# laurabragagnolo/SkelSplat

Hardware: AMD Instinct MI355X
Metric: rendered+backpropagated views/s (differentiable skeletal-Gaussian rasterizer fwd+bwd) (higher is better)
Workload: dtype f32

## Files before the change

include/skelsplat_hip.h:

```cpp
#ifndef SKELSPLAT_HIP_H
#define SKELSPLAT_HIP_H

#include <stddef.h>
#include <stdint.h>

#ifdef __cplusplus
extern "C" {
#endif

#define SKS_MAX_VIEWS 64
#define SKS_MAX_CHANNELS 32
#define SKS_SMALL_P 256

#define SKS_ANTIALIASING 1u
#define SKS_CLAMP01      2u
#define SKS_FORCE_BINNED 4u
#define SKS_DEBUG_SYNC   8u

#define SKS_NO_NT_STORES 16u

#define SKS_RAW_PARAMS   32u
#define SKS_RAW_GRADS    128u
#define SKS_BIN_CLEAN    64u
#define SKS_BIN_GROUPS_SHIFT 16
#define SKS_BIN_GROUPS(n) ((unsigned)(((n) - 1) & 7) << SKS_BIN_GROUPS_SHIFT)
#define SKS_FILL_LINEAR (1u << 21)
#define SKS_FILL_ROWS (1u << 22)
#define SKS_BWD_LDS_LIST (1u << 20)
#define SKS_BWD_WG_SHIFT 23
#define SKS_NO_EARLY_FILL (1u << 30)
#define SKS_EARLY_FILL(n) (((unsigned)(n) & 7u) << SKS_BIN_GROUPS_SHIFT)

const char* sks_last_error(void);
int sks_version(void);

int sks_scratch_bytes(int V, int P, int C, int W, int H, size_t bin_capacity,
                      size_t* geom_bytes, size_t* binning_bytes, size_t* accum_bytes);

int sks_forward(int V, int P, int C, int W, int H,
                const float* viewmatrix, const float* projmatrix,
                const float* tanfovx , const float* tanfovy ,
                const float* means3D, const float* features, const float* opacities,
                const float* scales, const float* rotations, const float* cov3D_precomp,
                float scale_modifier, unsigned flags,
                float* out_color, float* out_invdepth, int* radii,
                void* geom, void* binning, size_t bin_capacity, int* num_rendered_dev,
                float* final_T, uint32_t* n_contrib, void* stream);

int sks_backward(int V, int P, int C, int W, int H,
                 const float* viewmatrix, const float* projmatrix,
                 const float* tanfovx , const float* tanfovy ,
                 const float* bg,
                 const float* means3D, const float* features, const float* opacities,
                 const float* scales, const float* rotations, const float* cov3D_precomp,
                 float scale_modifier, unsigned flags,
                 const int* radii, const void* geom, const void* binning, size_t bin_capacity,
                 const float* dL_dout_color, const float* dL_dout_invdepth,
                 void* accum,
                 float* dL_dmeans3D, float* dL_dmeans2D, float* dL_dopacity,
                 float* dL_dscales, float* dL_drotations, float* dL_dcov3D, float* dL_dfeatures,
                 float* dL_dmeans3D_mean ,
                 void* stream);

#define SKS_FB_NO_JOIN 1u
int sks_forward_backward(int V, int P, int C, int W, int H,
                         const float* viewmatrix, const float* projmatrix,
                         const float* tanfovx , const float* tanfovy ,
                         const float* means3D, const float* features, const float* opacities,
                         const float* scales, const float* rotations, const float* cov3D_precomp,
                         float scale_modifier, unsigned flags,
                         float* out_color, float* out_invdepth, int* radii,
                         void* geom, void* binning, size_t bin_capacity, int* num_rendered_dev,
                         const float* bg, const float* dL_dout_color, const float* dL_dout_invdepth, void* accum,
                         float* dL_dmeans3D, float* dL_dmeans2D, float* dL_dopacity,
                         float* dL_dscales, float* dL_drotations, float* dL_dcov3D, float* dL_dfeatures,
                         float* dL_dmeans3D_mean, void* stream, void* aux_stream, unsigned fb_flags);

int sks_mean_views(int V, int P, const float* dL_dmeans3D, int shard_world, float* mean_out , void* stream);

int sks_mark_visible(int P, const float* means3D, const float* viewmatrix, const float* projmatrix,
                     uint8_t* present, void* stream);

int sks_export_lists(int V, int W, int H, const void* binning, size_t bin_capacity,
                     uint32_t* point_list, uint32_t* ranges, void* stream);

int sks_masked_l2(int V, size_t n_per_view, const float* render, const float* gt, float* dL_unscaled, double* sums,
                  void* stream);
int sks_masked_l2_loss(int V, size_t n_per_view, const float* render, const float* gt, float* dL_unscaled, double* sums,
                       float* loss , float* scale , int mean, void* stream);

#define SKS_SOFTARGMAX_STATS 6
size_t sks_softargmax_scratch_bytes(int planes, int W, int H);
int sks_softargmax_fwd(int planes, int W, int H, float beta, const float* img, float* xy ,
                       float* stats , void* scratch, size_t scratch_bytes, void* stream);
int sks_softargmax_bwd(int planes, int W, int H, float beta, const float* img, const float* stats ,
                       const float* dL_dxy , float* dL_dimg, void* stream);

int sks_heatmaps(int V, int J, int W, int H, const float* row, const float* col, const float* cmin, const float* den,
                 float* out, double* gt_totals, void* stream);
int sks_heatmap_factors(int V, int J, int W, int H, const float* means3D, const float* scales, const float* rotations,
                        float scale_modifier, const float* poses_2d, const float* viewmatrix, const float* tanfovx,
                        const float* tanfovy, float* row, float* col, float* cmin, float* den,
                        int frames ,
                        const int* view_wh ,
                        void* stream);
int sks_heatmap_totals(int V, int J, int W, int H, const float* row, const float* col, const float* cmin, const float* den,
                       const int* view_wh, double* gt_totals, void* stream);

int sks_triangulate(int N, int V, int J, const double* proj, size_t rig_stride, const float* poses_2d,
                    const double* poses_2d_f64, const unsigned char* valid, float* xyz, double* xyzw, int* n_used,
                    void* stream);

int sks_fuse_predictions(int N, int V, int J, const double* proj, size_t rig_stride, const float* poses_3d,
                         const double* poses_3d_f64, const float* poses_2d, const double* poses_2d_f64,
                         const unsigned char* valid, int norm_f32, float* xyz, double* xyz_f64, double* reproj_err,
                         int* n_used, void* stream);

int sks_fused_ssim_fwd(int B, int CH, int H, int W, float C1, float C2, const float* img1, const float* img2,
                       float* ssim_map, float* dm_dmu1, float* dm_dsigma1_sq, float* dm_dsigma12, void* stream);

int sks_fused_ssim_bwd(int B, int CH, int H, int W, float C1, float C2, const float* img1, const float* img2,
                       const float* dL_dmap, const float* dm_dmu1, const float* dm_dsigma1_sq, const float* dm_dsigma12,
                       float* dL_dimg1, void* stream);
int sks_fused_ssim_bwd_uniform(int B, int CH, int H, int W, const float* img1, const float* img2, const float* dL_value,
                               float dL_scale, int crop, const float* dm_dmu1, const float* dm_dsigma1_sq,
                               const float* dm_dsigma12, float* dL_dimg1, void* stream);
#define SKS_SSIM_SUM_SLOTS 64
#define SKS_SSIM_SCRATCH_BYTES (SKS_SSIM_SUM_SLOTS * 8)
int sks_fused_ssim_mean(int B, int CH, int H, int W, float C1, float C2, const float* img1, const float* img2, int crop,
                        float* dm_dmu1, float* dm_dsigma1_sq, float* dm_dsigma12, double* scratch, float* mean_out,
                        void* stream);

int sks_knn3_meandist2(int P, const float* points, float* mean_dist2, void* stream);
size_t sks_knn3_scratch_bytes(int P);
int sks_knn3_meandist2_grid(int P, const float* points, float* mean_dist2, void* scratch, size_t scratch_bytes, void* stream);

int sks_gt_tile_stats(int V, int C, int W, int H, const float* gt, float* tile_S, float* tile_N, double* totals, void* stream);
int sks_geometry(int V, int P, int C, int W, int H, const float* viewmatrix, const float* projmatrix,
                 const float* tanfovx , const float* tanfovy , const float* means3D,
                 const float* opacities, const float* scales, const float* rotations, const float* cov3D_precomp,
                 float scale_modifier, unsigned flags, int* radii, void* geom,
                 const int* view_wh , int frames ,
                 void* stream);
int sks_backward_fused_loss(int V, int P, int C, int W, int H, const float* viewmatrix, const float* projmatrix,
                            const float* tanfovx , const float* tanfovy , const float* bg,
                            const float* means3D, const float* features, const float* opacities, const float* scales,
                            const float* rotations, const float* cov3D_precomp, float scale_modifier, unsigned flags,
                            const int* radii, const void* geom, const float* gt, const float* tile_S, const float* tile_N,
                            const double* gt_totals, void* accum, float* dL_dmeans3D, float* dL_dmeans2D,
                            float* dL_dopacity, float* dL_dscales, float* dL_drotations, float* dL_dcov3D,
                            double* loss_sums, float* packed_raw_grads ,
                            const int* view_wh , const size_t* gt_offsets ,
                            const float* const* hm_factors , void* stream);

int sks_loop_pack_grads(int V, int P, const float* dL_dmeans3D, const float* dL_dscales, const float* dL_drotations,
                        const float* dL_dopacity, const float* raw_scaling, const float* raw_rotation,
                        const float* raw_opacity, const double* loss_sums, float* packed, void* stream);
int sks_loop_adam_step(int V, int P, const float* grads, float* slots, unsigned long long group_mask, int last_view,
                       float* xyz, float* scaling, float* rotation, float* opacity, float* exp_avg, float* exp_avg_sq,
                       int* counters, int acc_steps, const double* lr_sched ,
                       const double* lrs , const double* adam ,
                       float lambda_consistency, const int* limb ,
                       int shard_world ,
                       void* stream);

int sks_loop_adam_step_es(int V, int P, const float* grads, float* slots, unsigned long long group_mask, int last_view,
                          float* xyz, float* scaling, float* rotation, float* opacity, float* exp_avg, float* exp_avg_sq,
                          int* counters, int acc_steps, const double* lr_sched , const double* lrs ,
                          const double* adam , float lambda_consistency, const int* limb ,
                          int shard_world, const double* loss_sums, int* es_state, int es_window, float es_tolerance,
                          int* es_host_flag , void* stream);
size_t sks_loop_shard_floats(int V, int P, int shard_world);

int sks_adam_multi(int n_tensors, float* const* params, const float* const* grads, float* const* exp_avg, float* const* exp_avg_sq,
                   const long long* numel, const double* lr, const long long* step, double beta1, double beta2, double eps, void* stream);

int sks_loop_fused_step(int V, int P, int C, int W, int H, const float* viewmatrix, const float* projmatrix,
                        const float* tanfovx , const float* tanfovy , const float* features,
                        float scale_modifier, unsigned flags, int* radii, void* geom, const float* gt,
                        const double* gt_totals, void* accum, double* loss_sums, float* packed, float* slots,
                        unsigned long long group_mask, int last_view, float* xyz, float* scaling, float* rotation,
                        float* opacity, float* exp_avg, float* exp_avg_sq, int* counters, int acc_steps,
                        const double* lr_sched , const double* lrs , const double* adam ,
                        float lambda_consistency, const int* limb ,
                        const int* view_wh , const size_t* gt_offsets ,
                        int frames, const float* const* hm_factors ,
                        void* stream);
int sks_loop_fused_step_es(int V, int P, int C, int W, int H, const float* viewmatrix, const float* projmatrix,
                           const float* tanfovx , const float* tanfovy , const float* features,
                           float scale_modifier, unsigned flags, int* radii, void* geom, const float* gt,
                           const double* gt_totals, void* accum, double* loss_sums, float* packed, float* slots,
                           unsigned long long group_mask, int last_view, float* xyz, float* scaling, float* rotation,
                           float* opacity, float* exp_avg, float* exp_avg_sq, int* counters, int acc_steps,
                           const double* lr_sched , const double* lrs , const double* adam ,
                           float lambda_consistency, const int* limb ,
                           const int* view_wh , const size_t* gt_offsets ,
                           int frames, const float* const* hm_factors ,
                           int* es_state, int es_window, float es_tolerance, int* es_host_flags ,
                           void* stream);

int sks_rig_select(int R, int V, int frames, const int* rig_ids, const float* bank_viewmatrix, const float* bank_projmatrix,
                   const float* bank_tan, const int* slot_wh, const double* bank_proj, const double* bank_sched,
                   float* viewmatrix, float* projmatrix, void* views_dev, double* proj, double* lr_sched_dev, int* error_word,
                   void* stream);
int sks_geometry_dv(int V, int P, int C, int W, int H, const float* viewmatrix, const float* projmatrix, const void* views_dev,
                    const float* means3D, const float* opacities, const float* scales, const float* rotations,
                    const float* cov3D_precomp, float scale_modifier, unsigned flags, int* radii, void* geom, int frames,
                    void* stream);
int sks_heatmap_factors_dv(int V, int J, int W, int H, const float* means3D, const float* scales, const float* rotations,
                           float scale_modifier, const float* poses_2d, const float* viewmatrix, const void* views_dev,
                           float* row, float* col, float* cmin, float* den, int frames, void* stream);
int sks_heatmap_totals_dv(int V, int J, int W, int H, const float* row, const float* col, const float* cmin, const float* den,
                          const void* views_dev, double* gt_totals, void* stream);
int sks_loop_fused_step_dv(int V, int P, int C, int W, int H, const float* viewmatrix, const float* projmatrix,
                           const void* views_dev, const float* features, float scale_modifier, unsigned flags, int* radii,
// ... 38 lines not shown
```

skelsplat_amd/_lib.py:

```python
import ctypes as C
import os

_HERE = os.path.dirname(os.path.abspath(__file__))
LIB_PATH = os.path.join(_HERE, "libskelsplat_hip.so")
_lib = None

SKS_MAX_VIEWS = 64
SKS_MAX_CHANNELS = 32
SKS_SMALL_P = 256
SKS_ANTIALIASING = 1
SKS_CLAMP01 = 2
SKS_FORCE_BINNED = 4
SKS_DEBUG_SYNC = 8
SKS_NO_NT_STORES = 16
SKS_RAW_PARAMS = 32
SKS_BIN_CLEAN = 64
SKS_RAW_GRADS = 128
SKS_FB_NO_JOIN = 1
SKS_BIN_GROUPS_SHIFT = 16
SKS_BWD_WG_SHIFT = 23
SKS_SSIM_SCRATCH_BYTES = 64 * 8
SKS_SOFTARGMAX_STATS = 6
SKS_REPORT_MAX_SAVES = 8
SKS_EVAL_MAX_GROUPS = 64


SKS_NO_EARLY_FILL = 1 << 30


def SKS_EARLY_FILL(n):
    return (int(n) & 7) << SKS_BIN_GROUPS_SHIFT


def SKS_BIN_GROUPS(n):
    return ((int(n) - 1) & 7) << SKS_BIN_GROUPS_SHIFT


_vp, _i, _u, _f, _sz = C.c_void_p, C.c_int, C.c_uint, C.c_float, C.c_size_t

_CAMERAS = (("V", _i), ("P", _i), ("C", _i), ("W", _i), ("H", _i), ("viewmatrix", _vp), ("projmatrix", _vp),
            ("tanfovx", _vp), ("tanfovy", _vp))
_GAUSSIANS = (("means3D", _vp), ("features", _vp), ("opacities", _vp), ("scales", _vp), ("rotations", _vp),
              ("cov3D_precomp", _vp), ("scale_modifier", _f), ("flags", _u))
_UPSTREAM = (("dL_dout_color", _vp), ("dL_dout_invdepth", _vp), ("accum", _vp))
_GRADS = (("dL_dmeans3D", _vp), ("dL_dmeans2D", _vp), ("dL_dopacity", _vp), ("dL_dscales", _vp), ("dL_drotations", _vp),
          ("dL_dcov3D", _vp), ("dL_dfeatures", _vp), ("dL_dmeans3D_mean", _vp))
_FORWARD_IO = (("out_color", _vp), ("out_invdepth", _vp), ("radii", _vp), ("geom", _vp), ("binning", _vp),
               ("bin_capacity", _sz), ("num_rendered_dev", _vp))
FORWARD_PARAMS = _CAMERAS + _GAUSSIANS + _FORWARD_IO + (("final_T", _vp), ("n_contrib", _vp), ("stream", _vp))
BACKWARD_PARAMS = _CAMERAS + (("bg", _vp),) + _GAUSSIANS + (("radii", _vp), ("geom", _vp), ("binning", _vp), ("bin_capacity", _sz)) \
    + _UPSTREAM + _GRADS + (("stream", _vp),)
FORWARD_BACKWARD_PARAMS = _CAMERAS + _GAUSSIANS + _FORWARD_IO + (("bg", _vp),) + _UPSTREAM + _GRADS \
    + (("stream", _vp), ("aux_stream", _vp), ("fb_flags", _u))

FWD, BWD, FWD_BWD = ({name: i for i, (name, _) in enumerate(params)}
                     for params in (FORWARD_PARAMS, BACKWARD_PARAMS, FORWARD_BACKWARD_PARAMS))
FWD_BWD_SOURCES = tuple(("fwd", FWD[n]) if n in FWD else ("bwd", BWD[n]) if n in BWD else None for n in FWD_BWD)

_ull = C.c_ulonglong
_VIEWS_DV = (("viewmatrix", _vp), ("projmatrix", _vp), ("views_dev", _vp))
RIG_SELECT_PARAMS = (("R", _i), ("V", _i), ("frames", _i), ("rig_ids", _vp), ("bank_viewmatrix", _vp), ("bank_projmatrix", _vp),
                     ("bank_tan", _vp), ("slot_wh", _vp), ("bank_proj", _vp), ("bank_sched", _vp), ("viewmatrix", _vp),
                     ("projmatrix", _vp), ("views_dev", _vp), ("proj", _vp), ("lr_sched_dev", _vp), ("error_word", _vp),
                     ("stream", _vp))
GEOMETRY_DV_PARAMS = (("V", _i), ("P", _i), ("C", _i), ("W", _i), ("H", _i)) + _VIEWS_DV + (
    ("means3D", _vp), ("opacities", _vp), ("scales", _vp), ("rotations", _vp), ("cov3D_precomp", _vp), ("scale_modifier", _f),
    ("flags", _u), ("radii", _vp), ("geom", _vp), ("frames", _i), ("stream", _vp))
HEATMAP_FACTORS_DV_PARAMS = (("V", _i), ("J", _i), ("W", _i), ("H", _i), ("means3D", _vp), ("scales", _vp), ("rotations", _vp),
                             ("scale_modifier", _f), ("poses_2d", _vp), ("viewmatrix", _vp), ("views_dev", _vp), ("row", _vp),
                             ("col", _vp), ("cmin", _vp), ("den", _vp), ("frames", _i), ("stream", _vp))
HEATMAP_TOTALS_DV_PARAMS = (("V", _i), ("J", _i), ("W", _i), ("H", _i), ("row", _vp), ("col", _vp), ("cmin", _vp), ("den", _vp),
                            ("views_dev", _vp), ("gt_totals", _vp), ("stream", _vp))
OPTIMISER_PARAMS = (("slots", _vp), ("group_mask", _ull), ("last_view", _i), ("xyz", _vp), ("scaling", _vp), ("rotation", _vp),
                    ("opacity", _vp), ("exp_avg", _vp), ("exp_avg_sq", _vp), ("counters", _vp), ("acc_steps", _i),
                    ("lr_sched", _vp), ("lrs", _vp), ("adam", _vp), ("lambda_consistency", _f), ("limb", _vp))
OPTIMISER_DV_PARAMS = tuple(("lr_sched_dev", ct) if name == "lr_sched" else (name, ct) for name, ct in OPTIMISER_PARAMS)
_ES = (("es_state", _vp), ("es_window", _i), ("es_tolerance", _f))
ES_PARAMS, ES_FRAMES_PARAMS = _ES + (("es_host_flag", _vp),), _ES + (("es_host_flags", _vp),)
_ADAM_STEP = (("V", _i), ("P", _i), ("grads", _vp)) + OPTIMISER_PARAMS + (("shard_world", _i),)
_STEP_RENDER = (("features", _vp), ("scale_modifier", _f), ("flags", _u), ("radii", _vp), ("geom", _vp), ("gt", _vp),
                ("gt_totals", _vp), ("accum", _vp), ("loss_sums", _vp), ("packed", _vp))
_STEP_HEATMAPS = (("view_wh", _vp), ("gt_offsets", _vp), ("frames", _i), ("hm_factors", _vp))
_STEP = _CAMERAS + _STEP_RENDER + OPTIMISER_PARAMS + _STEP_HEATMAPS
_STEP_DV = (("V", _i), ("P", _i), ("C", _i), ("W", _i), ("H", _i)) + _VIEWS_DV + _STEP_RENDER + OPTIMISER_DV_PARAMS + _STEP_HEATMAPS
LOOP_ADAM_STEP_PARAMS = _ADAM_STEP + (("stream", _vp),)
LOOP_ADAM_STEP_ES_PARAMS = _ADAM_STEP + (("loss_sums", _vp),) + ES_PARAMS + (("stream", _vp),)
LOOP_FUSED_STEP_PARAMS = _STEP + (("stream", _vp),)
LOOP_FUSED_STEP_ES_PARAMS = _STEP + ES_FRAMES_PARAMS + (("stream", _vp),)
LOOP_FUSED_STEP_DV_PARAMS = _STEP_DV + (("stream", _vp),)
LOOP_FUSED_STEP_ES_DV_PARAMS = _STEP_DV + ES_FRAMES_PARAMS + (("stream", _vp),)
STEP_PARAMS = {"sks_loop_adam_step": LOOP_ADAM_STEP_PARAMS, "sks_loop_adam_step_es": LOOP_ADAM_STEP_ES_PARAMS,
               "sks_loop_fused_step": LOOP_FUSED_STEP_PARAMS, "sks_loop_fused_step_es": LOOP_FUSED_STEP_ES_PARAMS}
DV_PARAMS = {"sks_rig_select": RIG_SELECT_PARAMS, "sks_geometry_dv": GEOMETRY_DV_PARAMS,
             "sks_heatmap_factors_dv": HEATMAP_FACTORS_DV_PARAMS, "sks_heatmap_totals_dv": HEATMAP_TOTALS_DV_PARAMS,
             "sks_loop_fused_step_dv": LOOP_FUSED_STEP_DV_PARAMS, "sks_loop_fused_step_es_dv": LOOP_FUSED_STEP_ES_DV_PARAMS}

SIGNATURES = {
    "sks_last_error": (C.c_char_p, []),
    "sks_version": (_i, []),
    "sks_scratch_bytes": (_i, [_i, _i, _i, _i, _i, _sz, C.POINTER(_sz), C.POINTER(_sz), C.POINTER(_sz)]),
    "sks_forward": (_i, [ct for _, ct in FORWARD_PARAMS]),
    "sks_backward": (_i, [ct for _, ct in BACKWARD_PARAMS]),
    "sks_forward_backward": (_i, [ct for _, ct in FORWARD_BACKWARD_PARAMS]),
    "sks_mark_visible": (_i, [_i, _vp, _vp, _vp, _vp, _vp]),
    "sks_mean_views": (_i, [_i, _i, _vp, _i, _vp, _vp]),
    "sks_export_lists": (_i, [_i, _i, _i, _vp, _sz, _vp, _vp, _vp]),
    "sks_masked_l2": (_i, [_i, _sz, _vp, _vp, _vp, _vp, _vp]),
    "sks_masked_l2_loss": (_i, [_i, _sz, _vp, _vp, _vp, _vp, _vp, _vp, _i, _vp]),
    "sks_fused_ssim_fwd": (_i, [_i, _i, _i, _i, _f, _f, _vp, _vp, _vp, _vp, _vp, _vp, _vp]),
    "sks_fused_ssim_bwd": (_i, [_i, _i, _i, _i, _f, _f, _vp, _vp, _vp, _vp, _vp, _vp, _vp, _vp]),
    "sks_fused_ssim_bwd_uniform": (_i, [_i, _i, _i, _i, _vp, _vp, _vp, _f, _i, _vp, _vp, _vp, _vp, _vp]),
    "sks_fused_ssim_mean": (_i, [_i, _i, _i, _i, _f, _f, _vp, _vp, _i, _vp, _vp, _vp, _vp, _vp, _vp]),
    "sks_knn3_meandist2": (_i, [_i, _vp, _vp, _vp]),
    "sks_knn3_scratch_bytes": (_sz, [_i]),
    "sks_knn3_meandist2_grid": (_i, [_i, _vp, _vp, _vp, _sz, _vp]),
    "sks_softargmax_scratch_bytes": (_sz, [_i, _i, _i]),
    "sks_softargmax_fwd": (_i, [_i, _i, _i, _f, _vp, _vp, _vp, _vp, _sz, _vp]),
    "sks_softargmax_bwd": (_i, [_i, _i, _i, _f, _vp, _vp, _vp, _vp, _vp]),
    "sks_heatmaps": (_i, [_i, _i, _i, _i, _vp, _vp, _vp, _vp, _vp, _vp, _vp]),
    "sks_heatmap_factors": (_i, [_i, _i, _i, _i, _vp, _vp, _vp, _f, _vp, _vp, _vp, _vp, _vp, _vp, _vp, _vp, _i, _vp, _vp]),
    "sks_heatmap_totals": (_i, [_i, _i, _i, _i, _vp, _vp, _vp, _vp, _vp, _vp, _vp]),
    "sks_gt_tile_stats": (_i, [_i, _i, _i, _i, _vp, _vp, _vp, _vp, _vp]),
    "sks_geometry": (_i, [_i, _i, _i, _i, _i, _vp, _vp, _vp, _vp, _vp, _vp, _vp, _vp, _vp, _f, _u, _vp, _vp, _vp, _i, _vp]),
    "sks_backward_fused_loss": (_i, [_i, _i, _i, _i, _i, _vp, _vp, _vp, _vp, _vp, _vp, _vp, _vp, _vp, _vp, _vp, _f, _u,
                                     _vp, _vp, _vp, _vp, _vp, _vp, _vp, _vp, _vp, _vp, _vp, _vp, _vp, _vp, _vp, _vp, _vp, _vp, _vp]),
    "sks_loop_pack_grads": (_i, [_i, _i, _vp, _vp, _vp, _vp, _vp, _vp, _vp, _vp, _vp, _vp]),
    "sks_loop_shard_floats": (_sz, [_i, _i, _i]),
    "sks_adam_multi": (_i, [_i, _vp, _vp, _vp, _vp, _vp, _vp, _vp, C.c_double, C.c_double, C.c_double, _vp]),
    "sks_triangulate": (_i, [_i, _i, _i, _vp, _sz, _vp, _vp, _vp, _vp, _vp, _vp, _vp]),
    "sks_fuse_predictions": (_i, [_i, _i, _i, _vp, _sz, _vp, _vp, _vp, _vp, _vp, _i, _vp, _vp, _vp, _vp, _vp]),
    **{name: (_i, [ct for _, ct in params]) for name, params in {**STEP_PARAMS, **DV_PARAMS}.items()},
    "sks_pose_errors": (_i, [_i, _i, _vp, _vp, _vp, _vp, _vp]),
    "sks_loop_report": (_i, [_i, _i, _i, _vp, _vp, _i, _vp, _vp, _vp, _i, _i, _vp, _vp, _vp, _i, _vp, _vp, _vp]),
    "sks_eval_sequence": (_i, [_i, _i, _vp, _vp, _vp, _i, _vp, _vp, _vp]),
    "sks_prof_enable": (_i, [_i]),
    "sks_prof_spin": (_i, [C.c_double, _vp]),
    "sks_prof_read": (_i, [_i, C.POINTER(C.c_double), C.POINTER(C.c_longlong)]),
    "sks_prof_count": (_i, [_i, C.POINTER(C.c_longlong)]),
    "sks_prof_read_quantiles": (_i, [_i, C.POINTER(C.c_double), C.POINTER(C.c_double), C.POINTER(C.c_longlong)]),
}


def load(build_if_missing=True):
    global _lib
    if _lib is not None:
        return _lib
    if build_if_missing:
        try:
            from . import build as _b
            if _b._stale():
                _b.build()
        except Exception as e:
            if not os.path.exists(LIB_PATH):
                raise ImportError(f"libskelsplat_hip.so is missing and could not be built: {e}") from e
    if not os.path.exists(LIB_PATH):
        raise ImportError(f"{LIB_PATH} not found; run `python -m skelsplat_amd.build`")
    lib = C.CDLL(os.environ.get("SKS_LIB_OVERRIDE") or LIB_PATH)
    for name, (res, args) in SIGNATURES.items():
        fn = getattr(lib, name)
        fn.restype = res
        fn.argtypes = args
    _lib = lib
    return lib


def check(rc, what):
    if rc != 0:
        msg = load().sks_last_error().decode(errors="replace")
        raise RuntimeError(f"{what} failed (code {rc}): {msg}")


def scratch_bytes(V, P, C_, W, H, bin_capacity=0):
    g, b, a = _sz(0), _sz(0), _sz(0)
    check(load().sks_scratch_bytes(V, P, C_, W, H, bin_capacity, C.byref(g), C.byref(b), C.byref(a)), "sks_scratch_bytes")
    return g.value, b.value, a.value


def ptr(t):
    if t is None or t.numel() == 0:
        return None
    return t.data_ptr()


def farray(vals):
    return (C.c_float * len(vals))(*[float(v) for v in vals])


def prof_count(kind):
    n = C.c_longlong(0)
    check(load().sks_prof_count(kind, C.byref(n)), "sks_prof_count")
    return n.value


def prof_enable(on, every=1, kinds=(0, 1), recorded=False):
    skip = sum(1 << (16 + k) for k in (0, 1) if k not in kinds)
    check(load().sks_prof_enable((min(0xffff, max(1, int(every))) | skip | ((1 << 18) if recorded else 0)) if on else 0),
          "sks_prof_enable")


def prof_read_quantiles(kind):
    q = (C.c_double * 3)()
    ms, n = C.c_double(0), C.c_longlong(0)
    check(load().sks_prof_read_quantiles(kind, q, C.byref(ms), C.byref(n)), "sks_prof_read_quantiles")
    return ms.value, n.value, (q[0], q[1], q[2])


def prof_read(kind):
    ms, n = C.c_double(0), C.c_longlong(0)
    check(load().sks_prof_read(kind, C.byref(ms), C.byref(n)), "sks_prof_read")
    return ms.value, n.value
```

skelsplat_amd/csrc/sks_bwd_small.inc:

```
template <int CG>
struct BwdPix {
    float T, T_final, last_alpha, accum_inv, last_inv, dLi, bgdot;
    float dL[CG], accum_rec[CG], last_color[CG];
};

struct BwdArgs {
    int P, C, W, H;
    unsigned flags;
    Geom g;
    const float* features;
    const float* bg;
    const float* dL_color;
    const float* dL_invdepth;
    float* accum;
    const float* tile_S;
    const float* tile_N;
    const float* hm_row = nullptr;
    const float* hm_col = nullptr;
    const float* hm_cmin = nullptr;
    const float* hm_den = nullptr;
    const int* es_stop = nullptr;
    int es_stride = 0;
    int es_views = 1;
};
// ... 86 lines not shown
        L.invd[rank] = xyd.w;
        L.xr[rank] = (int)(r.x | (r.z << 16));
        L.yr[rank] = (int)(r.y | (r.w << 16));
        L.id[rank] = tid;
    }
    __syncthreads();
    if (tid < CG) {
        bool act = false;
        if (tid < C) {
            act = DFEAT || a.bg != nullptr;
            for (int k = 0; k < n && !act; k++) act = L.r_feat[L.id[k] * C + tid] != 0.0f;
        }
        s_act[tid] = act ? 1 : 0;
    }
    __syncthreads();
    if (tid < CG && s_act[tid]) {
        int pos = 0;
        for (int c = 0; c < tid; c++) pos += s_act[c];
        s_chan[pos] = tid;
    }
    int nc = 0;
    for (int c = 0; c < CG; c++) nc += s_act[c];
    __syncthreads();
    if (tid < n) {
        const int id = L.id[tid];
#pragma unroll
        for (int j = 0; j < CG; j++) L.feat[tid * CG + j] = j < nc ? L.r_feat[id * C + s_chan[j]] : 0.0f;
    }
    __syncthreads();
    int kg = 0;
    for (int k = 0; k < n; k++) kg = L.id[k] == g ? k : kg;
    const bool do_clamp = a.flags & SKS_CLAMP01;
    const float ddelx_dx = (float)(0.5 * W), ddely_dy = (float)(0.5 * H);
    float sum[NV];
#pragma unroll
    for (int j = 0; j < NV; j++) sum[j] = 0.0f;

    for (int c = sp; c < nchunks; c += BWD_SPLITS) {
        const int i = c * 256 + tid;
        if (i >= npx) continue;
        const int yy = i / wpx;
        const int x = x0 + (i - yy * wpx), y = y0 + yy;
        const int tx = x >> 4, ty = y >> 4;
        const float pxf = (float)x, pyf = (float)y;
        float T = 1.0f, col[CG];
#pragma unroll
        for (int ch = 0; ch < CG; ch++) col[ch] = 0.0f;
        int klast = -1;
        for (int k = 0; k < n; k++) {
            const int xr = L.xr[k], yr = L.yr[k];
            if (tx < (xr & 0xffff) || tx >= (xr >> 16) || ty < (yr & 0xffff) || ty >= (yr >> 16)) continue;
            const float2 xy = L.xy[k];
            const float4 co = L.co[k];
            const float dx = xy.x - pxf, dy = xy.y - pyf;
            const float power = -0.5f * (co.x * dx * dx + co.z * dy * dy) - co.y * dx * dy;
            if (power > 0.0f) continue;
            const float alpha = fminf(0.99f, co.w * expf_fixed(power));
            if (alpha < 1.0f / 255.0f) continue;
            const float test_T = T * (1 - alpha);
            if (test_T < 0.0001f) break;
            if (do_clamp) {
#pragma unroll
                for (int ch = 0; ch < CG; ch++) col[ch] += L.feat[k * CG + ch] * alpha * T;
            }
            T = test_T;
            klast = k;
        }
        if (klast < kg) continue;
        const size_t pix = (size_t)y * W + x;
        float dLraw[CG];
        {
            const float* dLc = a.dL_color + (size_t)v * C * HW + pix;
#pragma unroll
            for (int j = 0; j < CG; j++) dLraw[j] = j < nc ? dLc[(size_t)s_chan[j] * HW] : 0.0f;
        }
        const float dLi_raw = a.dL_invdepth ? a.dL_invdepth[(size_t)v * HW + pix] : 0.0f;
        BwdPix<CG> s;
        s.T = T;
        s.T_final = T;
        s.last_alpha = 0;
        s.accum_inv = 0;
        s.last_inv = 0;
        s.bgdot = 0;
        s.dLi = dLi_raw;
#pragma unroll
        for (int j = 0; j < CG; j++) {
            float d = dLraw[j];
            if (do_clamp && !(col[j] >= 0.0f && col[j] <= 1.0f)) d = 0.0f;
            if (a.bg && j < nc) s.bgdot += a.bg[s_chan[j]] * d;
            s.dL[j] = d;
            s.accum_rec[j] = 0;
            s.last_color[j] = 0;
        }
        for (int k = klast; k >= kg; k--) {
            const int xr = L.xr[k], yr = L.yr[k];
            if (tx < (xr & 0xffff) || tx >= (xr >> 16) || ty < (yr & 0xffff) || ty >= (yr >> 16)) continue;
            const float2 xy = L.xy[k];
            const float4 co = L.co[k];
            const float dx = xy.x - pxf, dy = xy.y - pyf;
            const float power = -0.5f * (co.x * dx * dx + co.z * dy * dy) - co.y * dx * dy;
            if (power > 0.0f) continue;
            const float G = expf_fixed(power);
            const float alpha = fminf(0.99f, co.w * G);
            if (alpha < 1.0f / 255.0f) continue;
            s.T = s.T / (1.f - alpha);
            const float dchannel_dcolor = alpha * s.T;
            float dL_dalpha = 0.0f;
            const bool mine = k == kg;
#pragma unroll
            for (int ch = 0; ch < CG; ch++) {
                const float cc = L.feat[k * CG + ch];
                s.accum_rec[ch] = s.last_alpha * s.last_color[ch] + (1.f - s.last_alpha) * s.accum_rec[ch];
                s.last_color[ch] = cc;
                const float dL_dchannel = s.dL[ch];
                dL_dalpha += (cc - s.accum_rec[ch]) * dL_dchannel;
                if (DFEAT && mine) sum[NACC + ch] += dchannel_dcolor * dL_dchannel;
            }
            const float invd = L.invd[k];
            s.accum_inv = s.last_alpha * s.last_inv + (1.f - s.last_alpha) * s.accum_inv;
            s.last_inv = invd;
            dL_dalpha += (invd - s.accum_inv) * s.dLi;
            dL_dalpha *= s.T;
            s.last_alpha = alpha;
            dL_dalpha += (-s.T_final / (1.f - alpha)) * s.bgdot;
            if (mine) {
                const float dL_dG = co.w * dL_dalpha;
                const float gdx = G * dx, gdy = G * dy;
                const float dG_ddelx = -gdx * co.x - gdy * co.y;
                const float dG_ddely = -gdy * co.z - gdx * co.y;
                sum[0] += dL_dG * dG_ddelx * ddelx_dx;
                sum[1] += dL_dG * dG_ddely * ddely_dy;
                sum[2] += -0.5f * gdx * dx * dL_dG;
                sum[3] += -0.5f * gdx * dy * dL_dG;
                sum[4] += -0.5f * gdy * dy * dL_dG;
                sum[5] += G * dL_dalpha;
                sum[6] += dchannel_dcolor * s.dLi;
            }
        }
    }
    const int lane = tid & 63, wv = tid >> 6;
#pragma unroll
    for (int j = 0; j < NV; j++) {
        const float r = wave_sum(sum[j]);
        if (lane == 0) s_red[wv][j] = r;
    }
    __syncthreads();
    if (tid < NVS)
        out[tid * BWD_SPLITS] = tid < NV ? ((s_red[0][tid] + s_red[1][tid]) + (s_red[2][tid] + s_red[3][tid])) : 0.0f;
}

__device__ __forceinline__ float rl(float x, int lane) { return __int_as_float(__builtin_amdgcn_readlane(__float_as_int(x), lane)); }
__device__ __forceinline__ unsigned rlu(unsigned x, int lane) { return (unsigned)__builtin_amdgcn_readlane((int)x, lane); }

template <int CG, bool DFEAT, bool LOSS, bool HMF = false, bool ES = false>
__global__ __launch_bounds__(256, (DFEAT || CG > 20) ? 1 : 4) void k_render_bwd_wave(BwdArgs a, ViewTan vt, ViewOff vo)
{
    static_assert(!(DFEAT && LOSS), "the fused-loss variant has no feature gradient");
    static_assert(LOSS || !HMF, "heat-map factors belong to the fused-loss variant");
    static_assert(LOSS || !ES, "early stopping belongs to the fused-loss variant");
    if constexpr (ES) {
        if (a.es_stop[(size_t)((int)blockIdx.y / a.es_views) * a.es_stride] != 0) return;
    }
    constexpr int NV = LOSS ? NACC + 1 : NACC + (DFEAT ? CG : 0);
    __shared__ float s_red[2][4][NV];
    const int g = blockIdx.x, v = blockIdx.y, sp = blockIdx.z, zs = gridDim.z, tid = threadIdx.x, lane = tid & 63, wv = tid >> 6;
    const int P = a.P, C = a.C, W = vt.w[v], H = vt.h[v];
    const int NVS = NACC + C;
    const size_t HW = (size_t)H * W;
    const size_t go = (size_t)v * P;
    const float* dL_view = a.dL_color + vo.off[v];
    float* out_g = a.accum + ((size_t)v * P + g) * NVS * BWD_SPLITS;
    const bool has = lane < P;
    const int li = has ? lane : 0;
    const float4 m_co = a.g.co[go + li];
    const float4 m_xyd = a.g.xyd[go + li];
    uint4 m_rect = a.g.rect[go + li];
    if (!has) m_rect = make_uint4(0, 0, 0, 0);
    float m_feat[CG];
    unsigned m_fmask = 0;
#pragma unroll
    for (int ch = 0; ch < CG; ch++) {
        m_feat[ch] = (ch < C && has) ? a.features[li * C + ch] : 0.0f;
        m_fmask |= m_feat[ch] != 0.0f ? (1u << ch) : 0u;
    }

    const unsigned gx0 = rlu(m_rect.x, g), gy0 = rlu(m_rect.y, g), gx1 = rlu(m_rect.z, g), gy1 = rlu(m_rect.w, g);
    const int wt = (int)gx1 - (int)gx0, ht = (int)gy1 - (int)gy0;
    const int nchunks = wt * ht;
    if (sp >= nchunks) {
        for (int slot = sp; slot < BWD_SPLITS; slot += zs)
            if (tid < NVS) out_g[tid * BWD_SPLITS + slot] = 0.0f;
        return;
    }
    const bool hit = m_rect.x < gx1 && m_rect.z > gx0 && m_rect.y < gy1 && m_rect.w > gy0;
    const unsigned long long hm = __ballot(hit);
    const int n = __popcll(hm);
    const unsigned mydepth = __float_as_uint(m_xyd.z);
    int rank = 0;
    for (unsigned long long m = hm; m; m &= m - 1) {
        const int j = __builtin_ctzll(m);
        const unsigned dj = rlu(mydepth, j);
        rank += (dj < mydepth || (dj == mydepth && j < lane)) ? 1 : 0;
    }
    const int kg = __builtin_amdgcn_readlane(rank, g);
    unsigned chmask = 0;
    if (DFEAT || a.bg != nullptr) {
        chmask = C >= 32 ? 0xffffffffu : ((1u << C) - 1u);
    } else {
        for (unsigned long long m = hm; m; m &= m - 1) chmask |= rlu(m_fmask, __builtin_ctzll(m));
    }
    const bool do_clamp = a.flags & SKS_CLAMP01;
    const float ddelx_dx = (float)(0.5 * W), ddely_dy = (float)(0.5 * H);
    const unsigned chmask_all = chmask;
    const size_t HW_all = HW;
    int buf = 0;
    for (int slot = sp; slot < BWD_SPLITS; slot += zs, buf ^= 1) {
    float* out = out_g + slot;
    if (slot >= nchunks) {
        if (tid < NVS) out[tid * BWD_SPLITS] = 0.0f;
        continue;
    }
    float sum[NV];
#pragma unroll
    for (int j = 0; j < NV; j++) sum[j] = 0.0f;
    for (int c = slot; c < nchunks; c += BWD_SPLITS) {
        unsigned chmask = chmask_all;
        size_t HW = HW_all;
        asm volatile("" : "+s"(chmask), "+s"(HW));
        const int tyl = c / wt;
        const int tx = (int)gx0 + (c - tyl * wt), ty = (int)gy0 + tyl;
        const int x = tx * TILE + (tid & 15), y = ty * TILE + (tid >> 4);
        const bool in = x < W && y < H;
        const float pxf = (float)x, pyf = (float)y;
        float T = 1.0f, col[CG];
#pragma unroll
        for (int ch = 0; ch < CG; ch++) col[ch] = 0.0f;
        int klast = -1;
        const bool hitc = hit && !((unsigned)tx < m_rect.x || (unsigned)tx >= m_rect.z || (unsigned)ty < m_rect.y || (unsigned)ty >= m_rect.w);
        const unsigned long long covm = __ballot(hitc);
        const int minid = covm ? __builtin_ctzll(covm) : 0x7fffffff;
        bool alive = in;
        unsigned chm_t = (DFEAT || a.bg != nullptr) ? chmask : 0u;
        for (int k = 0; k < n; k++) {
            const unsigned long long sel = __ballot(hitc && rank == k);
            if (!sel) continue;
            if (!LOSS && !__any(alive)) break;
            const int lk = __builtin_ctzll(sel);
            chm_t |= chmask & rlu(m_fmask, lk);
            const float ex = rl(m_xyd.x, lk), ey = rl(m_xyd.y, lk);
            const float cx = rl(m_co.x, lk), cy = rl(m_co.y, lk), cz = rl(m_co.z, lk), cw = rl(m_co.w, lk);
            const bool cov = alive;
            const float dx = ex - pxf, dy = ey - pyf;
            const float power = -0.5f * (cx * dx * dx + cz * dy * dy) - cy * dx * dy;
            const float alpha = fminf(0.99f, cw * expf_fixed(power));
            const float test_T = T * (1 - alpha);
            const bool pass = cov && !(power > 0.0f) && !(alpha < 1.0f / 255.0f);
            const bool stop = pass && test_T < 0.0001f;
            const bool acc = pass && !stop;
            if (do_clamp || LOSS) {
                for (unsigned fm = chmask & rlu(m_fmask, lk); fm; fm &= fm - 1) {
                    const int ch = __builtin_ctz(fm);
                    const float f = rl(m_feat[ch], lk);
                    const float add = f * alpha * T;
                    col[ch] += acc ? add : 0.0f;
                }
            }
            if (acc) { T = test_T; klast = k; }
            if (stop) alive = false;
        }
        const bool need = in && klast >= kg;
        bool own = false;
        if (LOSS && in && minid == g) {
            for (unsigned fm = chm_t; fm; fm &= fm - 1) own = own || col[__builtin_ctz(fm)] > 0.0f;
        }
        if (!__any(need || own)) continue;
        const size_t pix = (size_t)y * W + x;
        struct { float T, T_final, last_alpha, accum_inv, last_inv, bgdot, dLi; } s;
        s.T = T; s.T_final = T; s.last_alpha = 0; s.accum_inv = 0; s.last_inv = 0; s.bgdot = 0;
        s.dLi = (!LOSS && need && a.dL_invdepth) ? a.dL_invdepth[(size_t)v * HW + pix] : 0.0f;
        {
            const float* dLc = dL_view + pix;
            for (unsigned fm = chm_t; fm;) {
                int cc[4];
                float cv[4], gv[4];
#pragma unroll
                for (int i = 0; i < 4; i++) {
                    cc[i] = fm ? __builtin_ctz(fm) : -1;
                    fm &= fm - 1;
                }
#pragma unroll
                for (int i = 0; i < 4; i++) cv[i] = col[max(cc[i], 0)];
                if (HMF) {
                    float fr[4], fc[4], lo[4], dn[4];
#pragma unroll
                    for (int i = 0; i < 4; i++) {
                        const int vc = v * C + max(cc[i], 0);
                        const bool want = cc[i] >= 0 && (need || (own && cv[i] > 0.0f));
                        fr[i] = want ? a.hm_row[(size_t)vc * a.H + y] : 0.0f;
                        fc[i] = want ? a.hm_col[(size_t)vc * a.W + x] : 0.0f;
                        lo[i] = a.hm_cmin[vc];
                        dn[i] = a.hm_den[vc];
                    }
#pragma unroll
                    for (int i = 0; i < 4; i++) {
                        const bool want = cc[i] >= 0 && (need || (own && cv[i] > 0.0f));
                        gv[i] = want ? (fr[i] * fc[i] - lo[i]) / dn[i] : 0.0f;
                    }
                } else {
#pragma unroll
                    for (int i = 0; i < 4; i++) {
                        const bool want = LOSS ? (need || (own && cv[i] > 0.0f)) : need;
                        gv[i] = (cc[i] >= 0 && want) ? dLc[(size_t)max(cc[i], 0) * HW] : 0.0f;
                    }
                }
#pragma unroll
                for (int i = 0; i < 4; i++) {
                    if (cc[i] < 0) break;
                    const int ch = cc[i];
// ... 158 lines not shown
```

skelsplat_amd/csrc/sks_common.inc:

```
thread_local char g_err[512] = "";

int fail(int code, const char* fmt, ...)
{
    va_list ap;
    va_start(ap, fmt);
    vsnprintf(g_err, sizeof(g_err), fmt, ap);
    va_end(ap);
    return code;
}

#define HIP_TRY(expr)                                                                          \
    do {                                                                                       \
        hipError_t e_ = (expr);                                                                \
        if (e_ != hipSuccess) return fail((int)e_, "%s: %s", #expr, hipGetErrorString(e_));    \
    } while (0)

#define STAGE_CHECK(name)                                                                      \
    do {                                                                                       \
        HIP_TRY(hipGetLastError());                                                            \
        if (flags & SKS_DEBUG_SYNC) {                                                          \
            hipError_t e_ = hipStreamSynchronize(st);                                          \
            if (e_ != hipSuccess) return fail((int)e_, "stage %s: %s", name, hipGetErrorString(e_)); \
        }                                                                                      \
    } while (0)

constexpr int PROF_MAX = 16384;
struct ProfKind {
    hipEvent_t b[PROF_MAX], e[PROF_MAX];
    int created = 0, n = 0;
};
struct ProfState {
    bool on = false;
    int every = 1;
    int skip = 0;
    bool recorded = false;
    int seen[2] = { 0, 0 };
    ProfKind kind[2];
};
thread_local ProfState* tl_prof = nullptr;

struct ProfScope {
    ProfKind* k = nullptr;
    hipStream_t st;
    bool ext;
    bool began = false;
    ProfScope(int kind, hipStream_t s, bool ext_ = false) : st(s), ext(ext_)
    {
        ProfState* ps = tl_prof;
        if (!ps || !ps->on || ((ps->skip >> kind) & 1)) return;
        if (ps->seen[kind]++ % ps->every != 0) return;
        ProfKind& p = ps->kind[kind];
        if (p.n >= PROF_MAX) return;
        if (p.n >= p.created) {
            if (hipEventCreate(&p.b[p.created]) != hipSuccess || hipEventCreate(&p.e[p.created]) != hipSuccess) return;
            p.created++;
        }
        k = &p;
        if (ps->recorded) ext = false;
        if (!ext) (void)hipEventRecord(p.b[p.n], st);
    }
    hipEvent_t eb() const { return k->b[k->n]; }
    hipEvent_t ee() const { return k->e[k->n]; }
    ~ProfScope()
    {
        if (!k) return;
        if (!ext) (void)hipEventRecord(k->e[k->n], st);
        k->n++;
    }
};
#define SKS_LAUNCH(prof, kernel, grid, block, lds, stream, ...)                                                  \
    do {                                                                                                         \
        if ((prof).k)                                                                                            \
            hipExtLaunchKernelGGL(kernel, grid, block, lds, stream, (prof).began ? nullptr : (prof).eb(), (prof).ee(), 0, __VA_ARGS__); \
        else hipLaunchKernelGGL(kernel, grid, block, lds, stream, __VA_ARGS__);                                  \
    } while (0)
#define SKS_LAUNCH_FIRST(prof, kernel, grid, block, lds, stream, ...)                                            \
    do {                                                                                                         \
        if ((prof).k && (prof).ext) hipExtLaunchKernelGGL(kernel, grid, block, lds, stream, (prof).eb(), nullptr, 0, __VA_ARGS__); \
        else hipLaunchKernelGGL(kernel, grid, block, lds, stream, __VA_ARGS__);    \
        (prof).began = (prof).k != nullptr;                                                                      \
    } while (0)

constexpr int NACC = 8;
constexpr int BWD_SPLITS = 16;
constexpr int BWD_WG_PAIRS16 = 400;
constexpr int BWD_WG_PAIRS8 = 4096;

struct ViewTan {
    float x[SKS_MAX_VIEWS];
    float y[SKS_MAX_VIEWS];
    int w[SKS_MAX_VIEWS];
    int h[SKS_MAX_VIEWS];
};
struct ViewOff {
    unsigned long long off[SKS_MAX_VIEWS];
};
struct ViewTanDev {
    const float* x;
    const float* y;
    const int* w;
    const int* h;
    const double* sched;
};
inline ViewTanDev views_dev_from(const void* views_dev, const double* sched = nullptr)
{
    const ViewTan* t = (const ViewTan*)views_dev;
    return ViewTanDev{ t->x, t->y, t->w, t->h, sched };
}
inline bool fill_views(ViewTan& vt, ViewOff* vo, int V, int C, int W, int H, const float* tanfovx, const float* tanfovy,
                       const int* view_wh, const size_t* plane_off)
{
    for (int v = 0; v < V; v++) {
        vt.x[v] = tanfovx[v];
        vt.y[v] = tanfovy[v];
        vt.w[v] = view_wh ? view_wh[2 * v] : W;
        vt.h[v] = view_wh ? view_wh[2 * v + 1] : H;
        if (vt.w[v] < 1 || vt.h[v] < 1 || vt.w[v] > W || vt.h[v] > H) return false;
        if (vo) vo->off[v] = plane_off ? (unsigned long long)plane_off[v] : (unsigned long long)v * C * H * W;
    }
    return true;
}

struct Geom {
    float4* co;
    float4* xyd;
    uint4* rect;
    uint32_t* cover;
};

__host__ __device__ inline size_t align256(size_t x) { return (x + 255) & ~(size_t)255; }

struct Activated {
    float opacity, s[3], q[4], qnorm;
};
__device__ __forceinline__ Activated activate(bool raw, float op, const float s[3], const float q[4])
{
    Activated a;
    if (raw) {
        a.opacity = 1.0f / (1.0f + expf_fixed(-op));
#pragma unroll
        for (int k = 0; k < 3; k++) a.s[k] = expf_fixed(s[k]);
        const float nn = q[0] * q[0] + q[1] * q[1] + q[2] * q[2] + q[3] * q[3];
        a.qnorm = fmaxf(sqrtf(nn), 1e-12f);
#pragma unroll
        for (int k = 0; k < 4; k++) a.q[k] = q[k] / a.qnorm;
    } else {
        a.opacity = op;
        a.qnorm = 1.0f;
#pragma unroll
        for (int k = 0; k < 3; k++) a.s[k] = s[k];
#pragma unroll
        for (int k = 0; k < 4; k++) a.q[k] = q[k];
    }
    return a;
}

#ifndef SKS_COVER_MAX_WORDS
#define SKS_COVER_MAX_WORDS 6144
#endif
constexpr int COVER_MAX_WORDS = SKS_COVER_MAX_WORDS;
__host__ __device__ inline int cover_cw(int W) { return (1 + (((W + TILE - 1) / TILE) + 31) / 32 + 3) & ~3; }
inline bool cover_enabled(int P, int W, int H)
{
    return P <= SKS_SMALL_P && ((H + TILE - 1) / TILE) * cover_cw(W) <= COVER_MAX_WORDS;
}
inline bool cover_per_plane(int P, int W, int H, int C)
{
    return cover_enabled(P, W, H) && (C + 1) * ((H + TILE - 1) / TILE) * cover_cw(W) <= COVER_MAX_WORDS;
}
inline Geom geom_from(void* base, int V, int P, int W, int H)
{
    char* p = (char*)base;
    Geom g;
    size_t n = (size_t)V * P;
    g.co = (float4*)p; p += align256(n * sizeof(float4));
    g.xyd = (float4*)p; p += align256(n * sizeof(float4));
    g.rect = (uint4*)p; p += align256(n * sizeof(uint4));
    g.cover = cover_enabled(P, W, H) ? (uint32_t*)p : nullptr;
    return g;
}
inline size_t geom_bytes(int V, int P, int W, int H, int C)
{
    const int planes = cover_per_plane(P, W, H, C) ? C + 1 : 1;
    return 3 * align256((size_t)V * P * 16) + align256((size_t)V * planes * ((H + TILE - 1) / TILE) * cover_cw(W) * 4);
}

constexpr int BIN_WAVE_SORT = 64;
constexpr int BIN_ROWS = 2;
constexpr int BIN_CLASSES = 8;
constexpr int BIN_HDR_CLASS = 8;
constexpr int BIN_MAX_GROUPS = 7;
#ifndef SKS_BIN_FB_GROUPS
#define SKS_BIN_FB_GROUPS 1
#endif
constexpr int BIN_FB_GROUPS = SKS_BIN_FB_GROUPS;
inline int bin_groups_default()
{
    static const int n = [] {
        const char* e = getenv("SKS_BIN_GROUPS");
        const int want = (e && atoi(e) > 0) ? atoi(e) : BIN_FB_GROUPS;
        return want < 1 ? 1 : (want > BIN_MAX_GROUPS ? BIN_MAX_GROUPS : want);
    }();
    return n;
}
inline void bin_groups(unsigned flags, int V, int& vg, int& ng)
{
    const unsigned field = (flags >> SKS_BIN_GROUPS_SHIFT) & 7u;
    int want = field ? 1 + (int)field : bin_groups_default();
    if (want > BIN_MAX_GROUPS) want = BIN_MAX_GROUPS;
    if (want > V) want = V;
    vg = (V + want - 1) / want;
    ng = (V + vg - 1) / vg;
}
struct Bin {
    uint32_t* hdr;
    uint32_t* count;
    uint32_t* cursor;
    uint2* ranges;
    int* nrend;
    uint32_t* longt;
    uint4* tlist;
    uint32_t* tidx;
// ... 45 lines not shown
```

skelsplat_amd/csrc/sks_fwd_small.inc:

```
__device__ __forceinline__ float clamp01(float x) { return fminf(fmaxf(x, 0.0f), 1.0f); }

struct FwdArgs {
    int P, C, W, H;
    unsigned flags;
    Geom g;
    const float* features;
    float* out_color;
    float* out_invdepth;
    float* final_T;
    uint32_t* n_contrib;
    int tslots;
    unsigned cp1_magic;
    int ncomp;
    int cover_planes;
    unsigned w_magic;
};

inline int composite_slots(unsigned flags, int V, int P)
{
    const int t = (int)((flags >> 26) & 15u);
    return t ? t : ((long long)V * P <= 128 ? 4 : 8);
}

typedef float v4f __attribute__((ext_vector_type(4)));
// ... 225 lines not shown
    const int tid = threadIdx.x;
    const int P = a.P, C = a.C, W = a.W, H = a.H;
    const size_t HW = (size_t)H * W;

    const int xq = blockIdx.x, band_id = blockIdx.y, zid = blockIdx.z;
    const int xc = gridDim.x - fsplit;
    const bool comp_role = xq >= fsplit;
    if (comp_role) {
        const int cb = (zid * gy + band_id) * xc + (xq - fsplit);
        if (cb >= a.ncomp) return;
        const int T_SLOTS = a.tslots;
        const int slot = cb % T_SLOTS;
        const int g = (cb / T_SLOTS) % P;
        const int v = cb / (T_SLOTS * P);
        const size_t go = (size_t)v * P;
        const float4* gco = a.g.co + go;
        const float4* gxyd = a.g.xyd + go;
        const uint4* grect = a.g.rect + go;
        const uint4 rg = grect[g];
        const int wt = (int)(rg.z - rg.x), ht = (int)(rg.w - rg.y);
        const int ntiles = wt * ht;
        if (slot >= ntiles) return;
        const int cap = (P + 15) & ~15;
        DynList<CG> L(s_dyn, cap);
        if (tid < P) L.rect[tid] = grect[tid];
        __syncthreads();
        float* outc = a.out_color + (size_t)v * C * HW;
        float* outi = a.out_invdepth + (size_t)v * HW;
        const bool do_clamp = a.flags & SKS_CLAMP01;
        for (int t = slot; t < ntiles; t += T_SLOTS) {
            const int ty = (int)rg.y + t / wt, tx = (int)rg.x + t % wt;
            if (tid == 0) { s_n = 0; s_min = 0x7fffffff; }
            __syncthreads();
            if (tid < P) {
                const uint4 r = L.rect[tid];
                if ((int)r.x <= tx && tx < (int)r.z && (int)r.y <= ty && ty < (int)r.w) {
                    atomicMin(&s_min, tid);
                    const int sl = atomicAdd(&s_n, 1);
                    L.key[sl] = ((unsigned long long)__float_as_uint(gxyd[tid].z) << 32) | (unsigned)tid;
                }
            }
            __syncthreads();
            const int n = s_n;
            if (s_min == g) {
                if (tid < n) {
                    const unsigned long long key = L.key[tid];
                    int rank = 0;
                    for (int j = 0; j < n; j++) rank += (L.key[j] < key) ? 1 : 0;
                    const int id = (int)(unsigned)key;
                    const float4 xyd = gxyd[id];
                    L.xy[rank] = make_float2(xyd.x, xyd.y);
                    L.co[rank] = gco[id];
                    L.invd[rank] = xyd.w;
#pragma unroll
                    for (int ch = 0; ch < CG; ch++) L.feat[rank * CG + ch] = ch < C ? a.features[id * C + ch] : 0.0f;
                }
                __syncthreads();
                unsigned chm = 0xffffffffu;
                if (a.cover_planes) {
                    bool nz = false;
                    if (tid < CG)
                        for (int k = 0; k < n; k++) nz = nz || L.feat[k * CG + tid] != 0.0f;
                    if (tid < 64) {
                        const unsigned long long bl = __ballot(nz);
                        if (tid == 0) s_chm = (unsigned)bl;
                    }
                    __syncthreads();
                    chm = s_chm;
                }
                const int x = tx * TILE + (tid & 15), y = ty * TILE + (tid >> 4);
                if (x < W && y < H) {
                    const float pxf = (float)x, pyf = (float)y;
                    float T = 1.0f, inv = 0.0f, acc[CG];
#pragma unroll
                    for (int ch = 0; ch < CG; ch++) acc[ch] = 0.0f;
                    uint32_t contributor = 0, last = 0;
                    for (int k = 0; k < n; k++) {
                        contributor++;
                        const float2 xy = L.xy[k];
                        const float4 co = L.co[k];
                        const float dx = xy.x - pxf, dy = xy.y - pyf;
                        const float power = -0.5f * (co.x * dx * dx + co.z * dy * dy) - co.y * dx * dy;
                        if (power > 0.0f) continue;
                        const float alpha = fminf(0.99f, co.w * expf_fixed(power));
                        if (alpha < 1.0f / 255.0f) continue;
                        const float test_T = T * (1 - alpha);
                        if (test_T < 0.0001f) break;
#pragma unroll
                        for (int ch = 0; ch < CG; ch++) acc[ch] += L.feat[k * CG + ch] * alpha * T;
                        inv += L.invd[k] * alpha * T;
                        T = test_T;
                        last = contributor;
                    }
                    const size_t pix = (size_t)y * W + x;
#pragma unroll
                    for (int ch = 0; ch < CG; ch++)
                        if (ch < C && ((chm >> ch) & 1u)) outc[(size_t)ch * HW + pix] = do_clamp ? clamp01(acc[ch]) : acc[ch];
                    outi[pix] = inv;
                    if (a.final_T) a.final_T[(size_t)v * HW + pix] = T;
                    if (a.n_contrib) a.n_contrib[(size_t)v * HW + pix] = last;
                }
            }
            __syncthreads();
        }
        return;
    }
    fwd_fill_role<PPT, NT, HALF>(a, cp1_magic, xq, band_id, zid, gy, pb, cover);
}

struct EarlyFill {
    float* out_color;
    float* out_invdepth;
    int C, W, H, gy;
    int gplanes;
    int ngeom;
    int zid0;
    int fsplit, pb;
    unsigned cp1_magic;
    unsigned row_magic;
    unsigned fs_magic;
};

template <int PPT, bool NT>
__global__ __launch_bounds__(256) void k_geom_fwd_fill(EarlyFill f, int P, ViewTan vt, const float* __restrict__ vms,
                                                       const float* __restrict__ pms, const float* __restrict__ means,
                                                       const float* __restrict__ opac, const float* __restrict__ scales,
                                                       const float* __restrict__ rots, const float* __restrict__ cov3Dp, float smod,
                                                       unsigned flags, Geom g, int* __restrict__ radii,
                                                       const float* __restrict__ features, int cover_planes)
{
    const int b = blockIdx.x;
    if (b < f.ngeom) {
        const int v = f.gplanes == 1 ? b : (int)(((unsigned)b * f.cp1_magic) >> 20);
        extern __shared__ __attribute__((aligned(16))) char s_dyn[];
        geom_fwd_block((uint32_t*)s_dyn, 0, v, b - v * f.gplanes, P, f.W, f.H, vt, vms, pms, means, opac, scales, rots, cov3Dp, smod, flags, g, radii, 0,
                       nullptr, nullptr, features, f.C, nullptr, nullptr, cover_planes);
        return;
    }
    const unsigned e = (unsigned)(b - f.ngeom);
    const unsigned rows = (unsigned)(f.fsplit * f.gy);
    const unsigned zr = f.row_magic ? __umulhi(e, f.row_magic) : e;
    const unsigned rem = e - zr * rows;
    const int band = (int)(f.fs_magic ? __umulhi(rem, f.fs_magic) : rem);
    const int q = (int)rem - band * f.fsplit;
    const int zid = f.zid0 + (int)zr;
    const int v = (int)(((unsigned)zid * f.cp1_magic) >> 20);
    const int plane = zid - v * (f.C + 1);
    const size_t HW = (size_t)f.H * f.W;
    const int Nb = min(TILE, f.H - band * TILE) * f.W;
    float* out = (plane == f.C ? f.out_invdepth + (size_t)v * HW : f.out_color + ((size_t)v * f.C + plane) * HW) + (size_t)band * TILE * f.W;
    const int shift = (int)((reinterpret_cast<uintptr_t>(out) >> 2) & 31u);
    fill_bare<PPT, NT>(out, nullptr, nullptr, q * (256 * PPT) * f.pb + (int)threadIdx.x * PPT - shift, Nb, min(f.pb, 32));
}
```

skelsplat_amd/csrc/sks_geom_bwd.inc:

```
struct GeomBwdArgs {
    int P, C, W, H;
    unsigned flags;
    const float* vms;
    const float* pms;
    const float* means;
    const float* opac;
    const float* scales;
    const float* rots;
    const float* cov3Dp;
    float smod;
    const int* radii;
    const float* accum;
    int nsplit;
    const double* gt_totals;
    double* loss_sums;
    float* packed;
    float* dmeans3D;
    float* dmeans2D;
    float* dopacity;
    float* dscales;
    float* drots;
    float* dcov3D;
    float* dfeat;
    const uint4* rect = nullptr;
// ... 255 lines not shown
            M3 M2;
#pragma unroll
            for (int cc = 0; cc < 3; cc++)
#pragma unroll
                for (int rr = 0; rr < 3; rr++) M2.m[cc][rr] = 2.0f * M.m[cc][rr];
            const M3 dL_dM = m3mul(M2, dS);
            const M3 Rt = m3T(R);
            M3 dMt = m3T(dL_dM);
#pragma unroll
            for (int k = 0; k < 3; k++)
                dscale[k] = Rt.m[k][0] * dMt.m[k][0] + Rt.m[k][1] * dMt.m[k][1] + Rt.m[k][2] * dMt.m[k][2];
#pragma unroll
            for (int k = 0; k < 3; k++)
#pragma unroll
                for (int rr = 0; rr < 3; rr++) dMt.m[k][rr] *= s[k];
            dq[0] = 2 * z * (dMt.m[0][1] - dMt.m[1][0]) + 2 * y * (dMt.m[2][0] - dMt.m[0][2]) + 2 * x * (dMt.m[1][2] - dMt.m[2][1]);
            dq[1] = 2 * y * (dMt.m[1][0] + dMt.m[0][1]) + 2 * z * (dMt.m[2][0] + dMt.m[0][2]) + 2 * r * (dMt.m[1][2] - dMt.m[2][1]) - 4 * x * (dMt.m[2][2] + dMt.m[1][1]);
            dq[2] = 2 * x * (dMt.m[1][0] + dMt.m[0][1]) + 2 * r * (dMt.m[2][0] - dMt.m[0][2]) + 2 * z * (dMt.m[1][2] + dMt.m[2][1]) - 4 * y * (dMt.m[2][2] + dMt.m[0][0]);
            dq[3] = 2 * r * (dMt.m[0][1] - dMt.m[1][0]) + 2 * x * (dMt.m[2][0] + dMt.m[0][2]) + 2 * y * (dMt.m[1][2] + dMt.m[2][1]) - 4 * z * (dMt.m[1][1] + dMt.m[0][0]);
        }
    }
    if (a.dmeans3D) { a.dmeans3D[3 * o] = dmean[0]; a.dmeans3D[3 * o + 1] = dmean[1]; a.dmeans3D[3 * o + 2] = dmean[2]; }
    if (a.dmeans2D) { a.dmeans2D[3 * o] = dm2x; a.dmeans2D[3 * o + 1] = dm2y; a.dmeans2D[3 * o + 2] = 0.0f; }
    const bool rawg = (a.flags & SKS_RAW_PARAMS) && (a.flags & SKS_RAW_GRADS);
    if (a.dopacity) {
        float oj = 1.0f;
        if (rawg) {
            const float so = 1.0f / (1.0f + expf_fixed(-(PRE ? pre->opac : a.opac[idx])));
            oj = so * (1.0f - so);
        }
        a.dopacity[o] = dop * oj;
    }
    if (a.dcov3D) {
#pragma unroll
        for (int i = 0; i < 6; i++) a.dcov3D[6 * o + i] = dcov[i];
    }
    if (a.dscales) {
#pragma unroll
        for (int k = 0; k < 3; k++) a.dscales[3 * o + k] = dscale[k] * (rawg ? sc[k] : 1.0f);
    }
    if (a.drots) {
        float dot = 0.0f;
#pragma unroll
        for (int k = 0; k < 4; k++) dot += q[k] * dq[k];
#pragma unroll
        for (int k = 0; k < 4; k++) a.drots[4 * o + k] = rawg ? (dq[k] - q[k] * dot) / qnorm : dq[k];
    }
    if (a.packed) {
        float scl = 1.0f;
        if (a.loss_sums) scl = (float)(1.0 / (n_view < 1.0 ? 1.0 : n_view));
        float* pk = a.packed + o * 11;
        const bool raw = a.flags & SKS_RAW_PARAMS;
        pk[0] = dmean[0] * scl; pk[1] = dmean[1] * scl; pk[2] = dmean[2] * scl;
#pragma unroll
        for (int k = 0; k < 3; k++) pk[3 + k] = dscale[k] * (raw ? sc[k] : 1.0f) * scl;
        float dot = 0.0f;
#pragma unroll
        for (int k = 0; k < 4; k++) dot += q[k] * dq[k];
#pragma unroll
        for (int k = 0; k < 4; k++) pk[6 + k] = (raw ? (dq[k] - q[k] * dot) / qnorm : dq[k]) * scl;
        float oj = 1.0f;
        if (raw) {
            const float so = 1.0f / (1.0f + expf_fixed(-(PRE ? pre->opac : a.opac[idx])));
            oj = so * (1.0f - so);
        }
        pk[10] = dop * oj * scl;
    }
}

__global__ __launch_bounds__(256) void k_geom_bwd(GeomBwdArgs a, ViewTan vt)
{
    const int idx = blockIdx.x * 256 + threadIdx.x;
    const int v = blockIdx.y;
    float g[NACC];
    double pS, pN;
    if (a.dfeat) geom_bwd_dfeat(a, (size_t)v * a.P + blockIdx.x * 256, min(256, a.P - (int)blockIdx.x * 256), threadIdx.x, 256);
    geom_bwd_load<false>(a, v, idx, g, pS, pN);
    double n_view = 1.0;
    if (a.loss_sums) {
        __shared__ double s_l[2][4];
        pS = wave_sum_d(pS);
        pN = wave_sum_d(pN);
        if ((threadIdx.x & 63) == 0) { s_l[0][threadIdx.x >> 6] = pS; s_l[1][threadIdx.x >> 6] = pN; }
        __syncthreads();
        const double S = a.gt_totals[2 * v] + ((s_l[0][0] + s_l[0][1]) + (s_l[0][2] + s_l[0][3]));
        n_view = a.gt_totals[2 * v + 1] + ((s_l[1][0] + s_l[1][1]) + (s_l[1][2] + s_l[1][3]));
        if (threadIdx.x == 0) {
            a.loss_sums[2 * v] = S;
            a.loss_sums[2 * v + 1] = n_view;
        }
    }
    if (idx >= a.P) return;
    geom_bwd_finish(a, vt, v, idx, g, n_view);
}

constexpr int GEOMB_G = 64;
__global__ __launch_bounds__(256) void k_geom_bwd_binned(GeomBwdArgs a, ViewTan vt)
{
    __shared__ float s_g[GEOMB_G][4][NACC];
    const int tid = threadIdx.x, v = blockIdx.y + a.v0;
    const int idx = blockIdx.x * GEOMB_G + tid;
    GeomBwdIn in;
    const bool mine = tid < GEOMB_G && idx < a.P;
    if (mine) geom_bwd_fetch(a, v, idx, in);
    {
        const int gi = tid >> 2, st = tid & 3;
        const int gidx = blockIdx.x * GEOMB_G + gi;
        float sum[NACC];
#pragma unroll
        for (int k = 0; k < NACC; k++) sum[k] = 0.0f;
        if (gidx < a.P) {
            const size_t o = (size_t)v * a.P + gidx;
            const uint4 r = a.rect[o];
            const int n = BIN_ROWS * (int)((r.z - r.x) * (r.w - r.y));
            const size_t s0 = BIN_ROWS * (size_t)a.goff[o], send = BIN_ROWS * a.cap;
            const float4* rows = reinterpret_cast<const float4*>(a.part + (size_t)v * a.cap * BIN_ROWS * NACC);
            for (int i = st; i < n; i += 16) {
                float4 q[4][2];
#pragma unroll
                for (int u = 0; u < 4; u++) {
                    const bool on = i + 4 * u < n && s0 + i + 4 * u < send;
                    q[u][0] = on ? rows[(s0 + i + 4 * u) * 2] : make_float4(0, 0, 0, 0);
                    q[u][1] = on ? rows[(s0 + i + 4 * u) * 2 + 1] : make_float4(0, 0, 0, 0);
                }
#pragma unroll
                for (int u = 0; u < 4; u++) {
                    sum[0] += q[u][0].x; sum[1] += q[u][0].y; sum[2] += q[u][0].z; sum[3] += q[u][0].w;
                    sum[4] += q[u][1].x; sum[5] += q[u][1].y; sum[6] += q[u][1].z;
                }
            }
        }
        float4* sg = reinterpret_cast<float4*>(s_g[gi][st]);
        sg[0] = make_float4(sum[0], sum[1], sum[2], sum[3]);
        sg[1] = make_float4(sum[4], sum[5], sum[6], 0.0f);
    }
    __syncthreads();
    if (!mine) return;
    float g[NACC];
#pragma unroll
    for (int k = 0; k < NACC - 1; k++) g[k] = (s_g[tid][0][k] + s_g[tid][1][k]) + (s_g[tid][2][k] + s_g[tid][3][k]);
    g[NACC - 1] = 0.0f;
    if (a.bin_hdr[0]) {
#pragma unroll
        for (int k = 0; k < NACC - 1; k++) g[k] = __int_as_float(0x7fc00000);
    }
    if (a.dfeat) {
        const size_t o = (size_t)v * a.P + idx;
        const float* acc = a.accum + o * (NACC + a.C);
        for (int ch = 0; ch < a.C; ch++) a.dfeat[o * a.C + ch] = acc[NACC + ch];
    }
    geom_bwd_finish<true>(a, vt, v, idx, g, 1.0, &in);
}

__global__ __launch_bounds__(256) void k_geom_bwd_all(GeomBwdArgs a, ViewTan vt, int V, float* __restrict__ mean_out)
{
    const int t = threadIdx.x;
    const int v = t / a.P, idx = t - v * a.P;
    const bool live = v < V;
    float g[NACC];
    double pS, pN;
    if (a.dfeat) geom_bwd_dfeat(a, 0, V * a.P, t, 256);
    if (live) {
        geom_bwd_load<false>(a, v, idx, g, pS, pN);
        geom_bwd_finish(a, vt, v, idx, g, 1.0);
    }
    __syncthreads();
    if (t < a.P) {
        float m[3] = { 0.0f, 0.0f, 0.0f };
        for (int w0 = 0; w0 < V; w0 += 4) {
            float tv[4][3];
#pragma unroll
            for (int j = 0; j < 4; j++) {
                const float* gm = a.dmeans3D + ((size_t)(w0 + j < V ? w0 + j : V - 1) * a.P + t) * 3;
                tv[j][0] = gm[0]; tv[j][1] = gm[1]; tv[j][2] = gm[2];
            }
#pragma unroll
            for (int j = 0; j < 4; j++)
                if (w0 + j < V) { m[0] += tv[j][0]; m[1] += tv[j][1]; m[2] += tv[j][2]; }
        }
        mean_out[3 * t] = m[0] / (float)V; mean_out[3 * t + 1] = m[1] / (float)V; mean_out[3 * t + 2] = m[2] / (float)V;
    }
}
__global__ void k_mean_views(int V, int P, const float* __restrict__ dmeans3D, float* __restrict__ mean_out, int world = 1)
{
    const int i = blockIdx.x * blockDim.x + threadIdx.x;
    if (i >= 3 * P) return;
    const int vmax = (V + world - 1) / world;
    float m = 0.0f;
    for (int w0 = 0; w0 < V; w0 += 8) {
        float t[8];
#pragma unroll
        for (int j = 0; j < 8; j++) {
            const int w = w0 + j < V ? w0 + j : V - 1;
            const int row = world == 1 ? w : (w % world) * vmax + w / world;
            t[j] = dmeans3D[(size_t)row * P * 3 + i];
        }
#pragma unroll
        for (int j = 0; j < 8; j++)
            if (w0 + j < V) m += t[j];
    }
    mean_out[i] = m / (float)V;
}

template <bool ES = false, class VT = ViewTan>
__global__ __launch_bounds__(256) void k_step_tail(GeomBwdArgs ga, VT vt, sksloop::AdamArgs aa, int V, Geom g, int* radii)
{
    __shared__ float s_xyz[256 * 3];
    __shared__ float s_hyp[6];
    __shared__ double s_d[4];
    __shared__ int s_it[2];
    __shared__ float s_np[64 * 11];
    const int tid = threadIdx.x, lane = tid & 63, wv = tid >> 6;
    const int P = ga.P;
    const int f = blockIdx.x, vb = f * V;
    if (f) {
        ga.means += (size_t)f * P * 3; ga.opac += (size_t)f * P; ga.scales += (size_t)f * P * 3; ga.rots += (size_t)f * P * 4;
        aa.grads += (size_t)vb * P * 11; aa.slots += (size_t)vb * P * 3;
        aa.xyz += (size_t)f * P * 3; aa.scaling += (size_t)f * P * 3; aa.rotation += (size_t)f * P * 4; aa.opacity += (size_t)f * P;
        aa.m += (size_t)f * P * 11; aa.vv += (size_t)f * P * 11; aa.counters += 2 * f;
    }
    if constexpr (std::is_same<VT, ViewTanDev>::value) {
        const double* r = vt.sched + 5 * (size_t)f;
        aa.log_lr_init = r[0]; aa.log_lr_final = r[1]; aa.lr_delay_mult = r[2];
        aa.lr_delay_steps = (int)r[3]; aa.lr_max_steps = (int)r[4];
        aa.lr_init = r[0] == -INFINITY ? 0.0 : 1.0;
        aa.lr_final = r[1] == -INFINITY ? 0.0 : 1.0;
    }
    if constexpr (ES) {
        aa.es_state += (size_t)f * (2 + 2 * aa.es_window);
        if (aa.es_host_flag) aa.es_host_flag += f;
        if (aa.es_state[1] != 0) return;
    }
    sksloop::adam_block_begin(aa, s_xyz, s_d, s_it);
    const bool split = ga.nsplit == BWD_SPLITS && ga.dfeat == nullptr;
    GeomBwdRaw raw;
    if (split && wv < V) geom_bwd_issue16(ga, vb + wv, lane, raw);
    __syncthreads();
    if (tid == 0) sksloop::adam_step_sizes(aa, s_d, s_hyp);
    for (int v = wv; v < V; v += 4) {
        const int vg = vb + v;
        float gs[NACC];
        double pS, pN;
        if (split) {
            if (v != wv) geom_bwd_issue16(ga, vg, lane, raw);
            geom_bwd_sum16(ga, lane, raw, gs, pS, pN);
        } else {
            geom_bwd_load(ga, vg, lane, gs, pS, pN);
        }
        pS = wave_sum_d(pS);
        pN = wave_sum_d(pN);
        const double S = ga.gt_totals[2 * vg] + pS, n_view = ga.gt_totals[2 * vg + 1] + pN;
        if (lane == 0) { ga.loss_sums[2 * vg] = S; ga.loss_sums[2 * vg + 1] = n_view; }
        if (lane < ga.P) geom_bwd_finish(ga, vt, vg, lane, gs, n_view);
    }
    __syncthreads();
    if constexpr (ES) {
        __shared__ unsigned long long s_mask;
        __shared__ int s_cut[3];
        if (tid == 0)
            sksloop::early_stop_decide(aa, aa.es_state, aa.es_host_flag, s_xyz,
                                       [&](int v) { return (const double*)ga.loss_sums + 2 * (size_t)(vb + v); }, &s_mask, s_cut);
        __syncthreads();
        aa.group_mask = s_mask; aa.last_view = s_cut[0];
        if (s_cut[1] != aa.acc_steps) {
            aa.acc_steps = s_cut[1];
            sksloop::adam_block_begin(aa, s_xyz, s_d, s_it);
            __syncthreads();
            if (tid == 0) sksloop::adam_step_sizes(aa, s_d, s_hyp);
        }
    }
    const sksloop::AdamLdsParams mirror{ s_np, s_np + 3 * P, s_np + 6 * P, s_np + 10 * P };
    sksloop::adam_block_finish(aa, s_xyz, s_hyp, s_d, s_it, &mirror, true);
    __syncthreads();
    for (int v = wv; v < V; v += 4)
        geom_fwd_one(P, vt, ga.vms, ga.pms, mirror.xyz, mirror.opacity, mirror.scaling, mirror.rotation, nullptr,
                     ga.smod, ga.flags, g, radii, vb + v, lane, lane < P);
}
```

skelsplat_amd/csrc/sks_raster.hip:

```cpp
#include <hip/hip_runtime.h>
#include <hip/hip_ext.h>
#include <stdarg.h>
#include <stdlib.h>
#include <stdio.h>
#include <string.h>
#include <type_traits>

#include "../../include/skelsplat_hip.h"
#include "sks_math.h"
#include "sks_loop_dev.h"

using namespace sks;

namespace {

#include "sks_common.inc"
#include "sks_geom_fwd.inc"
#include "sks_fwd_small.inc"
#include "sks_bwd_small.inc"
#include "sks_geom_bwd.inc"
#include "sks_binned.inc"

inline int pick_cg(int C) { return C <= 4 ? 4 : C <= 16 ? 16 : C <= 20 ? 20 : 32; }

int check_common(int V, int P, int C, int W, int H)
{
    if (V < 1 || V > SKS_MAX_VIEWS) return fail(-1, "V=%d out of range [1,%d]", V, SKS_MAX_VIEWS);
    if (P < 0) return fail(-1, "P=%d negative", P);
    if (C < 1 || C > SKS_MAX_CHANNELS) return fail(-1, "C=%d out of range [1,%d]", C, SKS_MAX_CHANNELS);
    if (W < 1 || H < 1 || W > 4096 * TILE || H > 65535 * TILE) return fail(-1, "image %dx%d out of range", W, H);
    return 0;
}

inline bool fill_half_mode(const FwdArgs& a) { return a.W % 4 == 2 && a.H % 2 == 0 && !(a.flags & SKS_NO_NT_STORES); }

inline void fill_geometry(const FwdArgs& a, bool have_cover, bool binned, int& fsplit, int& pb)
{
    const int ppt = (a.W % 4 == 0 || fill_half_mode(a)) ? 4 : 1;
    const bool lines = (((uintptr_t)a.out_color | (uintptr_t)a.out_invdepth) & 127u) == 0;
    const int lead = (lines && (long long)a.H * a.W % 32 == 0 && TILE * a.W % 32 == 0) ? 0 : 31;
    const int passes = (TILE * a.W + lead + 256 * ppt - 1) / (256 * ppt);
    const int tune = (int)((a.flags >> 8) & 0xff);
    const int chunks = (a.W + 1023) / 1024;
    const bool rowmode = ((ppt == 4 && a.W % 4 == 0 && have_cover && a.W % 32 == 0 && (long long)a.W * 10 >= (long long)chunks * 1024 * 9) ||
                          (ppt == 4 && a.W % 4 == 0 && have_cover && (a.flags & SKS_FILL_ROWS))) && !(a.flags & SKS_FILL_LINEAR);
    if (rowmode) {
        int pbr = tune;
        if (pbr <= 0) pbr = binned ? 3 : 2;
        if (pbr > TILE) pbr = TILE;
        fsplit = chunks * ((TILE + pbr - 1) / pbr);
        pb = -pbr;
        return;
    }
    pb = tune;
    if (pb <= 0) pb = passes / 8 > 2 ? (passes + 4) / 8 : 2;
    if (pb > 32) pb = 32;
    fsplit = (passes + pb - 1) / pb;
}

template <int CG>
void launch_fwd_small(const FwdArgs& a_in, int V, int gy, int zfill, hipStream_t st, const ProfScope& prof)
{
    FwdArgs a = a_in;
    const int ncomp = a.tslots * a.P * V;
    a.ncomp = ncomp;
    int fsplit, pb;
    fill_geometry(a, a.g.cover != nullptr, false, fsplit, pb);
    if (zfill == 0) fsplit = 0;
    const int rows_zy = (zfill > 0 ? zfill : 1) * gy;
    const int xc = (ncomp + rows_zy - 1) / rows_zy;
    const int cap = (a.P + 15) & ~15;
    const size_t lds = DynList<CG>::bytes(cap, CG);
    dim3 grid(fsplit + xc, gy, zfill > 0 ? zfill : 1);
    const bool nt = !(a.flags & SKS_NO_NT_STORES);
    if (a.W % 4 == 0) {
        if (nt) SKS_LAUNCH(prof, (k_render_fwd_sparse<CG, 4, true>), grid, dim3(256), lds, st, a, a.cp1_magic, gy, fsplit, pb, (const uint32_t*)a.g.cover);
        else SKS_LAUNCH(prof, (k_render_fwd_sparse<CG, 4, false>), grid, dim3(256), lds, st, a, a.cp1_magic, gy, fsplit, pb, (const uint32_t*)a.g.cover);
    } else if (fill_half_mode(a)) {
        SKS_LAUNCH(prof, (k_render_fwd_sparse<CG, 4, true, true>), grid, dim3(256), lds, st, a, a.cp1_magic, gy, fsplit, pb, (const uint32_t*)a.g.cover);
    } else {
        SKS_LAUNCH(prof, (k_render_fwd_sparse<CG, 1, false>), grid, dim3(256), lds, st, a, a.cp1_magic, gy, fsplit, pb, (const uint32_t*)a.g.cover);
    }
}

#ifndef SKS_EARLY_FILL_BYTES
#define SKS_EARLY_FILL_BYTES (36u << 20)
#endif
inline int early_fill_planes(unsigned flags, int planes, size_t plane_bytes)
{
    const int field = (int)((flags >> SKS_BIN_GROUPS_SHIFT) & 7u);
    if (field == 7) return planes;
    if (field) return (planes * field + 15) / 16;
    const size_t want = ((size_t)SKS_EARLY_FILL_BYTES + plane_bytes / 2) / plane_bytes;
    return (int)(want < (size_t)(planes / 4) ? want : (size_t)(planes / 4));
}

inline unsigned magic32(unsigned d) { return (unsigned)(((1ull << 32) + d - 1) / d); }

bool early_fill_cut(const FwdArgs& a_in, int V, int gy, int gplanes, int zid0, int& fsplit, int& pb)
{
    FwdArgs a = a_in;
    a.flags |= SKS_FILL_LINEAR;
    fill_geometry(a, true, false, fsplit, pb);
    const long long rows = (long long)fsplit * gy, nfill = rows * ((a.C + 1) * V - zid0);
    return fsplit >= 1 && pb >= 1 && nfill * rows < (1ll << 32) && (long long)V * gplanes + nfill < (1ll << 31);
}

void launch_geom_fill(const FwdArgs& a, int V, int gy, int gplanes, int zid0, int fsplit, int pb, const ViewTan& vt,
                      const float* viewmatrix, const float* projmatrix, const float* means3D, const float* opacities,
                      const float* scales, const float* rotations, const float* cov3D_precomp, float smod, int* radii,
                      hipStream_t st, ProfScope& prof)
{
    const long long rows = (long long)fsplit * gy, nfill = rows * ((a.C + 1) * V - zid0);
    const int ngeom = V * gplanes;
    const EarlyFill f{ a.out_color, a.out_invdepth, a.C, a.W, a.H, gy, gplanes, ngeom, zid0, fsplit, pb, a.cp1_magic,
                       rows > 1 ? magic32((unsigned)rows) : 0u, fsplit > 1 ? magic32((unsigned)fsplit) : 0u };
    const dim3 grid((unsigned)(ngeom + nfill));
    const size_t lds = (size_t)gy * cover_cw(a.W) * 4;
    const bool nt = !(a.flags & SKS_NO_NT_STORES);
    const int ppt = (a.W % 4 == 0 || fill_half_mode(a)) ? 4 : 1;
#define SKS_GF_ARGS f, a.P, vt, viewmatrix, projmatrix, means3D, opacities, scales, rotations, cov3D_precomp, smod, a.flags, a.g, radii, a.features, a.cover_planes
    if (ppt == 4 && nt) SKS_LAUNCH_FIRST(prof, (k_geom_fwd_fill<4, true>), grid, dim3(256), lds, st, SKS_GF_ARGS);
    else if (ppt == 4) SKS_LAUNCH_FIRST(prof, (k_geom_fwd_fill<4, false>), grid, dim3(256), lds, st, SKS_GF_ARGS);
    else SKS_LAUNCH_FIRST(prof, (k_geom_fwd_fill<1, false>), grid, dim3(256), lds, st, SKS_GF_ARGS);
#undef SKS_GF_ARGS
}

template <int CG>
void launch_fwd_binned(const FwdArgs& a, const BinView& bv, int V, int gx, int gy, const uint32_t* cover, hipStream_t st)
{
    int fsplit, pb;
    fill_geometry(a, true, true, fsplit, pb);
    const int xc = ((gx + TGROUP - 1) / TGROUP + a.C) / (a.C + 1);
    dim3 grid(fsplit + xc, gy, (a.C + 1) * V);
    const bool nt = !(a.flags & SKS_NO_NT_STORES);
    if (a.W % 4 == 0) {
        if (nt) hipLaunchKernelGGL((k_render_fwd_binned<CG, 4, true>), grid, dim3(256), 0, st, a, bv, gx, gy, fsplit, pb, cover);
        else hipLaunchKernelGGL((k_render_fwd_binned<CG, 4, false>), grid, dim3(256), 0, st, a, bv, gx, gy, fsplit, pb, cover);
    } else if (fill_half_mode(a)) {
        hipLaunchKernelGGL((k_render_fwd_binned<CG, 4, true, true>), grid, dim3(256), 0, st, a, bv, gx, gy, fsplit, pb, cover);
    } else {
        hipLaunchKernelGGL((k_render_fwd_binned<CG, 1, false>), grid, dim3(256), 0, st, a, bv, gx, gy, fsplit, pb, cover);
    }
}

inline int bwd_tile_blocks()
{
    static const int n = [] {
        int dev = 0, cus = 256;
        if (hipGetDevice(&dev) == hipSuccess) {
            hipDeviceProp_t pr;
            if (hipGetDeviceProperties(&pr, dev) == hipSuccess && pr.multiProcessorCount > 0) cus = pr.multiProcessorCount;
        }
        const char* e = getenv("SKS_BWD_TILE_BLOCKS");
        return (e && atoi(e) > 0) ? atoi(e) : cus * BWD_TILE_BLOCKS_PER_CU;
    }();
    return n;
}

inline int bwd_wave_groups(int V, int P, unsigned flags)
{
    unsigned t = (flags >> SKS_BWD_WG_SHIFT) & 7u;
    static const int env = [] { const char* e = getenv("SKS_BWD_WG"); return e ? atoi(e) : 0; }();
    if (!t && env > 0) t = (unsigned)env;
    if (t) return t > 5 ? 1 : (BWD_SPLITS >> (t - 1));
    const int pairs = V * P;
    return pairs <= BWD_WG_PAIRS16 ? 16 : (pairs <= BWD_WG_PAIRS8 ? 8 : 4);
}

template <bool ES = false>
inline void launch_bwd_loss(const BwdArgs& a, const ViewTan& vt, const ViewOff& vo, dim3 grid, int cg, hipStream_t st)
{
    if (a.hm_row) {
        switch (cg) {
            case 4: hipLaunchKernelGGL((k_render_bwd_wave<4, false, true, true, ES>), grid, dim3(256), 0, st, a, vt, vo); break;
            case 16: hipLaunchKernelGGL((k_render_bwd_wave<16, false, true, true, ES>), grid, dim3(256), 0, st, a, vt, vo); break;
            case 20: hipLaunchKernelGGL((k_render_bwd_wave<20, false, true, true, ES>), grid, dim3(256), 0, st, a, vt, vo); break;
            default: hipLaunchKernelGGL((k_render_bwd_wave<32, false, true, true, ES>), grid, dim3(256), 0, st, a, vt, vo); break;
        }
        return;
    }
    switch (cg) {
        case 4: hipLaunchKernelGGL((k_render_bwd_wave<4, false, true, false, ES>), grid, dim3(256), 0, st, a, vt, vo); break;
        case 16: hipLaunchKernelGGL((k_render_bwd_wave<16, false, true, false, ES>), grid, dim3(256), 0, st, a, vt, vo); break;
        case 20: hipLaunchKernelGGL((k_render_bwd_wave<20, false, true, false, ES>), grid, dim3(256), 0, st, a, vt, vo); break;
        default: hipLaunchKernelGGL((k_render_bwd_wave<32, false, true, false, ES>), grid, dim3(256), 0, st, a, vt, vo); break;
    }
}

template <int CG>
void launch_bwd_small(const BwdArgs& a, const ViewTan& vt, const ViewOff& vo, int V, int gy, bool dfeat, hipStream_t st,
                      const ProfScope& prof)
{
    (void)gy;
    if (a.P <= 64 && !(a.flags & (1u << 20))) {
        dim3 grid(a.P, V, bwd_wave_groups(V, a.P, a.flags));
        if (dfeat) SKS_LAUNCH(prof, (k_render_bwd_wave<CG, true, false>), grid, dim3(256), 0, st, a, vt, vo);
        else SKS_LAUNCH(prof, (k_render_bwd_wave<CG, false, false>), grid, dim3(256), 0, st, a, vt, vo);
        return;
    }
    dim3 grid(a.P, V, BWD_SPLITS);
    const size_t lds = GatherLds<CG>::bytes((a.P + 15) & ~15, CG, a.C);
    if (lds > 48 * 1024) {
        (void)hipFuncSetAttribute(reinterpret_cast<const void*>(&k_render_bwd_gather<CG, true>),
                                  hipFuncAttributeMaxDynamicSharedMemorySize, (int)lds);
        (void)hipFuncSetAttribute(reinterpret_cast<const void*>(&k_render_bwd_gather<CG, false>),
                                  hipFuncAttributeMaxDynamicSharedMemorySize, (int)lds);
    }
    if (dfeat) SKS_LAUNCH(prof, (k_render_bwd_gather<CG, true>), grid, dim3(256), lds, st, a);
    else SKS_LAUNCH(prof, (k_render_bwd_gather<CG, false>), grid, dim3(256), lds, st, a);
}

__global__ void k_spin_us(unsigned long long ticks)
{
    const unsigned long long t0 = wall_clock64();
    while (wall_clock64() - t0 < ticks) __builtin_amdgcn_s_sleep(8);
}

struct FwdHook {
    hipEvent_t geom_done;
    int (*after_geom)(void* ctx);
    int (*after_group)(void* ctx, int g, int v0, int nv);
    void* ctx;
};
constexpr int FB_MAX_EVENTS = BIN_MAX_GROUPS;
constexpr int FB_OVERLAP_MAX_PAIRS = BWD_WG_PAIRS16;
struct FbEvents {
    hipEvent_t geom = nullptr, done = nullptr;
    hipEvent_t grp[FB_MAX_EVENTS] = {};
    int dev = -1;
};
thread_local FbEvents tl_fb_events;
int fb_events(int ngroups, FbEvents*& out)
{
    FbEvents& ev = tl_fb_events;
    int cur_dev = 0;
    HIP_TRY(hipGetDevice(&cur_dev));
    if (ev.geom && ev.dev != cur_dev) {
        (void)hipEventDestroy(ev.geom);
        (void)hipEventDestroy(ev.done);
        for (hipEvent_t& e : ev.grp)
            if (e) { (void)hipEventDestroy(e); e = nullptr; }
        ev.geom = ev.done = nullptr;
    }
    unsigned evf = hipEventDisableTiming | hipEventDisableSystemFence;
    if (const char* e = getenv("SKS_FB_EVENT_FLAGS")) evf = (unsigned)strtoul(e, nullptr, 0);
    if (!ev.geom) {
        ev.dev = cur_dev;
        HIP_TRY(hipEventCreateWithFlags(&ev.geom, evf));
        HIP_TRY(hipEventCreateWithFlags(&ev.done, evf));
    }
    for (int gi = 0; gi < ngroups && gi < FB_MAX_EVENTS; gi++)
        if (!ev.grp[gi]) HIP_TRY(hipEventCreateWithFlags(&ev.grp[gi], evf));
    out = &ev;
    return 0;
}

}

#ifndef SKS_GEOM_BINNED_THREADS
#define SKS_GEOM_BINNED_THREADS 256
#endif

extern "C" {

const char* sks_last_error(void) { return g_err; }
void sks_set_error_(const char* msg)
{
    snprintf(g_err, sizeof(g_err), "%s", msg);
}
int sks_version(void) { return 14; }

int sks_scratch_bytes(int V, int P, int C, int W, int H, size_t bin_capacity, size_t* geom, size_t* binning, size_t* accum)
{
    if (int rc = check_common(V, P, C, W, H)) return rc;
    const int NT = ((W + TILE - 1) / TILE) * ((H + TILE - 1) / TILE);
    if (geom) *geom = geom_bytes(V, P > 0 ? P : 1, W, H, C);
    if (binning) *binning = bin_bytes(V, P, NT, bin_capacity, C + 1, (size_t)((H + TILE - 1) / TILE) * cover_cw(W));
    if (accum) *accum = (size_t)V * (P > 0 ? P : 1) * BWD_SPLITS * (NACC + C) * sizeof(float);
    return 0;
}

}

namespace {

int forward_impl(int V, int P, int C, int W, int H, const float* viewmatrix, const float* projmatrix,
                 const float* tanfovx, const float* tanfovy, const float* means3D, const float* features,
                 const float* opacities, const float* scales, const float* rotations, const float* cov3D_precomp,
                 float scale_modifier, unsigned flags, float* out_color, float* out_invdepth, int* radii, void* geom,
                 void* binning, size_t bin_capacity, int* num_rendered_dev, float* final_T, uint32_t* n_contrib,
                 void* stream, const FwdHook* hook)
{
    if (int rc = check_common(V, P, C, W, H)) return rc;
    hipStream_t st = (hipStream_t)stream;
    if (!out_color || !out_invdepth) return fail(-2, "out_color / out_invdepth must be provided");
    if (((uintptr_t)out_color | (uintptr_t)out_invdepth) & 15u)
        return fail(-2, "out_color / out_invdepth must be 16-byte aligned (the planes are written with 16-byte stores)");
    const size_t HW = (size_t)H * W;
    if (P == 0) {
        HIP_TRY(hipMemsetAsync(out_color, 0, (size_t)V * C * HW * 4, st));
        HIP_TRY(hipMemsetAsync(out_invdepth, 0, (size_t)V * HW * 4, st));
        if (final_T) return fail(-2, "final_T not available for P == 0");
        return 0;
    }
    if (!viewmatrix || !projmatrix || !tanfovx || !tanfovy || !means3D || !features || !opacities || !radii || !geom)
        return fail(-2, "missing required pointer");
    if (!cov3D_precomp && (!scales || !rotations)) return fail(-2, "need scales+rotations or cov3D_precomp");
    ViewTan vt;
    ViewOff vo;
    fill_views(vt, &vo, V, C, W, H, tanfovx, tanfovy, nullptr, nullptr);
    Geom g = geom_from(geom, V, P, W, H);
    const int gx = (W + TILE - 1) / TILE, gy = (H + TILE - 1) / TILE, NT = gx * gy;

    const bool small = P <= SKS_SMALL_P && !(flags & SKS_FORCE_BINNED);
    Bin b{};
    if (!small) {
        if (!binning) return fail(-2, "binned path needs a binning buffer");
        if (bin_capacity < 1) return fail(-1, "binned path needs bin_capacity >= 1");
        b = bin_from(binning, V, P, NT, bin_capacity);
    }
    if (!small) g.cover = nullptr;
    const int gthreads = small ? 256 : SKS_GEOM_BINNED_THREADS;
    const int gplanes = (small && g.cover && cover_per_plane(P, W, H, C)) ? C + 1 : 1;
    FwdArgs a{ P, C, W, H, flags, g, features, out_color, out_invdepth, final_T, n_contrib, composite_slots(flags, V, P),
               ((1u << 20) + (unsigned)C) / (unsigned)(C + 1), 0, (!small || (g.cover && cover_per_plane(P, W, H, C))) ? 1 : 0,
               (W >= 2 && W < 16384) ? (unsigned)(((1ull << 32) + (unsigned)W - 1) / (unsigned)W) : 0u };
    const int cg = pick_cg(C);
    const int planes = (C + 1) * V;
    int early = 0;
    if (small && !hook && g.cover && !final_T && !n_contrib && !(flags & (SKS_DEBUG_SYNC | SKS_NO_EARLY_FILL)))
        early = early_fill_planes(flags, planes, HW * 4);
    int efs = 0, epb = 0;
    if (early > 0 && early_fill_cut(a, V, gy, gplanes, planes - early, efs, epb)) {
        ProfScope prof(0, st, true);
        launch_geom_fill(a, V, gy, gplanes, planes - early, efs, epb, vt, viewmatrix, projmatrix, means3D, opacities, scales, rotations,
                         cov3D_precomp, scale_modifier, radii, st, prof);
        switch (cg) {
            case 4: launch_fwd_small<4>(a, V, gy, planes - early, st, prof); break;
            case 16: launch_fwd_small<16>(a, V, gy, planes - early, st, prof); break;
            case 20: launch_fwd_small<20>(a, V, gy, planes - early, st, prof); break;
            default: launch_fwd_small<32>(a, V, gy, planes - early, st, prof); break;
        }
        HIP_TRY(hipGetLastError());
        return 0;
    }
    if (hook && small && hook->geom_done)
        hipExtLaunchKernelGGL(k_geom_fwd, dim3((P + gthreads - 1) / gthreads, V, gplanes), dim3(gthreads), 0, st, nullptr, hook->geom_done, 0,
                              P, W, H, vt, viewmatrix, projmatrix, means3D, opacities, scales, rotations, cov3D_precomp, scale_modifier,
                              flags, g, radii, 0, (uint32_t*)nullptr, (uint32_t*)nullptr, features, C, (uint2*)nullptr, (uint32_t*)nullptr,
                              cover_per_plane(P, W, H, C) ? 1 : 0);
    else
    hipLaunchKernelGGL(k_geom_fwd, dim3((P + gthreads - 1) / gthreads, V, gplanes), dim3(gthreads), 0, st, P, W, H, vt, viewmatrix, projmatrix,
                       means3D, opacities, scales, rotations, cov3D_precomp, scale_modifier, flags, g, radii, 0,
                       small ? (uint32_t*)nullptr : b.count, small ? (uint32_t*)nullptr : b.touched, features, C,
                       small ? (uint2*)nullptr : b.fmask, small ? (uint32_t*)nullptr : b.hdr, (small && cover_per_plane(P, W, H, C)) ? 1 : 0);
    STAGE_CHECK("geometry");
    if (hook && small && hook->after_geom) {
        if (int rc = hook->after_geom(hook->ctx)) return rc;
    }

    if (small) {
        {
            ProfScope prof(0, st, true);
            switch (cg) {
                case 4: launch_fwd_small<4>(a, V, gy, planes, st, prof); break;
                case 16: launch_fwd_small<16>(a, V, gy, planes, st, prof); break;
                case 20: launch_fwd_small<20>(a, V, gy, planes, st, prof); break;
                default: launch_fwd_small<32>(a, V, gy, planes, st, prof); break;
            }
        }
        STAGE_CHECK("render(small)");
        return 0;
    }
    uint32_t* cover = b.coverp;
    const int cw = cover_cw(W);
    hipLaunchKernelGGL(k_bin_band_count, dim3(gy, V), dim3(BAND_TC), (size_t)2 * gx * 4, st, P, gx, g, b);
    int vg, ng;
    bin_groups(flags, V, vg, ng);
    {
        const int bpc = gx >= SCAN_T * 8 ? 1 : (SCAN_T * 8) / gx;
        const int nchunk_t = (gy + bpc - 1) / bpc, nchunk_g = (P + SCAN_G - 1) / SCAN_G;
        hipLaunchKernelGGL(k_bin_scan, dim3(nchunk_t + nchunk_g, V), dim3(SCAN_T), (size_t)bpc * cw * 4, st, P, gx, gy, cw, bpc,
                           nchunk_t, bin_capacity, b, cover, num_rendered_dev, V, C + 1, vg);
    }
    hipLaunchKernelGGL(k_bin_band_scatter, dim3(gy, V), dim3(BAND_TS), (size_t)2 * gx * 4, st, P, gx, bin_capacity, g, b, C, cw);
    STAGE_CHECK("binning");
    const BinView bv_all = bin_view(b, NT, bin_capacity);
    {
        ProfScope prof(0, st);
        for (int gi = 0; gi < ng; gi++) {
            const int v0 = gi * vg, nv = (V - v0 < vg) ? V - v0 : vg;
            FwdArgs ag = a;
            ag.out_color = a.out_color + (size_t)v0 * C * HW;
            ag.out_invdepth = a.out_invdepth + (size_t)v0 * HW;
            if (a.final_T) ag.final_T = a.final_T + (size_t)v0 * HW;
            if (a.n_contrib) ag.n_contrib = a.n_contrib + (size_t)v0 * HW;
            BinView bv = bv_all;
            bv.ranges += (size_t)v0 * NT;
            bv.tidx += (size_t)v0 * NT;
            bv.aux += (size_t)v0 * NT * TILE * TILE;
            bv.e_co += (size_t)v0 * bin_capacity;
            bv.e_xyd += (size_t)v0 * bin_capacity;
            bv.e_ids += (size_t)v0 * bin_capacity;
            bv.part += (size_t)v0 * bin_capacity * BIN_ROWS * NACC;
            const uint32_t* cov_g = cover + (size_t)v0 * (C + 1) * gy * cw;
            switch (cg) {
                case 4: launch_fwd_binned<4>(ag, bv, nv, gx, gy, cov_g, st); break;
                case 16: launch_fwd_binned<16>(ag, bv, nv, gx, gy, cov_g, st); break;
                case 20: launch_fwd_binned<20>(ag, bv, nv, gx, gy, cov_g, st); break;
                default: launch_fwd_binned<32>(ag, bv, nv, gx, gy, cov_g, st); break;
            }
            if (hook && hook->after_group)
                if (int rc = hook->after_group(hook->ctx, gi, v0, nv)) return rc;
        }
    }
    STAGE_CHECK("render(binned)");
    return 0;
}

}

extern "C" {

int sks_forward(int V, int P, int C, int W, int H, const float* viewmatrix, const float* projmatrix,
                const float* tanfovx, const float* tanfovy, const float* means3D, const float* features,
                const float* opacities, const float* scales, const float* rotations, const float* cov3D_precomp,
                float scale_modifier, unsigned flags, float* out_color, float* out_invdepth, int* radii, void* geom,
                void* binning, size_t bin_capacity, int* num_rendered_dev, float* final_T, uint32_t* n_contrib,
                void* stream)
{
    return forward_impl(V, P, C, W, H, viewmatrix, projmatrix, tanfovx, tanfovy, means3D, features, opacities, scales, rotations,
                        cov3D_precomp, scale_modifier, flags, out_color, out_invdepth, radii, geom, binning, bin_capacity,
                        num_rendered_dev, final_T, n_contrib, stream, nullptr);
}

}

namespace {

constexpr unsigned BWD_RENDER = 1u, BWD_GEOM = 2u;
int backward_impl(int V, int P, int C, int W, int H, const float* viewmatrix, const float* projmatrix,
                  const float* tanfovx, const float* tanfovy, const float* bg, const float* means3D,
                  const float* features, const float* opacities, const float* scales, const float* rotations,
                  const float* cov3D_precomp, float scale_modifier, unsigned flags, const int* radii, const void* geom,
                  const void* binning, size_t bin_capacity, const float* dL_dout_color, const float* dL_dout_invdepth,
                  void* accum, float* dL_dmeans3D, float* dL_dmeans2D, float* dL_dopacity, float* dL_dscales,
                  float* dL_drotations, float* dL_dcov3D, float* dL_dfeatures, float* dL_dmeans3D_mean, void* stream,
                  unsigned phases, int group)
{
    if (int rc = check_common(V, P, C, W, H)) return rc;
    if (P == 0) return 0;
    hipStream_t st = (hipStream_t)stream;
    if (!viewmatrix || !projmatrix || !tanfovx || !tanfovy || !means3D || !features || !opacities || !radii ||
        !geom || !dL_dout_color || !accum || !dL_dmeans3D || !dL_dmeans2D || !dL_dopacity)
        return fail(-2, "missing required pointer");
    if (!cov3D_precomp && (!scales || !rotations)) return fail(-2, "need scales+rotations or cov3D_precomp");
    ViewTan vt;
    ViewOff vo;
    fill_views(vt, &vo, V, C, W, H, tanfovx, tanfovy, nullptr, nullptr);
    Geom g = geom_from(const_cast<void*>(geom), V, P, W, H);
    const int gx = (W + TILE - 1) / TILE, gy = (H + TILE - 1) / TILE, NT = gx * gy;
    BwdArgs a{ P, C, W, H, flags, g, features, bg, dL_dout_color, dL_dout_invdepth, (float*)accum, nullptr, nullptr };
    const int cg = pick_cg(C);
    const bool dfeat = dL_dfeatures != nullptr;
    const bool small = P <= SKS_SMALL_P && !(flags & SKS_FORCE_BINNED);
    int vg = V, ng = 1;
    if (!small) bin_groups(flags, V, vg, ng);
    if (group >= ng) return fail(-1, "view group %d of %d", group, ng);
    if ((phases & BWD_RENDER) && small) {
        ProfScope prof(1, st, true);
        switch (cg) {
            case 4: launch_bwd_small<4>(a, vt, vo, V, gy, dfeat, st, prof); break;
            case 16: launch_bwd_small<16>(a, vt, vo, V, gy, dfeat, st, prof); break;
            case 20: launch_bwd_small<20>(a, vt, vo, V, gy, dfeat, st, prof); break;
            default: launch_bwd_small<32>(a, vt, vo, V, gy, dfeat, st, prof); break;
        }
        STAGE_CHECK("render-backward(small)");
    } else if (phases & BWD_RENDER) {
        if (!binning) return fail(-2, "binned path needs the forward's binning buffer");
        Bin b = bin_from(const_cast<void*>(binning), V, P, NT, bin_capacity);
        BinView bv = bin_view(b, NT, bin_capacity);
        if (dfeat && group <= 0) HIP_TRY(hipMemsetAsync(accum, 0, (size_t)V * P * (NACC + C) * sizeof(float), st));
        dim3 grid(bwd_tile_blocks());
        const unsigned magic_nt = (unsigned)(((1ull << 32) + (unsigned)NT - 1) / (unsigned)NT), magic_gx = (unsigned)(((1ull << 32) + (unsigned)gx - 1) / (unsigned)gx);
        const bool extra = bg != nullptr || dL_dout_invdepth != nullptr;
        for (int gi = group < 0 ? 0 : group; gi < (group < 0 ? ng : group + 1); gi++) {
            const uint4* tl = b.tlist + (size_t)gi * vg * NT;
            const uint32_t* hd = b.hdr + gi * BIN_CLASSES;
            ProfScope prof(1, st);
            if (dfeat) hipLaunchKernelGGL((k_render_bwd_tile<true, true>), grid, dim3(BWD_TILE_THREADS), 0, st, a, bv, gx, V, magic_nt, magic_gx, tl, hd);
            else if (extra) hipLaunchKernelGGL((k_render_bwd_tile<false, true>), grid, dim3(BWD_TILE_THREADS), 0, st, a, bv, gx, V, magic_nt, magic_gx, tl, hd);
            else hipLaunchKernelGGL((k_render_bwd_tile<false, false>), grid, dim3(BWD_TILE_THREADS), 0, st, a, bv, gx, V, magic_nt, magic_gx, tl, hd);
        }
        STAGE_CHECK("render-backward(binned)");
    }
    if (!(phases & BWD_GEOM)) return 0;
    GeomBwdArgs ga{ P, C, W, H, flags, viewmatrix, projmatrix, means3D, opacities, scales, rotations, cov3D_precomp,
                    scale_modifier, radii, (const float*)accum, small ? BWD_SPLITS : 0, nullptr, nullptr, nullptr, dL_dmeans3D, dL_dmeans2D, dL_dopacity, dL_dscales,
                    dL_drotations, dL_dcov3D, dL_dfeatures };
    if (!small) {
        Bin b = bin_from(const_cast<void*>(binning), V, P, NT, bin_capacity);
        ga.rect = g.rect;
        ga.goff = b.goff;
        ga.part = b.part;
        ga.cap = bin_capacity;
        ga.bin_hdr = b.hdr;
    }
    if (dL_dmeans3D_mean && V * P <= 256 && small) {
        hipLaunchKernelGGL(k_geom_bwd_all, dim3(1), dim3(256), 0, st, ga, vt, V, dL_dmeans3D_mean);
    } else {
        if (small) hipLaunchKernelGGL(k_geom_bwd, dim3((P + 255) / 256, V), dim3(256), 0, st, ga, vt);
        else {
            const int v0 = group < 0 ? 0 : group * vg, nv = group < 0 ? V : ((V - v0 < vg) ? V - v0 : vg);
            ga.v0 = v0;
            hipLaunchKernelGGL(k_geom_bwd_binned, dim3((P + GEOMB_G - 1) / GEOMB_G, nv), dim3(256), 0, st, ga, vt);
        }
        if (dL_dmeans3D_mean && (small || group < 0 || group == ng - 1))
            hipLaunchKernelGGL(k_mean_views, dim3((3 * P + 255) / 256), dim3(256), 0, st, V, P, dL_dmeans3D, dL_dmeans3D_mean);
    }
    STAGE_CHECK("geometry-backward");
    return 0;
}

}

extern "C" {

int sks_backward(int V, int P, int C, int W, int H, const float* viewmatrix, const float* projmatrix,
                 const float* tanfovx, const float* tanfovy, const float* bg, const float* means3D,
                 const float* features, const float* opacities, const float* scales, const float* rotations,
                 const float* cov3D_precomp, float scale_modifier, unsigned flags, const int* radii, const void* geom,
                 const void* binning, size_t bin_capacity, const float* dL_dout_color, const float* dL_dout_invdepth,
                 void* accum, float* dL_dmeans3D, float* dL_dmeans2D, float* dL_dopacity, float* dL_dscales,
                 float* dL_drotations, float* dL_dcov3D, float* dL_dfeatures, float* dL_dmeans3D_mean, void* stream)
{
    return backward_impl(V, P, C, W, H, viewmatrix, projmatrix, tanfovx, tanfovy, bg, means3D, features, opacities, scales, rotations,
                         cov3D_precomp, scale_modifier, flags, radii, geom, binning, bin_capacity, dL_dout_color, dL_dout_invdepth, accum,
                         dL_dmeans3D, dL_dmeans2D, dL_dopacity, dL_dscales, dL_drotations, dL_dcov3D, dL_dfeatures, dL_dmeans3D_mean,
                         stream, BWD_RENDER | BWD_GEOM, -1);
}

int sks_forward_backward(int V, int P, int C, int W, int H, const float* viewmatrix, const float* projmatrix,
                         const float* tanfovx, const float* tanfovy, const float* means3D, const float* features,
                         const float* opacities, const float* scales, const float* rotations, const float* cov3D_precomp,
                         float scale_modifier, unsigned flags, float* out_color, float* out_invdepth, int* radii, void* geom,
                         void* binning, size_t bin_capacity, int* num_rendered_dev, const float* bg,
                         const float* dL_dout_color, const float* dL_dout_invdepth, void* accum, float* dL_dmeans3D,
                         float* dL_dmeans2D, float* dL_dopacity, float* dL_dscales, float* dL_drotations, float* dL_dcov3D,
                         float* dL_dfeatures, float* dL_dmeans3D_mean, void* stream, void* aux_stream, unsigned fb_flags)
{
    const bool small = P <= SKS_SMALL_P && !(flags & SKS_FORCE_BINNED);
    int vg = V, ng = 1;
    if (!small && V >= 1) bin_groups(flags, V, vg, ng);
    struct Ctx {
        int V, P, C, W, H;
        const float *vm, *pm, *tx, *ty, *bg, *means, *feat, *opac, *scales, *rots, *cov;
        float smod;
        unsigned flags;
        const int* radii;
        const void *geom, *binning;
        size_t cap;
        const float *dL, *dLinv;
        void* accum;
        float *m3, *m2, *op, *sc, *rot, *dcov, *dfeat, *mean;
        hipStream_t s, aux;
        bool ext, handed;
        int rc_aux;
        int backward(unsigned phases, int group) const
        {
            return backward_impl(V, P, C, W, H, vm, pm, tx, ty, bg, means, feat, opac, scales, rots, cov, smod, flags, radii, geom, binning, cap,
                                 dL, dLinv, accum, m3, m2, op, sc, rot, dcov, dfeat, mean, aux, phases, group);
        }
    } c{ V, P, C, W, H, viewmatrix, projmatrix, tanfovx, tanfovy, bg, means3D, features, opacities, scales, rotations, cov3D_precomp,
         scale_modifier, flags, radii, geom, binning, bin_capacity, dL_dout_color, dL_dout_invdepth, accum, dL_dmeans3D, dL_dmeans2D,
         dL_dopacity, dL_dscales, dL_drotations, dL_dcov3D, dL_dfeatures, dL_dmeans3D_mean, (hipStream_t)stream, (hipStream_t)aux_stream,
         true, false, 0 };
    {
        static const bool ext_off = [] { const char* e = getenv("SKS_FB_EXT"); return e && atoi(e) == 0; }();
        if (ext_off) c.ext = false;
    }
    const bool no_join = (fb_flags & SKS_FB_NO_JOIN) != 0;
    const bool crowded = small && (long long)V * P > FB_OVERLAP_MAX_PAIRS && !no_join;
    if (!aux_stream || aux_stream == stream || P == 0 || (flags & SKS_DEBUG_SYNC) || (!small && ng < 2) || crowded) {
        if (int rc = forward_impl(V, P, C, W, H, viewmatrix, projmatrix, tanfovx, tanfovy, means3D, features, opacities, scales, rotations,
                                  cov3D_precomp, scale_modifier, flags | SKS_NO_EARLY_FILL, out_color, out_invdepth, radii, geom, binning, bin_capacity,
                                  num_rendered_dev, nullptr, nullptr, stream, nullptr))
            return rc;
        if (int rc = backward_impl(V, P, C, W, H, viewmatrix, projmatrix, tanfovx, tanfovy, bg, means3D, features, opacities, scales,
                                   rotations, cov3D_precomp, scale_modifier, flags, radii, geom, binning, bin_capacity, dL_dout_color,
                                   dL_dout_invdepth, accum, dL_dmeans3D, dL_dmeans2D, dL_dopacity, dL_dscales, dL_drotations, dL_dcov3D,
                                   dL_dfeatures, dL_dmeans3D_mean, stream, BWD_RENDER | BWD_GEOM, -1))
            return rc;
        if (no_join && aux_stream && aux_stream != stream) {
            FbEvents* ev = nullptr;
            if (int rc = fb_events(0, ev)) return rc;
            HIP_TRY(hipEventRecord(ev->done, (hipStream_t)stream));
            HIP_TRY(hipStreamWaitEvent((hipStream_t)aux_stream, ev->done, 0));
        }
        return 0;
    }
    FbEvents* evp = nullptr;
    if (int rc = fb_events(small ? 0 : ng, evp)) return rc;
    FbEvents& ev = *evp;
    struct Run {
        static int after_geom(void* p)
        {
            Ctx& k = *(Ctx*)p;
            FbEvents& e = tl_fb_events;
            if (!k.ext) HIP_TRY(hipEventRecord(e.geom, k.s));
            HIP_TRY(hipStreamWaitEvent(k.aux, e.geom, 0));
            k.handed = true;
            return k.rc_aux = k.backward(BWD_RENDER | BWD_GEOM, -1);
        }
        static int after_group(void* p, int g, int, int)
        {
            Ctx& k = *(Ctx*)p;
            FbEvents& e = tl_fb_events;
            HIP_TRY(hipEventRecord(e.grp[g], k.s));
            HIP_TRY(hipStreamWaitEvent(k.aux, e.grp[g], 0));
            k.handed = true;
            return k.rc_aux = k.backward(BWD_RENDER | BWD_GEOM, g);
        }
    };
    const FwdHook hook{ (small && c.ext) ? ev.geom : nullptr, small ? &Run::after_geom : nullptr, small ? nullptr : &Run::after_group, &c };
    int rc = forward_impl(V, P, C, W, H, viewmatrix, projmatrix, tanfovx, tanfovy, means3D, features, opacities, scales, rotations,
                          cov3D_precomp, scale_modifier, flags, out_color, out_invdepth, radii, geom, binning, bin_capacity,
                          num_rendered_dev, nullptr, nullptr, stream, &hook);
    if (rc == 0 && !c.handed) rc = fail(-3, "sks_forward_backward: the forward did not reach the point the backward starts from");
    if (c.handed && (!no_join || rc != 0)) {
        const hipError_t e1 = hipEventRecord(ev.done, c.aux);
        const hipError_t e2 = e1 == hipSuccess ? hipStreamWaitEvent(c.s, ev.done, 0) : e1;
        if (rc == 0 && e2 != hipSuccess) rc = fail((int)e2, "sks_forward_backward: joining the two streams: %s", hipGetErrorString(e2));
    }
    return rc;
}

int sks_mean_views(int V, int P, const float* dL_dmeans3D, int shard_world, float* mean_out, void* stream)
{
    if (V < 1 || P < 1 || shard_world < 1) return fail(-1, "mean_views: bad shape");
    if (!dL_dmeans3D || !mean_out) return fail(-2, "mean_views: missing pointer");
    hipLaunchKernelGGL(k_mean_views, dim3((3 * P + 255) / 256), dim3(256), 0, (hipStream_t)stream, V, P, dL_dmeans3D, mean_out,
                       shard_world);
    HIP_TRY(hipGetLastError());
    return 0;
}

int sks_gt_tile_stats(int V, int C, int W, int H, const float* gt, float* tile_S, float* tile_N, double* totals, void* stream)
{
    if (int rc = check_common(V, 1, C, W, H)) return rc;
    if (!gt || !totals) return fail(-2, "gt_tile_stats: missing pointer");
    hipStream_t st = (hipStream_t)stream;
    HIP_TRY(hipMemsetAsync(totals, 0, (size_t)V * 2 * sizeof(double), st));
    dim3 grid((H + TILE - 1) / TILE, C, V);
    hipLaunchKernelGGL(k_gt_tile_stats, grid, dim3(256), 0, st, C, W, H, gt, tile_S, tile_N, totals);
    HIP_TRY(hipGetLastError());
    return 0;
}

int sks_backward_fused_loss(int V, int P, int C, int W, int H, const float* viewmatrix, const float* projmatrix,
                            const float* tanfovx, const float* tanfovy, const float* bg, const float* means3D,
                            const float* features, const float* opacities, const float* scales, const float* rotations,
                            const float* cov3D_precomp, float scale_modifier, unsigned flags, const int* radii,
                            const void* geom, const float* gt, const float* tile_S, const float* tile_N,
                            const double* gt_totals, void* accum, float* dL_dmeans3D, float* dL_dmeans2D,
                            float* dL_dopacity, float* dL_dscales, float* dL_drotations, float* dL_dcov3D,
                            double* loss_sums, float* packed_raw_grads, const int* view_wh, const size_t* gt_offsets,
                            const float* const* hm_factors, void* stream)
{
    if (int rc = check_common(V, P, C, W, H)) return rc;
    if (P < 1 || P > 64) return fail(-1, "fused-loss backward needs 1 <= P <= 64 (got %d)", P);
    hipStream_t st = (hipStream_t)stream;
    if (!viewmatrix || !projmatrix || !tanfovx || !tanfovy || !means3D || !features || !opacities || !radii || !geom ||
        (!gt && !hm_factors) || !gt_totals || !accum || !dL_dmeans3D || !dL_dmeans2D || !dL_dopacity || !loss_sums)
        return fail(-2, "missing required pointer");
    if (hm_factors && (!hm_factors[0] || !hm_factors[1] || !hm_factors[2] || !hm_factors[3]))
        return fail(-2, "hm_factors: row, col, cmin, den must all be given");
    if (!cov3D_precomp && (!scales || !rotations)) return fail(-2, "need scales+rotations or cov3D_precomp");
    ViewTan vt;
    ViewOff vo;
    if (!fill_views(vt, &vo, V, C, W, H, tanfovx, tanfovy, view_wh, gt_offsets))
        return fail(-1, "view_wh: every view's size must be within [1, W] x [1, H] (pass the largest as W, H)");
    if (!hm_factors && (view_wh != nullptr) != (gt_offsets != nullptr)) return fail(-2, "view_wh and gt_offsets go together");
    Geom g = geom_from(const_cast<void*>(geom), V, P, W, H);
    BwdArgs a{ P, C, W, H, flags | SKS_CLAMP01, g, features, bg, gt, nullptr, (float*)accum, tile_S, tile_N };
    if (hm_factors) { a.hm_row = hm_factors[0]; a.hm_col = hm_factors[1]; a.hm_cmin = hm_factors[2]; a.hm_den = hm_factors[3]; }
    dim3 grid(P, V, bwd_wave_groups(V, P, flags));
    {
        ProfScope prof(1, st);
        launch_bwd_loss(a, vt, vo, grid, pick_cg(C), st);
    }
    STAGE_CHECK("fused loss + render-backward");
    GeomBwdArgs ga{ P, C, W, H, flags, viewmatrix, projmatrix, means3D, opacities, scales, rotations, cov3D_precomp,
// ... 56 lines not shown
                                float* xyz, float* scaling, float* rotation, float* opacity, float* exp_avg, float* exp_avg_sq,
                                int* counters, int acc_steps, const double* lr_sched, const double* lrs, const double* adam,
                                float lambda_consistency, const int* limb, const int* view_wh, const size_t* gt_offsets,
                                int frames, const float* const* hm_factors, int* es_state, int es_window, float es_tolerance,
                                int* es_host_flags, void* stream, const void* views_dev = nullptr,
                                const double* lr_sched_dev = nullptr)
{
    if (int rc = check_common(V, P, C, W, H)) return rc;
    if (P < 1 || P > 64) return fail(-1, "fused step needs 1 <= P <= 64 (got %d)", P);
    static const float no_tan[SKS_MAX_VIEWS] = {};
    static const double no_sched[5] = { 1.0, 1.0, 1.0, 0.0, 1.0 };
    if (views_dev) { tanfovx = tanfovy = no_tan; lr_sched = no_sched; }
    if (frames < 1 || V % frames) return fail(-1, "frames must divide the number of views (V = %d, frames = %d)", V, frames);
    const int Vf = V / frames;
    if (!viewmatrix || !projmatrix || !tanfovx || !tanfovy || !features || !radii || !geom || (!gt && !hm_factors) || !gt_totals ||
        !accum || !loss_sums || !packed)
        return fail(-2, "missing required pointer");
    if (hm_factors && (!hm_factors[0] || !hm_factors[1] || !hm_factors[2] || !hm_factors[3]))
        return fail(-2, "hm_factors: row, col, cmin, den must all be given");
    hipStream_t st = (hipStream_t)stream;
    ViewTan vt;
    ViewOff vo;
    if (!fill_views(vt, &vo, V, C, W, H, tanfovx, tanfovy, view_wh, gt_offsets))
        return fail(-1, "view_wh: every view's size must be within [1, W] x [1, H] (pass the largest as W, H)");
    if (!hm_factors && (view_wh != nullptr) != (gt_offsets != nullptr)) return fail(-2, "view_wh and gt_offsets go together");
    flags |= SKS_RAW_PARAMS | SKS_CLAMP01;
    sksloop::AdamArgs aa;
    if (const char* err = sksloop::fill_adam_args(aa, Vf, P, packed, slots, group_mask, last_view, xyz, scaling, rotation, opacity,
                                                  exp_avg, exp_avg_sq, counters, acc_steps, lr_sched, lrs, adam,
                                                  lambda_consistency, limb))
        return fail(-2, "%s", err);
    const bool es = es_state != nullptr;
    if (es) { aa.es_state = es_state; aa.es_window = es_window; aa.es_tol = es_tolerance; aa.es_host_flag = es_host_flags; }
    Geom g = geom_from(geom, V, P, W, H);
    g.cover = nullptr;
    BwdArgs a{ P, C, W, H, flags, g, features, nullptr, gt, nullptr, (float*)accum, nullptr, nullptr };
    if (hm_factors) { a.hm_row = hm_factors[0]; a.hm_col = hm_factors[1]; a.hm_cmin = hm_factors[2]; a.hm_den = hm_factors[3]; }
    if (es) { a.es_stop = es_state + 1; a.es_stride = 2 + 2 * es_window; a.es_views = Vf; }
    dim3 grid(P, V, bwd_wave_groups(V, P, flags));
    {
        ProfScope prof(1, st);
        if (es) launch_bwd_loss<true>(a, vt, vo, grid, pick_cg(C), st);
        else launch_bwd_loss(a, vt, vo, grid, pick_cg(C), st);
    }
    STAGE_CHECK("render-backward(fused loss)");
    GeomBwdArgs ga{ P, C, W, H, flags, viewmatrix, projmatrix, xyz, opacity, scaling, rotation, nullptr, scale_modifier, radii,
                    (const float*)accum, BWD_SPLITS, gt_totals, loss_sums, packed, nullptr, nullptr, nullptr, nullptr, nullptr,
                    nullptr, nullptr };
    if (views_dev) {
        const ViewTanDev vd = views_dev_from(views_dev, lr_sched_dev);
        if (es) hipLaunchKernelGGL((k_step_tail<true, ViewTanDev>), dim3(frames), dim3(256), 0, st, ga, vd, aa, Vf, g, radii);
        else hipLaunchKernelGGL((k_step_tail<false, ViewTanDev>), dim3(frames), dim3(256), 0, st, ga, vd, aa, Vf, g, radii);
    } else if (es) hipLaunchKernelGGL(k_step_tail<true>, dim3(frames), dim3(256), 0, st, ga, vt, aa, Vf, g, radii);
    else hipLaunchKernelGGL(k_step_tail<false>, dim3(frames), dim3(256), 0, st, ga, vt, aa, Vf, g, radii);
    STAGE_CHECK("step tail");
    return 0;
}

int sks_loop_fused_step(int V, int P, int C, int W, int H, const float* viewmatrix, const float* projmatrix,
                        const float* tanfovx, const float* tanfovy, const float* features, float scale_modifier,
                        unsigned flags, int* radii, void* geom, const float* gt, const double* gt_totals, void* accum,
                        double* loss_sums, float* packed, float* slots, unsigned long long group_mask, int last_view,
                        float* xyz, float* scaling, float* rotation, float* opacity, float* exp_avg, float* exp_avg_sq,
                        int* counters, int acc_steps, const double* lr_sched, const double* lrs, const double* adam,
                        float lambda_consistency, const int* limb, const int* view_wh, const size_t* gt_offsets, int frames,
                        const float* const* hm_factors, void* stream)
{
    return loop_fused_step_impl(V, P, C, W, H, viewmatrix, projmatrix, tanfovx, tanfovy, features, scale_modifier, flags, radii,
                                geom, gt, gt_totals, accum, loss_sums, packed, slots, group_mask, last_view, xyz, scaling,
                                rotation, opacity, exp_avg, exp_avg_sq, counters, acc_steps, lr_sched, lrs, adam,
                                lambda_consistency, limb, view_wh, gt_offsets, frames, hm_factors, nullptr, 0, 0.0f, nullptr,
                                stream);
}

int sks_loop_fused_step_es(int V, int P, int C, int W, int H, const float* viewmatrix, const float* projmatrix,
                           const float* tanfovx, const float* tanfovy, const float* features, float scale_modifier,
                           unsigned flags, int* radii, void* geom, const float* gt, const double* gt_totals, void* accum,
                           double* loss_sums, float* packed, float* slots, unsigned long long group_mask, int last_view,
                           float* xyz, float* scaling, float* rotation, float* opacity, float* exp_avg, float* exp_avg_sq,
                           int* counters, int acc_steps, const double* lr_sched, const double* lrs, const double* adam,
                           float lambda_consistency, const int* limb, const int* view_wh, const size_t* gt_offsets, int frames,
                           const float* const* hm_factors, int* es_state, int es_window, float es_tolerance,
                           int* es_host_flags, void* stream)
{
    if (!es_state)
        return fail(-2, "loop_fused_step_es: es_state is required (sks_loop_fused_step is the step without a criterion)");
    if (es_window < 1 || es_window > sksloop::ES_MAX_WINDOW)
        return fail(-1, "loop_fused_step_es: window %d out of range [1, %d]", es_window, sksloop::ES_MAX_WINDOW);
    return loop_fused_step_impl(V, P, C, W, H, viewmatrix, projmatrix, tanfovx, tanfovy, features, scale_modifier, flags, radii,
                                geom, gt, gt_totals, accum, loss_sums, packed, slots, group_mask, last_view, xyz, scaling,
                                rotation, opacity, exp_avg, exp_avg_sq, counters, acc_steps, lr_sched, lrs, adam,
                                lambda_consistency, limb, view_wh, gt_offsets, frames, hm_factors, es_state, es_window,
                                es_tolerance, es_host_flags, stream);
}

int sks_loop_fused_step_dv(int V, int P, int C, int W, int H, const float* viewmatrix, const float* projmatrix,
                           const void* views_dev, const float* features, float scale_modifier, unsigned flags, int* radii,
                           void* geom, const float* gt, const double* gt_totals, void* accum, double* loss_sums, float* packed,
                           float* slots, unsigned long long group_mask, int last_view, float* xyz, float* scaling,
                           float* rotation, float* opacity, float* exp_avg, float* exp_avg_sq, int* counters, int acc_steps,
                           const double* lr_sched_dev, const double* lrs, const double* adam, float lambda_consistency,
                           const int* limb, const int* view_wh, const size_t* gt_offsets, int frames,
                           const float* const* hm_factors, void* stream)
{
    if (!views_dev || !lr_sched_dev) return fail(-2, "loop_fused_step_dv: views_dev and lr_sched_dev are required");
    return loop_fused_step_impl(V, P, C, W, H, viewmatrix, projmatrix, nullptr, nullptr, features, scale_modifier, flags, radii,
                                geom, gt, gt_totals, accum, loss_sums, packed, slots, group_mask, last_view, xyz, scaling,
                                rotation, opacity, exp_avg, exp_avg_sq, counters, acc_steps, nullptr, lrs, adam,
                                lambda_consistency, limb, view_wh, gt_offsets, frames, hm_factors, nullptr, 0, 0.0f, nullptr,
                                stream, views_dev, lr_sched_dev);
}

int sks_loop_fused_step_es_dv(int V, int P, int C, int W, int H, const float* viewmatrix, const float* projmatrix,
                              const void* views_dev, const float* features, float scale_modifier, unsigned flags, int* radii,
                              void* geom, const float* gt, const double* gt_totals, void* accum, double* loss_sums,
                              float* packed, float* slots, unsigned long long group_mask, int last_view, float* xyz,
                              float* scaling, float* rotation, float* opacity, float* exp_avg, float* exp_avg_sq, int* counters,
                              int acc_steps, const double* lr_sched_dev, const double* lrs, const double* adam,
                              float lambda_consistency, const int* limb, const int* view_wh, const size_t* gt_offsets,
                              int frames, const float* const* hm_factors, int* es_state, int es_window, float es_tolerance,
                              int* es_host_flags, void* stream)
{
    if (!views_dev || !lr_sched_dev) return fail(-2, "loop_fused_step_es_dv: views_dev and lr_sched_dev are required");
    if (!es_state)
        return fail(-2, "loop_fused_step_es_dv: es_state is required (sks_loop_fused_step_dv is the step without a criterion)");
    if (es_window < 1 || es_window > sksloop::ES_MAX_WINDOW)
        return fail(-1, "loop_fused_step_es_dv: window %d out of range [1, %d]", es_window, sksloop::ES_MAX_WINDOW);
    return loop_fused_step_impl(V, P, C, W, H, viewmatrix, projmatrix, nullptr, nullptr, features, scale_modifier, flags, radii,
                                geom, gt, gt_totals, accum, loss_sums, packed, slots, group_mask, last_view, xyz, scaling,
                                rotation, opacity, exp_avg, exp_avg_sq, counters, acc_steps, nullptr, lrs, adam,
                                lambda_consistency, limb, view_wh, gt_offsets, frames, hm_factors, es_state, es_window,
                                es_tolerance, es_host_flags, stream, views_dev, lr_sched_dev);
}

int sks_prof_spin(double microseconds, void* stream)
{
    if (!(microseconds >= 0.0) || microseconds > 1e6) return fail(-1, "prof_spin: 0 .. 1e6 us");
    hipLaunchKernelGGL(k_spin_us, dim3(1), dim3(64), 0, (hipStream_t)stream, (unsigned long long)(microseconds * 100.0));
    HIP_TRY(hipGetLastError());
    return 0;
}

int sks_prof_enable(int on)
{
    if (!tl_prof) {
        if (!on) return 0;
        tl_prof = new ProfState();
    }
    tl_prof->on = on != 0;
    tl_prof->every = (on & 0xffff) > 1 ? (on & 0xffff) : 1;
    tl_prof->skip = (on >> 16) & 3;
    tl_prof->recorded = (on >> 18) & 1;
    tl_prof->seen[0] = tl_prof->seen[1] = 0;
    return 0;
}

int sks_prof_count(int kind, long long* launches)
{
    if (kind < 0 || kind > 1 || !launches) return fail(-2, "bad profile query");
    *launches = tl_prof ? tl_prof->kind[kind].n : 0;
    return 0;
}

int sks_prof_read(int kind, double* total_ms, long long* launches)
{
    if (kind < 0 || kind > 1 || !total_ms || !launches) return fail(-2, "bad profile query");
    if (!tl_prof) { *total_ms = 0.0; *launches = 0; return 0; }
    ProfKind& p = tl_prof->kind[kind];
    double tot = 0;
    for (int i = 0; i < p.n; i++) {
        HIP_TRY(hipEventSynchronize(p.e[i]));
        float ms = 0;
        HIP_TRY(hipEventElapsedTime(&ms, p.b[i], p.e[i]));
        tot += ms;
    }
    *total_ms = tot;
    *launches = p.n;
    p.n = 0;
    return 0;
}

int sks_prof_read_quantiles(int kind, double* q_ms , double* total_ms, long long* launches)
{
    if (kind < 0 || kind > 1 || !q_ms || !total_ms || !launches) return fail(-2, "bad profile query");
    if (!tl_prof) { q_ms[0] = q_ms[1] = q_ms[2] = 0.0; *total_ms = 0.0; *launches = 0; return 0; }
    ProfKind& p = tl_prof->kind[kind];
    static thread_local float t[PROF_MAX];
    double tot = 0;
    for (int i = 0; i < p.n; i++) {
        HIP_TRY(hipEventSynchronize(p.e[i]));
        HIP_TRY(hipEventElapsedTime(&t[i], p.b[i], p.e[i]));
        tot += t[i];
    }
    const int n = p.n;
    for (int i = 1; i < n; i++) {
        const float v = t[i];
        int j = i - 1;
        for (; j >= 0 && t[j] > v; j--) t[j + 1] = t[j];
        t[j + 1] = v;
    }
    q_ms[0] = n ? t[(int)(0.1 * (n - 1) + 0.5)] : 0.0;
    q_ms[1] = n ? t[(n - 1) / 2] : 0.0;
    q_ms[2] = n ? t[(int)(0.9 * (n - 1) + 0.5)] : 0.0;
    *total_ms = tot;
    *launches = n;
    p.n = 0;
    return 0;
}

int sks_mark_visible(int P, const float* means3D, const float* viewmatrix, const float* projmatrix, uint8_t* present,
                     void* stream)
{
    (void)projmatrix;
    if (P < 0) return fail(-1, "P negative");
    if (P == 0) return 0;
    if (!means3D || !viewmatrix || !present) return fail(-2, "missing required pointer");
    hipLaunchKernelGGL(k_mark_visible, dim3((P + 255) / 256), dim3(256), 0, (hipStream_t)stream, P, means3D, viewmatrix, present);
    HIP_TRY(hipGetLastError());
    return 0;
}

int sks_export_lists(int V, int W, int H, const void* binning, size_t bin_capacity, uint32_t* point_list,
                     uint32_t* ranges, void* stream)
{
    if (!binning || !point_list || !ranges) return fail(-2, "missing required pointer");
    const int NT = ((W + TILE - 1) / TILE) * ((H + TILE - 1) / TILE);
    Bin b = bin_from(const_cast<void*>(binning), V, 1, NT, bin_capacity);
    const size_t m = bin_capacity > (size_t)NT ? bin_capacity : (size_t)NT;
    hipLaunchKernelGGL(k_export_lists, dim3((unsigned)((m + 255) / 256), V), dim3(256), 0, (hipStream_t)stream, NT,
                       bin_capacity, b.ranges, b.nrend, point_list, ranges);
    hipLaunchKernelGGL(k_export_sorted, dim3((NT + 3) / 4, V), dim3(256), 0, (hipStream_t)stream, bin_view(b, NT, bin_capacity),
                       point_list);
    HIP_TRY(hipGetLastError());
    return 0;
}

}
```

skelsplat_amd/rasterizer.py:

```python
from collections import namedtuple
from typing import NamedTuple, Optional

import operator
import os

import torch
import torch.nn as nn

from . import _arena, _lib
from ._arena import _BIN_CAP_HINT, _BIN_CAP_SEEN, _BIN_PROBE
from ._base import (ForwardState, ViewBatch, _accum, _bg_channels, _f32c, _f32c_params, _fresh, _grad_dict,
                    _need_gpu, _scratch_bytes_cached, reset_scratch)
from ._tuning import (PLAIN_STORES, TUNE_CANDIDATES, TUNE_CANDIDATES_FRESH, TUNE_CANDIDATES_WITH_PLAIN, TUNE_WARM,
                      _FILL_BITS, _FILL_TUNE, _FILL_TUNE_LOG, _MEASURING, _pick, _time_candidates, _tune_flag_bits, fill_tuning,
                      tune_name)
from .sparse import (GtStats, HeatmapFactors, HeatmapSet, backward_fused_loss, geometry_views, gt_tile_stats,
                     loop_fused_step)

_ENV_TUNE = int(os.environ.get("SKS_FWD_TUNE", "0"), 0)
AUTOTUNE = os.environ.get("SKS_AUTOTUNE", "1") != "0"


class GaussianRasterizationSettings(NamedTuple):
    image_height: int
    image_width: int
    tanfovx: float
    tanfovy: float
    bg: torch.Tensor
    scale_modifier: float
    viewmatrix: torch.Tensor
    projmatrix: torch.Tensor
    sh_degree: int
    campos: torch.Tensor
    prefiltered: bool
    debug: bool
    antialiasing: bool


class Workspace:

    def __init__(self):
        self._t = {}
        self._plans = {}
        self._aux = {}
        self._pending_join = None

    def aux_stream(self, dev_index):
        st = self._aux.get(dev_index)
        if st is None:
            st = self._aux[dev_index] = torch.cuda.Stream(device=dev_index)
        return st

    def join(self, dev_index):
        torch.cuda.current_stream(dev_index).wait_stream(self.aux_stream(dev_index))
        self._pending_join = None

    def tune(self, step_fn, candidates=None, reps=8, rounds=3, confirm=True):
        plan = self._plans.get("fwd")
        if plan is None or torch.cuda.is_current_stream_capturing():
            return None, {}
        candidates = TUNE_CANDIDATES if candidates is None else candidates
        args, dev_index = plan.args, plan.dev_index
        base = args[_F_FLAGS] & ~_FILL_BITS

        def set_bits(bits):
            args[_F_FLAGS] = base | bits
        times = _time_candidates(set_bits, step_fn, candidates, reps, rounds, dev_index)
        best, med = _pick(times, candidates, set_bits, step_fn, reps, dev_index, confirm)
        set_bits(_tune_flag_bits(best))
        key = (dev_index, *(args[_lib.FWD[n]] for n in ("V", "P", "C", "W", "H")), "workspace")
        _FILL_TUNE[key] = _tune_flag_bits(best)
        _FILL_TUNE_LOG[key] = {tune_name(c): round(v, 2) for c, v in med.items()}
        return best, med

    def settle(self):
        if self._pending_join is not None:
            self.join(self._pending_join)

    def get(self, name, shape, dtype, device):
        key = (name, tuple(shape), dtype, device)
        t = self._t.get(key)
        if t is None:
            t = torch.empty(shape, dtype=dtype, device=device)
            self._t[key] = t
        return t


def _sig(t):
    if t is None or t.numel() == 0:
        return None
    if t.dtype is not torch.float32 or not t.is_cuda or not t.is_contiguous():
        return False
    return (t.data_ptr(), t.shape)


_FwdRecord = namedtuple("_FwdRecord", "key keep args dev_index result arena")
_BwdRecord = namedtuple("_BwdRecord", "key keep args dev_index result")
_Block = namedtuple("_Block", "args dev_index dev shape")

_F_V, _F_FLAGS, _F_COLOR, _F_INVDEPTH, _F_RADII, _F_GEOM, _F_NUM_RENDERED = (
    _lib.FWD[n] for n in ("V", "flags", "out_color", "out_invdepth", "radii", "geom", "num_rendered_dev"))
_B_RADII, _B_GEOM, _B_DL_COLOR, _B_DL_INVDEPTH = (_lib.BWD[n] for n in ("radii", "geom", "dL_dout_color", "dL_dout_invdepth"))
_GRAD_SLOTS = tuple((k, _lib.BWD[n]) for k, n in (
    ("means3D", "dL_dmeans3D"), ("means2D", "dL_dmeans2D"), ("opacities", "dL_dopacity"), ("scales", "dL_dscales"),
    ("rotations", "dL_drotations"), ("cov3D", "dL_dcov3D"), ("features", "dL_dfeatures")))
_FB_STREAM, _FB_AUX_STREAM, _FB_FLAGS = (_lib.FWD_BWD[n] for n in ("stream", "aux_stream", "fb_flags"))
_FB_GATHER = operator.itemgetter(*(_lib.FWD["stream"] if src is None else src[1] + (len(_lib.FWD) if src[0] == "bwd" else 0)
                                   for src in _lib.FWD_BWD_SOURCES))


def _replay(fn, args, dev_index, stream_slot=-1):
    args[stream_slot] = torch._C._cuda_getCurrentRawStream(dev_index)
    if torch._C._cuda_getDevice() == dev_index:
        return fn(*args)
    with torch.cuda.device(dev_index):
        return fn(*args)


def forward_views(views: ViewBatch, means3D, features, opacities, scales, rotations, cov3D_precomp,
                  scale_modifier=1.0, antialiasing=False, clamp01=False, debug=False, force_binned=False,
                  bin_capacity=None, want_aux=False, tune_flags=0, check_capacity=True, workspace=None, plans=None):
    lib = _lib.load()
    key = None
    if features is not None and features.numel() and means3D is not None and means3D.dim() == 2 and means3D.shape[0] \
            and features.numel() // means3D.shape[0] > _lib.SKS_MAX_CHANNELS:
        return _forward_views_wide(views, means3D, features, opacities, scales, rotations, cov3D_precomp, scale_modifier, antialiasing,
                                   clamp01, debug, force_binned, bin_capacity, want_aux, tune_flags, check_capacity)
    if not want_aux and (workspace is not None or plans is not None):
        key = _fwd_key(views, means3D, features, opacities, scales, rotations, cov3D_precomp, scale_modifier, antialiasing,
                       clamp01, debug, force_binned, bin_capacity, tune_flags, check_capacity)
    if key is not None and workspace is None:
        hit = plans.get(key)
        if hit is not None:
            args_t, dev_index, dev, (V, P, C, H, W, gbytes, flags) = hit
            color = torch.empty((V, C, H, W), dtype=torch.float32, device=dev)
            invdepth = torch.empty((V, 1, H, W), dtype=torch.float32, device=dev)
            radii = torch.empty((V, P), dtype=torch.int32, device=dev)
            geom = torch.empty((gbytes,), dtype=torch.uint8, device=dev)
            args = list(args_t)
            args[_F_COLOR], args[_F_INVDEPTH], args[_F_RADII], args[_F_GEOM] = color.data_ptr(), invdepth.data_ptr(), radii.data_ptr(), geom.data_ptr()
            _lib.check(_replay(lib.sks_forward, args, dev_index), "sks_forward")
            st = ForwardState(views, P, C, flags, scale_modifier, radii, geom)
            st.plan_key = key
            return color, invdepth, radii, st
    if workspace is not None:
        workspace.settle()
    if key is not None and workspace is not None:
        plan = workspace._plans.get("fwd")
        if plan is not None and plan.key == key:
            ticket = _replay_ticket(workspace, plan)
            rc = _replay(lib.sks_forward, plan.args, plan.dev_index)
            if rc != 0:
                del workspace._plans["fwd"]
            _lib.check(rc, "sks_forward")
            if ticket is None or (_arena.finish(ticket) or 0) <= ticket.cap:
                return plan.result
            del workspace._plans["fwd"]
    if views.mixed:
        raise RuntimeError("the dense forward writes one (V,C,H,W) tensor: all views of the batch must share the image size")
    if means3D is None or means3D.dim() != 2 or means3D.shape[1] != 3:
        raise RuntimeError("means3D must have dimensions (num_points, 3)")
    _need_gpu(means3D, "means3D")
    if means3D.shape[0] == 0:
        dev, V, W, H = means3D.device, views.V, views.W, views.H
        C = int(features.shape[-1])
        st = ForwardState(views, 0, C, 0, scale_modifier, torch.zeros((V, 0), dtype=torch.int32, device=dev))
        out = (torch.zeros((V, C, H, W), device=dev), torch.zeros((V, 1, H, W), device=dev), st.radii, st)
        if want_aux:
            out += (torch.ones((V, H, W), device=dev), torch.zeros((V, H, W), dtype=torch.int32, device=dev))
        return out
    means3D, features, opacities, scales, rotations, cov3D_precomp = _f32c_params(means3D, features, opacities, scales, rotations, cov3D_precomp)
    dev = means3D.device
    P = means3D.shape[0]
    feat2 = features.reshape(P, -1)
    C = feat2.shape[1]
    V, W, H = views.V, views.W, views.H
    flags = (_lib.SKS_ANTIALIASING if antialiasing else 0) | (_lib.SKS_CLAMP01 if clamp01 else 0) | \
            (_lib.SKS_DEBUG_SYNC if debug else 0) | (_lib.SKS_FORCE_BINNED if force_binned else 0) | int(tune_flags) | _ENV_TUNE
    if plans is not None and workspace is None and AUTOTUNE and not flags & _FILL_BITS and not _MEASURING[0] and not force_binned \
            and (dev.index, V, P, C, W, H, "fresh") not in _FILL_TUNE:
        tune_forward(views, means3D, feat2, opacities, scales, rotations, cov3D_precomp, scale_modifier, antialiasing, clamp01,
                     tune_flags=tune_flags)
    if not flags & _FILL_BITS and not _MEASURING[0]:
        flags |= _FILL_TUNE.get((dev.index, V, P, C, W, H, "workspace" if workspace is not None else "fresh"), 0)
    binned = force_binned or P > _lib.SKS_SMALL_P
    ticket = _arena.begin((dev.index, V, P, C, W, H), bin_capacity, check_capacity, torch.cuda.is_current_stream_capturing()) if binned else None
    cap = ticket.cap if binned else int(bin_capacity or 0)
    gbytes, bbytes, _ = _scratch_bytes_cached(V, max(P, 1), C, W, H, cap)
    def new(name, shape, dtype):
        if workspace is None:
            return torch.empty(shape, dtype=dtype, device=dev)
        return workspace.get(("fwd", name), shape, dtype, dev)

    color = new("color", (V, C, H, W), torch.float32)
    invdepth = new("invdepth", (V, 1, H, W), torch.float32)
    radii = new("radii", (V, P), torch.int32)
    geom = new("geom", (gbytes,), torch.uint8)
    binning = new("binning", (bbytes,), torch.uint8) if binned else None
    nrend = None if not binned else new("nrend", (V + 1,), torch.int32) if ticket.device else ticket.host
    final_T = torch.empty((V, H, W), dtype=torch.float32, device=dev) if want_aux else None
    n_contrib = torch.empty((V, H, W), dtype=torch.int32, device=dev) if want_aux else None
    args = [V, P, C, W, H, views.viewmatrix.data_ptr(), views.projmatrix.data_ptr(), views.tanfovx,
            views.tanfovy, _lib.ptr(means3D), _lib.ptr(feat2), _lib.ptr(opacities), _lib.ptr(scales),
            _lib.ptr(rotations), _lib.ptr(cov3D_precomp), float(scale_modifier), flags,
            color.data_ptr(), invdepth.data_ptr(), _lib.ptr(radii), geom.data_ptr(),
            _lib.ptr(binning), cap, _lib.ptr(nrend), _lib.ptr(final_T), _lib.ptr(n_contrib), None]
    _lib.check(_replay(lib.sks_forward, args, dev.index), "sks_forward")
    if binned:
        need = _arena.finish(ticket, nrend)
        if need is not None and need > cap:
            return forward_views(views, means3D, features, opacities, scales, rotations, cov3D_precomp, scale_modifier,
                                 antialiasing, clamp01, debug, force_binned, _arena.grown(need), want_aux, tune_flags,
                                 check_capacity, workspace)
    st = ForwardState(views, P, C, flags, scale_modifier, radii, geom, binning, cap, nrend)
    if want_aux:
        return color, invdepth, radii, st, final_T, n_contrib
    if key is None or not _recordable(key):
        return color, invdepth, radii, st
    if workspace is None:
        if not binned and P:
            if len(plans) > 64:
                plans.clear()
            plans[key] = _Block(list(args), dev.index, dev, (V, P, C, H, W, gbytes, flags))
            plans[("keep", key)] = (views, means3D, feat2, opacities, scales, rotations, cov3D_precomp)
            st.plan_key = key
    elif not torch.cuda.is_current_stream_capturing():
        keep = (means3D, feat2, opacities, scales, rotations, cov3D_precomp)
        arena = (ticket.key, cap, True if check_capacity is True else "lazy") if binned and check_capacity else None
        workspace._plans["fwd"] = _FwdRecord(key, (views, keep), args, dev.index, (color, invdepth, radii, st), arena)
    return color, invdepth, radii, st


def _replay_ticket(workspace, plan):
    if plan.arena is None:
        return None
    try:
        ticket = _arena.begin(*plan.arena, torch.cuda.is_current_stream_capturing())
    except RuntimeError:
        workspace._plans.pop("fwd", None)
        raise
    plan.args[_F_NUM_RENDERED] = _lib.ptr(ticket.host)
    plan.result[3].num_rendered_dev = ticket.host
    return ticket


def _forward_views_wide(views, means3D, features, opacities, scales, rotations, cov3D_precomp, scale_modifier, antialiasing, clamp01,
                        debug, force_binned, bin_capacity, want_aux, tune_flags, check_capacity):
    if want_aux:
        raise RuntimeError("final_T / n_contrib are not available beyond SKS_MAX_CHANNELS channels")
    if views.mixed:
        raise RuntimeError("the dense forward writes one (V,C,H,W) tensor: all views of the batch must share the image size")
    _need_gpu(means3D, "means3D")
    P = means3D.shape[0]
    feat2 = _f32c(features, "features").reshape(P, -1)
    C, V, W, H, dev = feat2.shape[1], views.V, views.W, views.H, means3D.device
    M = _lib.SKS_MAX_CHANNELS
    color = torch.empty((V, C, H, W), dtype=torch.float32, device=dev)
    invdepth = torch.empty((V, 1, H, W), dtype=torch.float32, device=dev)
    radii = torch.empty((V, P), dtype=torch.int32, device=dev)
    st = ForwardState(views, P, C, 0, scale_modifier, radii)
    st.chunks = []
    for v in range(V):
        one = ViewBatch(views.viewmatrix[v:v + 1], views.projmatrix[v:v + 1], [views.tanfovx[v]], [views.tanfovy[v]], W, H)
        for c0 in range(0, C, M):
            c1 = min(C, c0 + M)
            fc = feat2[:, c0:c1].contiguous()
            col, inv, rad, sub = forward_views(one, means3D, fc, opacities, scales, rotations, cov3D_precomp, scale_modifier,
                                               antialiasing, clamp01, debug, force_binned, bin_capacity, False, tune_flags, check_capacity)
            color[v, c0:c1].copy_(col[0])
            if c0 == 0:
                invdepth[v].copy_(inv[0])
                radii[v].copy_(rad[0])
            st.chunks.append((v, c0, c1, fc, sub))
    return color, invdepth, radii, st


def _backward_views_wide(st, means3D, opacities, scales, rotations, cov3D_precomp, dL_dcolor, dL_dinvdepth, bg, want_dfeatures,
                         tune_flags):
    dev, V, P, C = means3D.device, st.views.V, st.P, st.C
    dL_dcolor = _f32c(dL_dcolor, "dL_dout_color").reshape(V, C, st.views.H, st.views.W)
    dL_dinvdepth = _f32c(dL_dinvdepth, "dL_dout_invdepth")
    out = _grad_dict(_fresh(torch.zeros, dev), V, P, C, scales is not None and scales.numel(),
                     rotations is not None and rotations.numel(), want_dfeatures)
    bgC = _bg_channels(bg, C, dev)
    for v, c0, c1, fc, sub in st.chunks:
        g = backward_views(sub, means3D, fc, opacities, scales, rotations, cov3D_precomp, dL_dcolor[v:v + 1, c0:c1],
                           None if (dL_dinvdepth is None or c0) else dL_dinvdepth.reshape(V, 1, st.views.H, st.views.W)[v:v + 1],
                           None if bgC is None else bgC[c0:c1], want_dfeatures, tune_flags)
        for k in ("means3D", "means2D", "opacities", "cov3D", "scales", "rotations"):
            if out[k] is not None:
                out[k][v] += g[k][0]
        if want_dfeatures:
            out["features"][v, :, c0:c1] = g["features"][0]
    return out


def _fwd_key(views, means3D, features, opacities, scales, rotations, cov3D_precomp, scale_modifier, antialiasing, clamp01, debug,
             force_binned, bin_capacity, tune_flags, check_capacity):
    return (id(views), (_sig(means3D), _sig(features), _sig(opacities), _sig(scales), _sig(rotations), _sig(cov3D_precomp)),
            scale_modifier, antialiasing, clamp01, debug, force_binned, bin_capacity, tune_flags, check_capacity)


def _bwd_key(st, means3D, features, opacities, scales, rotations, cov3D_precomp, dL_dcolor, dL_dinvdepth, bg, want_dfeatures,
             tune_flags, want_mean, out_means3D, stream):
    return (id(st), (_sig(means3D), _sig(features), _sig(opacities), _sig(scales), _sig(rotations), _sig(cov3D_precomp),
                     _sig(dL_dcolor), _sig(dL_dinvdepth)), None if bg is None else (id(bg), bg._version), want_dfeatures, tune_flags,
            want_mean, None if out_means3D is None else out_means3D.data_ptr(), stream)


def _recordable(key):
    _owner, sigs, *_switches = key
    return all(sg is not False for sg in sigs)


def backward_views(st: ForwardState, means3D, features, opacities, scales, rotations, cov3D_precomp, dL_dcolor,
                   dL_dinvdepth=None, bg=None, want_dfeatures=False, tune_flags=0, workspace=None, want_mean=False,
                   out_means3D=None, plans=None):
    lib = _lib.load()
    key = pkey = None
    if st.chunks is not None:
        if want_mean or out_means3D is not None:
            raise RuntimeError("want_mean / out_means3D are not available beyond SKS_MAX_CHANNELS channels")
        return _backward_views_wide(st, means3D, opacities, scales, rotations, cov3D_precomp, dL_dcolor, dL_dinvdepth, bg,
                                    want_dfeatures, tune_flags)
    if plans is not None and workspace is None and st.plan_key is not None and out_means3D is None and not want_mean \
            and _sig(dL_dcolor) is not False and (dL_dinvdepth is None or _sig(dL_dinvdepth) is not False):
        stream = torch._C._cuda_getCurrentRawStream(st.geom.device.index)
        pkey = ("bwd", st.plan_key, dL_dcolor.shape, dL_dinvdepth is None, None if bg is None else (id(bg), bg._version),
                want_dfeatures, tune_flags, stream)
        hit = plans.get(pkey)
        if hit is not None:
            args_t, dev_index, dev, shape = hit
            out = _grad_dict(_fresh(torch.empty, dev), *shape, want_dfeatures)
            args = list(args_t)
            args[_B_RADII], args[_B_GEOM], args[_B_DL_COLOR], args[_B_DL_INVDEPTH] = \
                st.radii.data_ptr(), st.geom.data_ptr(), dL_dcolor.data_ptr(), _lib.ptr(dL_dinvdepth)
            for k, i in _GRAD_SLOTS:
                g = out[k]
                args[i] = None if g is None else g.data_ptr()
            rc = _replay(lib.sks_backward, args, dev_index)
            if rc != 0:
                reset_scratch()
                plans.pop(pkey, None)
            _lib.check(rc, "sks_backward")
            return out
    if workspace is not None:
        workspace.settle()
    if workspace is not None and st.P:
        key = _bwd_key(st, means3D, features, opacities, scales, rotations, cov3D_precomp, dL_dcolor, dL_dinvdepth, bg,
                       want_dfeatures, tune_flags, want_mean, out_means3D, torch._C._cuda_getCurrentRawStream(st.geom.device.index))
        plan = workspace._plans.get("bwd")
        if plan is not None and plan.key == key:
            rc = _replay(lib.sks_backward, plan.args, plan.dev_index)
            if rc != 0:
                reset_scratch()
                del workspace._plans["bwd"]
            _lib.check(rc, "sks_backward")
            return plan.result
    if st.P == 0:
        dev = means3D.device
        empty = _grad_dict(_fresh(torch.zeros, dev), st.views.V, 0, st.C, True, True, want_dfeatures)
        if want_mean:
            empty["means3D_mean"] = torch.zeros((0, 3), dtype=torch.float32, device=dev)
        return empty
    means3D, features, opacities, scales, rotations, cov3D_precomp = _f32c_params(means3D, features, opacities, scales, rotations, cov3D_precomp)
    dev = means3D.device
    V, P, C, W, H = st.views.V, st.P, st.C, st.views.W, st.views.H
    feat2 = features.reshape(P, -1)
    dL_dcolor, dL_dinvdepth = _f32c(dL_dcolor, "dL_dout_color"), _f32c(dL_dinvdepth, "dL_dout_invdepth")
    if dL_dcolor.numel() != V * C * H * W:
        raise RuntimeError("dL_dout_color has the wrong number of elements")
    bgC = _bg_channels(bg, C, dev)
    e = _fresh(torch.empty, dev) if workspace is None else lambda name, *s: workspace.get(("bwd", name), s, torch.float32, dev)
    out = _grad_dict(e, V, P, C, scales is not None, rotations is not None, want_dfeatures)
    if want_mean:
        out["means3D_mean"] = e("m3mean", P, 3)
    if out_means3D is not None:
        if tuple(out_means3D.shape) != (V, P, 3) or out_means3D.dtype != torch.float32 or not out_means3D.is_contiguous() \
                or out_means3D.device != dev:
            raise ValueError(f"out_means3D must be a contiguous fp32 (V,P,3) = {(V, P, 3)} tensor on {dev}")
        out["means3D"] = out_means3D
    stream = torch._C._cuda_getCurrentRawStream(dev.index)
    accum = _accum(dev, stream, V, P, C)
    args = [V, P, C, W, H, st.views.viewmatrix.data_ptr(), st.views.projmatrix.data_ptr(),
            st.views.tanfovx, st.views.tanfovy, _lib.ptr(bgC), _lib.ptr(means3D), _lib.ptr(feat2),
            _lib.ptr(opacities), _lib.ptr(scales), _lib.ptr(rotations), _lib.ptr(cov3D_precomp),
            st.scale_modifier, st.flags | int(tune_flags), _lib.ptr(st.radii), st.geom.data_ptr(), _lib.ptr(st.binning),
            st.bin_capacity, dL_dcolor.data_ptr(), _lib.ptr(dL_dinvdepth), accum.data_ptr(),
            _lib.ptr(out["means3D"]), _lib.ptr(out["means2D"]), _lib.ptr(out["opacities"]),
            _lib.ptr(out["scales"]), _lib.ptr(out["rotations"]), _lib.ptr(out["cov3D"]),
            _lib.ptr(out["features"]), _lib.ptr(out.get("means3D_mean")), None]
    rc = _replay(lib.sks_backward, args, dev.index)
    if rc != 0:
        reset_scratch()
    _lib.check(rc, "sks_backward")
    if key is not None and _recordable(key) and not torch.cuda.is_current_stream_capturing():
        keep = (st, means3D, feat2, opacities, scales, rotations, cov3D_precomp, dL_dcolor, dL_dinvdepth, bg, bgC, accum)
        workspace._plans["bwd"] = _BwdRecord(key, keep, args, dev.index, out)
    if pkey is not None and st.binning is None:
        plans[pkey] = _Block(list(args), dev.index, dev, (V, P, C, scales is not None, rotations is not None))
        plans[("keep", pkey)] = (bg, bgC, accum)
    return out


def forward_backward_views(views: ViewBatch, means3D, features, opacities, scales, rotations, cov3D_precomp, dL_dcolor,
                           dL_dinvdepth=None, bg=None, scale_modifier=1.0, antialiasing=False, clamp01=False, want_dfeatures=False,
                           tune_flags=0, workspace=None, want_mean=False, out_means3D=None, overlap=True, join=True,
                           force_binned=False, bin_capacity=None, check_capacity=True):
    if workspace is None:
        raise ValueError("forward_backward_views needs a Workspace (outputs, scratch and the second stream live there)")
    lib = _lib.load()
    workspace.settle()
    fplan, bplan = workspace._plans.get("fwd"), workspace._plans.get("bwd")
    if fplan is not None and bplan is not None:
        dev_index = fplan.dev_index
        fkey = _fwd_key(views, means3D, features, opacities, scales, rotations, cov3D_precomp, scale_modifier, antialiasing, clamp01,
                        False, force_binned, bin_capacity, tune_flags, check_capacity)
        if fplan.key == fkey:
            _color, _invdepth, _radii, st = fplan.result
            bkey = _bwd_key(st, means3D, features, opacities, scales, rotations, cov3D_precomp, dL_dcolor, dL_dinvdepth, bg,
                            want_dfeatures, tune_flags, want_mean, out_means3D, torch._C._cuda_getCurrentRawStream(dev_index))
            if bplan.key == bkey:
                aux = workspace.aux_stream(dev_index) if (overlap or not join) else None
                ticket = _replay_ticket(workspace, fplan)
                no_join = overlap and not join
                args = list(_FB_GATHER(fplan.args + bplan.args))
                args[_FB_AUX_STREAM], args[_FB_FLAGS] = aux.cuda_stream if overlap else None, _lib.SKS_FB_NO_JOIN if no_join else 0
                rc = _replay(lib.sks_forward_backward, args, dev_index, _FB_STREAM)
                if rc != 0:
                    reset_scratch()
                    workspace._plans.pop("fwd", None), workspace._plans.pop("bwd", None)
                _lib.check(rc, "sks_forward_backward")
                if no_join:
                    workspace._pending_join = dev_index
                if not join and not overlap:
                    aux.wait_stream(torch.cuda.current_stream(dev_index))
                if ticket is None or (_arena.finish(ticket) or 0) <= ticket.cap:
                    return fplan.result + (bplan.result,)
                del workspace._plans["fwd"]
                workspace.settle()
    out = forward_views(views, means3D, features, opacities, scales, rotations, cov3D_precomp, scale_modifier, antialiasing, clamp01,
                        force_binned=force_binned, bin_capacity=bin_capacity, check_capacity=check_capacity,
                        tune_flags=tune_flags, workspace=workspace)
    g = backward_views(out[3], means3D, features, opacities, scales, rotations, cov3D_precomp, dL_dcolor, dL_dinvdepth, bg,
                       want_dfeatures, tune_flags, workspace, want_mean, out_means3D)
    if not join:
        workspace.aux_stream(means3D.device.index).wait_stream(torch.cuda.current_stream(means3D.device))
    return out + (g,)


def tune_forward(views, means3D, features, opacities, scales, rotations, cov3D_precomp, scale_modifier=1.0, antialiasing=False,
                 clamp01=False, tune_flags=0, reps=6, rounds=3, rotate=4):
    P = means3D.shape[0]
    dev = means3D.device
    feat2 = features.reshape(P, -1)
    C = feat2.shape[1]
    key = (dev.index, views.V, P, C, views.W, views.H, "fresh")
    if key in _FILL_TUNE:
        return _FILL_TUNE[key]
    if torch.cuda.is_current_stream_capturing():
        return 0
    _FILL_TUNE[key] = 0
    if P == 0 or P > _lib.SKS_SMALL_P or C > _lib.SKS_MAX_CHANNELS:
        return 0
    wss = [Workspace() for _ in range(rotate)]
    state = {"bits": 0, "i": 0}

    def step():
        ws = wss[state["i"] % rotate]
        state["i"] += 1
        forward_views(views, means3D, feat2, opacities, scales, rotations, cov3D_precomp, scale_modifier, antialiasing, clamp01,
                      tune_flags=(int(tune_flags) & ~_FILL_BITS) | state["bits"], workspace=ws)

    def set_bits(bits):
        state["bits"] = bits
    _MEASURING[0] = True
    try:
        with torch.no_grad():
            times = _time_candidates(set_bits, step, TUNE_CANDIDATES_FRESH, reps, rounds, dev.index, warm=2 * rotate)
            best, med = _pick(times, TUNE_CANDIDATES_FRESH, set_bits, step, reps, dev.index)
    finally:
        _MEASURING[0] = False
    _FILL_TUNE[key] = _tune_flag_bits(best)
    _FILL_TUNE_LOG[key] = {tune_name(c): round(v, 2) for c, v in med.items()}
    return _FILL_TUNE[key]


def mean_views(grads, V, world=1, out=None):
    vmax = (V + world - 1) // world
    P = grads.shape[1]
    if grads.dtype != torch.float32 or not grads.is_contiguous() or grads.shape[0] < (V if world == 1 else world * vmax) \
            or grads.shape[2] != 3:
        raise ValueError("mean_views: grads must be a contiguous fp32 (rows,P,3) tensor with a row for every view")
    _need_gpu(grads, "grads")
    if out is None:
        out = torch.empty((P, 3), dtype=torch.float32, device=grads.device)
    rc = _lib.load().sks_mean_views(V, P, grads.data_ptr(), world, out.data_ptr(),
                                    torch._C._cuda_getCurrentRawStream(grads.device.index))
    _lib.check(rc, "sks_mean_views")
    return out


def export_lists(st: ForwardState):
    lib = _lib.load()
    if st.binning is None:
        raise RuntimeError("lists exist only on the binned path (force_binned=True)")
    dev = st.geom.device
    V, W, H = st.views.V, st.views.W, st.views.H
    NT = ((W + 15) // 16) * ((H + 15) // 16)
    pl = torch.empty((V, max(st.bin_capacity, 1)), dtype=torch.int32, device=dev)
    rg = torch.empty((V, NT, 2), dtype=torch.int32, device=dev)
    with torch.cuda.device(dev):
        rc = lib.sks_export_lists(V, W, H, st.binning.data_ptr(), st.bin_capacity, pl.data_ptr(), rg.data_ptr(),
                                  torch.cuda.current_stream(dev).cuda_stream)
    _lib.check(rc, "sks_export_lists")
    nr = rg[..., 1].amax(dim=1) if st.num_rendered_dev is None or not st.num_rendered_dev.is_cuda else st.num_rendered_dev[:V]
    return pl, rg, nr


def _features_of(sh, colors_precomp, P):
    if sh is not None and sh.numel() > 0:
        if sh.dim() == 3 and sh.shape[1] != 1:
            raise RuntimeError(f"features must have exactly one SH coefficient (M == 1), got shape {tuple(sh.shape)}")
        return sh, "sh"
    if colors_precomp is not None and colors_precomp.numel() > 0:
        return colors_precomp, "colors"
    raise RuntimeError("no features: provide shs (P,1,C) or colors_precomp (P,C)")


_AUTOGRAD_PLANS = {}
if os.environ.get("SKS_AUTOGRAD_PLANS", "1") == "0":
    _AUTOGRAD_PLANS = None


class _RasterizeViews(torch.autograd.Function):

    @staticmethod
    def forward(ctx, means3D, means2D, sh, colors_precomp, opacities, scales, rotations, cov3Ds_precomp, views,
                scale_modifier, antialiasing, clamp01, debug, bg, single, raw=False):
        P = means3D.shape[0] if means3D.dim() == 2 else 0
        feats, src = _features_of(sh, colors_precomp, P)
        tune = (_lib.SKS_RAW_PARAMS | _lib.SKS_RAW_GRADS) if raw else 0
        color, invdepth, radii, st = forward_views(views, means3D, feats, opacities, scales, rotations, cov3Ds_precomp,
                                                   scale_modifier, antialiasing, clamp01, debug, check_capacity=True,
                                                   tune_flags=tune, plans=_AUTOGRAD_PLANS)
        ctx.st, ctx.src, ctx.bg, ctx.single = st, src, bg, single
        ctx.save_for_backward(means3D, sh, colors_precomp, opacities, scales, rotations, cov3Ds_precomp)
        ctx.mark_non_differentiable(radii)
        ctx.set_materialize_grads(False)
        if single:
            return color[0], radii[0], invdepth[0]
        return color, radii, invdepth

    @staticmethod
    def backward(ctx, grad_color, _grad_radii, grad_invdepth):
        means3D, sh, colors_precomp, opacities, scales, rotations, cov3Ds_precomp = ctx.saved_tensors
        st = ctx.st
        feats = sh if ctx.src == "sh" else colors_precomp
        if grad_color is None:
            V, C, H, W = st.views.V, st.C, st.views.H, st.views.W
            grad_color = torch.zeros((V, C, H, W), dtype=torch.float32, device=means3D.device)
        need_feat = ctx.needs_input_grad[2] or ctx.needs_input_grad[3]
        g = backward_views(st, means3D, feats, opacities, scales, rotations, cov3Ds_precomp, grad_color, grad_invdepth,
                           ctx.bg, want_dfeatures=need_feat, plans=_AUTOGRAD_PLANS)
        red = (lambda t: None if t is None else t[0]) if st.views.V == 1 else (lambda t: None if t is None else t.sum(0))
        gf = red(g["features"])
        grad_sh = gf.reshape(sh.shape) if (gf is not None and ctx.src == "sh") else None
        grad_cp = gf.reshape(colors_precomp.shape) if (gf is not None and ctx.src == "colors") else None
        has_cov = cov3Ds_precomp is not None and cov3Ds_precomp.numel() > 0
        return (red(g["means3D"]), red(g["means2D"]), grad_sh, grad_cp, red(g["opacities"]).reshape(opacities.shape),
                red(g["scales"]), red(g["rotations"]), red(g["cov3D"]) if has_cov else None,
                None, None, None, None, None, None, None, None)


def rasterize_gaussians(means3D, means2D, sh, colors_precomp, opacities, scales, rotations, cov3Ds_precomp,
                        raster_settings, clamp01=False, raw_params=False):
    views = ViewBatch.from_settings(raster_settings)
    return _RasterizeViews.apply(means3D, means2D, sh, colors_precomp, opacities, scales, rotations, cov3Ds_precomp,
                                 views, raster_settings.scale_modifier, bool(raster_settings.antialiasing), clamp01,
                                 bool(raster_settings.debug), raster_settings.bg, True, bool(raw_params))


def rasterize_views(views: ViewBatch, means3D, means2D, sh, opacities, scales=None, rotations=None, cov3D_precomp=None,
                    colors_precomp=None, scale_modifier=1.0, antialiasing=False, clamp01=False, debug=False, bg=None):
    emp = torch.empty(0)
    z = lambda t: emp if t is None else t
    return _RasterizeViews.apply(means3D, z(means2D), z(sh), z(colors_precomp), opacities, z(scales), z(rotations),
                                 z(cov3D_precomp), views, scale_modifier, antialiasing, clamp01, debug, bg, False)


class GaussianRasterizer(nn.Module):
# ... 68 lines not shown
```

Measured before the change: 63240.

## Prefill next iteration's output planes inside backward kernels using double-buffered outputs

```diff
diff --git a/include/skelsplat_hip.h b/include/skelsplat_hip.h
--- a/include/skelsplat_hip.h
+++ b/include/skelsplat_hip.h
@@ -61,6 +61,31 @@
                  float* dL_dscales, float* dL_drotations, float* dL_dcov3D, float* dL_dfeatures,
                  float* dL_dmeans3D_mean ,
                  void* stream);
+
+int sks_prefill_planes(int V, int P, int C, int W, int H, unsigned flags, int* planes_wave, int* planes_geom);
+int sks_forward_prefilled(int V, int P, int C, int W, int H,
+                          const float* viewmatrix, const float* projmatrix,
+                          const float* tanfovx , const float* tanfovy ,
+                          const float* means3D, const float* features, const float* opacities,
+                          const float* scales, const float* rotations, const float* cov3D_precomp,
+                          float scale_modifier, unsigned flags,
+                          float* out_color, float* out_invdepth, int* radii,
+                          void* geom, void* binning, size_t bin_capacity, int* num_rendered_dev,
+                          float* final_T, uint32_t* n_contrib, int prefilled_planes, void* stream);
+int sks_backward_prefill(int V, int P, int C, int W, int H,
+                         const float* viewmatrix, const float* projmatrix,
+                         const float* tanfovx , const float* tanfovy ,
+                         const float* bg,
+                         const float* means3D, const float* features, const float* opacities,
+                         const float* scales, const float* rotations, const float* cov3D_precomp,
+                         float scale_modifier, unsigned flags,
+                         const int* radii, const void* geom, const void* binning, size_t bin_capacity,
+                         const float* dL_dout_color, const float* dL_dout_invdepth,
+                         void* accum,
+                         float* dL_dmeans3D, float* dL_dmeans2D, float* dL_dopacity,
+                         float* dL_dscales, float* dL_drotations, float* dL_dcov3D, float* dL_dfeatures,
+                         float* dL_dmeans3D_mean,
+                         float* next_color, float* next_invdepth, int planes_wave, int planes_geom, void* stream);
 
 #define SKS_FB_NO_JOIN 1u
 int sks_forward_backward(int V, int P, int C, int W, int H,
diff --git a/skelsplat_amd/_lib.py b/skelsplat_amd/_lib.py
--- a/skelsplat_amd/_lib.py
+++ b/skelsplat_amd/_lib.py
@@ -50,6 +50,9 @@
 FORWARD_PARAMS = _CAMERAS + _GAUSSIANS + _FORWARD_IO + (("final_T", _vp), ("n_contrib", _vp), ("stream", _vp))
 BACKWARD_PARAMS = _CAMERAS + (("bg", _vp),) + _GAUSSIANS + (("radii", _vp), ("geom", _vp), ("binning", _vp), ("bin_capacity", _sz)) \
     + _UPSTREAM + _GRADS + (("stream", _vp),)
+FORWARD_PREFILLED_PARAMS = FORWARD_PARAMS[:-1] + (("prefilled_planes", _i), ("stream", _vp))
+BACKWARD_PREFILL_PARAMS = BACKWARD_PARAMS[:-1] + (("next_color", _vp), ("next_invdepth", _vp), ("planes_wave", _i), ("planes_geom", _i),
+                                                  ("stream", _vp))
 FORWARD_BACKWARD_PARAMS = _CAMERAS + _GAUSSIANS + _FORWARD_IO + (("bg", _vp),) + _UPSTREAM + _GRADS \
     + (("stream", _vp), ("aux_stream", _vp), ("fb_flags", _u))
 
@@ -102,6 +105,9 @@
     "sks_forward": (_i, [ct for _, ct in FORWARD_PARAMS]),
     "sks_backward": (_i, [ct for _, ct in BACKWARD_PARAMS]),
     "sks_forward_backward": (_i, [ct for _, ct in FORWARD_BACKWARD_PARAMS]),
+    "sks_forward_prefilled": (_i, [ct for _, ct in FORWARD_PREFILLED_PARAMS]),
+    "sks_backward_prefill": (_i, [ct for _, ct in BACKWARD_PREFILL_PARAMS]),
+    "sks_prefill_planes": (_i, [_i, _i, _i, _i, _i, _u, C.POINTER(_i), C.POINTER(_i)]),
     "sks_mark_visible": (_i, [_i, _vp, _vp, _vp, _vp, _vp]),
     "sks_mean_views": (_i, [_i, _i, _vp, _i, _vp, _vp]),
     "sks_export_lists": (_i, [_i, _i, _i, _vp, _sz, _vp, _vp, _vp]),
@@ -141,6 +147,10 @@
 }
 
 
+_PREFILL_SYMBOLS = ("sks_forward_prefilled", "sks_backward_prefill", "sks_prefill_planes")
+HAS_PREFILL = True
+
+
 def load(build_if_missing=True):
     global _lib
     if _lib is not None:
@@ -155,8 +165,13 @@
                 raise ImportError(f"libskelsplat_hip.so is missing and could not be built: {e}") from e
     if not os.path.exists(LIB_PATH):
         raise ImportError(f"{LIB_PATH} not found; run `python -m skelsplat_amd.build`")
-    lib = C.CDLL(os.environ.get("SKS_LIB_OVERRIDE") or LIB_PATH)
+    override = os.environ.get("SKS_LIB_OVERRIDE")
+    lib = C.CDLL(override or LIB_PATH)
+    global HAS_PREFILL
     for name, (res, args) in SIGNATURES.items():
+        if override and name in _PREFILL_SYMBOLS and not hasattr(lib, name):
+            HAS_PREFILL = False
+            continue
         fn = getattr(lib, name)
         fn.restype = res
         fn.argtypes = args
@@ -176,6 +191,12 @@
     return g.value, b.value, a.value
 
 
+def prefill_planes(V, P, C_, W, H, flags=0):
+    nw, ng = _i(0), _i(0)
+    check(load().sks_prefill_planes(V, P, C_, W, H, flags, C.byref(nw), C.byref(ng)), "sks_prefill_planes")
+    return nw.value, ng.value
+
+
 def ptr(t):
     if t is None or t.numel() == 0:
         return None
diff --git a/skelsplat_amd/csrc/sks_bwd_small.inc b/skelsplat_amd/csrc/sks_bwd_small.inc
--- a/skelsplat_amd/csrc/sks_bwd_small.inc
+++ b/skelsplat_amd/csrc/sks_bwd_small.inc
@@ -262,9 +262,17 @@
 __device__ __forceinline__ float rl(float x, int lane) { return __int_as_float(__builtin_amdgcn_readlane(__float_as_int(x), lane)); }
 __device__ __forceinline__ unsigned rlu(unsigned x, int lane) { return (unsigned)__builtin_amdgcn_readlane((int)x, lane); }
 
-template <int CG, bool DFEAT, bool LOSS, bool HMF = false, bool ES = false>
-__global__ __launch_bounds__(256, (DFEAT || CG > 20) ? 1 : 4) void k_render_bwd_wave(BwdArgs a, ViewTan vt, ViewOff vo)
+template <int CG, bool DFEAT, bool LOSS, bool HMF = false, bool ES = false, class... PF>
+__global__ __launch_bounds__(256, (DFEAT || CG > 20) ? 1 : 4) void k_render_bwd_wave(BwdArgs a, ViewTan vt, ViewOff vo, PF... pf)
 {
+    static_assert(sizeof...(PF) <= 1 && (!LOSS || sizeof...(PF) == 0), "the prefill role belongs to the plain variants");
+    if constexpr (sizeof...(PF) == 1) {
+        const PreFill& f = (pf, ...);
+        if ((int)blockIdx.z >= f.zs) {
+            prefill_block(f, ((unsigned)((int)blockIdx.z - f.zs) * gridDim.y + blockIdx.y) * gridDim.x + blockIdx.x);
+            return;
+        }
+    }
     static_assert(!(DFEAT && LOSS), "the fused-loss variant has no feature gradient");
     static_assert(LOSS || !HMF, "heat-map factors belong to the fused-loss variant");
     static_assert(LOSS || !ES, "early stopping belongs to the fused-loss variant");
@@ -273,7 +281,9 @@
     }
     constexpr int NV = LOSS ? NACC + 1 : NACC + (DFEAT ? CG : 0);
     __shared__ float s_red[2][4][NV];
-    const int g = blockIdx.x, v = blockIdx.y, sp = blockIdx.z, zs = gridDim.z, tid = threadIdx.x, lane = tid & 63, wv = tid >> 6;
+    int zs_ = gridDim.z;
+    if constexpr (sizeof...(PF) == 1) zs_ = (pf, ...).zs;
+    const int g = blockIdx.x, v = blockIdx.y, sp = blockIdx.z, zs = zs_, tid = threadIdx.x, lane = tid & 63, wv = tid >> 6;
     const int P = a.P, C = a.C, W = vt.w[v], H = vt.h[v];
     const int NVS = NACC + C;
     const size_t HW = (size_t)H * W;
diff --git a/skelsplat_amd/csrc/sks_common.inc b/skelsplat_amd/csrc/sks_common.inc
--- a/skelsplat_amd/csrc/sks_common.inc
+++ b/skelsplat_amd/csrc/sks_common.inc
@@ -28,6 +28,9 @@
 struct ProfKind {
     hipEvent_t b[PROF_MAX], e[PROF_MAX];
     int created = 0, n = 0;
+    hipEvent_t xb[PROF_MAX], xe[PROF_MAX];
+    bool hasx[PROF_MAX];
+    int xcreated = 0;
 };
 struct ProfState {
     bool on = false;
@@ -36,6 +39,9 @@
     bool recorded = false;
     int seen[2] = { 0, 0 };
     ProfKind kind[2];
+    hipEvent_t park_b = nullptr, park_e = nullptr;
+    bool parked = false;
+    hipStream_t park_st = nullptr;
 };
 thread_local ProfState* tl_prof = nullptr;
 
@@ -44,10 +50,13 @@
     hipStream_t st;
     bool ext;
     bool began = false;
-    ProfScope(int kind, hipStream_t s, bool ext_ = false) : st(s), ext(ext_)
+    ProfScope(int kind, hipStream_t s, bool ext_ = false, bool take_parked = false) : st(s), ext(ext_)
     {
         ProfState* ps = tl_prof;
-        if (!ps || !ps->on || ((ps->skip >> kind) & 1)) return;
+        if (!ps) return;
+        const bool parked = kind == 0 && ps->parked && take_parked && ps->park_st == s;
+        if (kind == 0) ps->parked = false;
+        if (!ps->on || ((ps->skip >> kind) & 1)) return;
         if (ps->seen[kind]++ % ps->every != 0) return;
         ProfKind& p = ps->kind[kind];
         if (p.n >= PROF_MAX) return;
@@ -55,6 +64,16 @@
             if (hipEventCreate(&p.b[p.created]) != hipSuccess || hipEventCreate(&p.e[p.created]) != hipSuccess) return;
             p.created++;
         }
+        p.hasx[p.n] = false;
+        if (parked) {
+            while (p.xcreated <= p.n) {
+                if (hipEventCreate(&p.xb[p.xcreated]) != hipSuccess || hipEventCreate(&p.xe[p.xcreated]) != hipSuccess) return;
+                p.xcreated++;
+            }
+            hipEvent_t t = p.xb[p.n]; p.xb[p.n] = ps->park_b; ps->park_b = t;
+            t = p.xe[p.n]; p.xe[p.n] = ps->park_e; ps->park_e = t;
+            p.hasx[p.n] = true;
+        }
         k = &p;
         if (ps->recorded) ext = false;
         if (!ext) (void)hipEventRecord(p.b[p.n], st);
@@ -68,6 +87,37 @@
         k->n++;
     }
 };
+inline bool prof_next_forward_sampled()
+{
+    const ProfState* ps = tl_prof;
+    return ps && ps->on && !(ps->skip & 1) && ps->seen[0] % ps->every == 0 && ps->kind[0].n < PROF_MAX;
+}
+inline bool prof_has_parked(hipStream_t st) { return tl_prof && tl_prof->parked && tl_prof->park_st == st; }
+inline void prof_park_begin(hipStream_t st)
+{
+    ProfState* ps = tl_prof;
+    ps->parked = false;
+    if (!ps->park_b && (hipEventCreate(&ps->park_b) != hipSuccess || hipEventCreate(&ps->park_e) != hipSuccess)) { ps->park_b = ps->park_e = nullptr; return; }
+    ps->park_st = st;
+    ps->parked = hipEventRecord(ps->park_b, st) == hipSuccess;
+}
+inline void prof_park_end(hipStream_t st)
+{
+    ProfState* ps = tl_prof;
+    if (ps && ps->parked && ps->park_st == st && hipEventRecord(ps->park_e, st) != hipSuccess) ps->parked = false;
+}
+inline hipError_t prof_elapsed(ProfKind& p, int i, float* ms)
+{
+    hipError_t e = hipEventSynchronize(p.e[i]);
+    if (e == hipSuccess) e = hipEventElapsedTime(ms, p.b[i], p.e[i]);
+    if (e == hipSuccess && p.hasx[i]) {
+        float x = 0;
+        e = hipEventSynchronize(p.xe[i]);
+        if (e == hipSuccess) e = hipEventElapsedTime(&x, p.xb[i], p.xe[i]);
+        *ms += x;
+    }
+    return e;
+}
 #define SKS_LAUNCH(prof, kernel, grid, block, lds, stream, ...)                                                  \
     do {                                                                                                         \
         if ((prof).k)                                                                                            \
diff --git a/skelsplat_amd/csrc/sks_fwd_small.inc b/skelsplat_amd/csrc/sks_fwd_small.inc
--- a/skelsplat_amd/csrc/sks_fwd_small.inc
+++ b/skelsplat_amd/csrc/sks_fwd_small.inc
@@ -401,3 +401,34 @@
     const int shift = (int)((reinterpret_cast<uintptr_t>(out) >> 2) & 31u);
     fill_bare<PPT, NT>(out, nullptr, nullptr, q * (256 * PPT) * f.pb + (int)threadIdx.x * PPT - shift, Nb, min(f.pb, 32));
 }
+
+struct PreFill {
+    float* out_color;
+    float* out_invdepth;
+    int C, W, H, gy;
+    int zid0;
+    unsigned nfill;
+    int fsplit, pb;
+    int zs;
+    unsigned cp1_magic;
+    unsigned row_magic;
+    unsigned fs_magic;
+};
+
+__device__ __forceinline__ void prefill_block(const PreFill& f, unsigned e)
+{
+    if (e >= f.nfill) return;
+    const unsigned rows = (unsigned)(f.fsplit * f.gy);
+    const unsigned zr = f.row_magic ? __umulhi(e, f.row_magic) : e;
+    const unsigned rem = e - zr * rows;
+    const int band = (int)(f.fs_magic ? __umulhi(rem, f.fs_magic) : rem);
+    const int q = (int)rem - band * f.fsplit;
+    const int zid = f.zid0 + (int)zr;
+    const int v = (int)(((unsigned)zid * f.cp1_magic) >> 20);
+    const int plane = zid - v * (f.C + 1);
+    const size_t HW = (size_t)f.H * f.W;
+    const int Nb = min(TILE, f.H - band * TILE) * f.W;
+    float* out = (plane == f.C ? f.out_invdepth + (size_t)v * HW : f.out_color + ((size_t)v * f.C + plane) * HW) + (size_t)band * TILE * f.W;
+    const int shift = (int)((reinterpret_cast<uintptr_t>(out) >> 2) & 31u);
+    fill_bare<4, true>(out, nullptr, nullptr, q * 1024 * f.pb + (int)threadIdx.x * 4 - shift, Nb, min(f.pb, 32));
+}
diff --git a/skelsplat_amd/csrc/sks_geom_bwd.inc b/skelsplat_amd/csrc/sks_geom_bwd.inc
--- a/skelsplat_amd/csrc/sks_geom_bwd.inc
+++ b/skelsplat_amd/csrc/sks_geom_bwd.inc
@@ -431,8 +431,16 @@
     geom_bwd_finish<true>(a, vt, v, idx, g, 1.0, &in);
 }
 
-__global__ __launch_bounds__(256) void k_geom_bwd_all(GeomBwdArgs a, ViewTan vt, int V, float* __restrict__ mean_out)
-{
+template <class... PF>
+__global__ __launch_bounds__(256) void k_geom_bwd_all(GeomBwdArgs a, ViewTan vt, int V, float* __restrict__ mean_out, PF... pf)
+{
+    static_assert(sizeof...(PF) <= 1, "at most one PreFill");
+    if constexpr (sizeof...(PF) == 1) {
+        if (blockIdx.x > 0) {
+            prefill_block((pf, ...), blockIdx.x - 1u);
+            return;
+        }
+    }
     const int t = threadIdx.x;
     const int v = t / a.P, idx = t - v * a.P;
     const bool live = v < V;
diff --git a/skelsplat_amd/csrc/sks_raster.hip b/skelsplat_amd/csrc/sks_raster.hip
--- a/skelsplat_amd/csrc/sks_raster.hip
+++ b/skelsplat_amd/csrc/sks_raster.hip
@@ -97,21 +97,21 @@
 
 inline unsigned magic32(unsigned d) { return (unsigned)(((1ull << 32) + d - 1) / d); }
 
-bool early_fill_cut(const FwdArgs& a_in, int V, int gy, int gplanes, int zid0, int& fsplit, int& pb)
+bool early_fill_cut(const FwdArgs& a_in, int V, int gy, int gplanes, int zid0, int zid1, int& fsplit, int& pb)
 {
     FwdArgs a = a_in;
     a.flags |= SKS_FILL_LINEAR;
     fill_geometry(a, true, false, fsplit, pb);
-    const long long rows = (long long)fsplit * gy, nfill = rows * ((a.C + 1) * V - zid0);
+    const long long rows = (long long)fsplit * gy, nfill = rows * (zid1 - zid0);
     return fsplit >= 1 && pb >= 1 && nfill * rows < (1ll << 32) && (long long)V * gplanes + nfill < (1ll << 31);
 }
 
-void launch_geom_fill(const FwdArgs& a, int V, int gy, int gplanes, int zid0, int fsplit, int pb, const ViewTan& vt,
+void launch_geom_fill(const FwdArgs& a, int V, int gy, int gplanes, int zid0, int zid1, int fsplit, int pb, const ViewTan& vt,
                       const float* viewmatrix, const float* projmatrix, const float* means3D, const float* opacities,
                       const float* scales, const float* rotations, const float* cov3D_precomp, float smod, int* radii,
                       hipStream_t st, ProfScope& prof)
 {
-    const long long rows = (long long)fsplit * gy, nfill = rows * ((a.C + 1) * V - zid0);
+    const long long rows = (long long)fsplit * gy, nfill = rows * (zid1 - zid0);
     const int ngeom = V * gplanes;
     const EarlyFill f{ a.out_color, a.out_invdepth, a.C, a.W, a.H, gy, gplanes, ngeom, zid0, fsplit, pb, a.cp1_magic,
                        rows > 1 ? magic32((unsigned)rows) : 0u, fsplit > 1 ? magic32((unsigned)fsplit) : 0u };
@@ -188,13 +188,54 @@
     }
 }
 
+struct PrefillReq {
+    float* color;
+    float* invdepth;
+    int planes_wave, planes_geom;
+};
+#ifndef SKS_PREFILL_PASSES
+#define SKS_PREFILL_PASSES 2
+#endif
+inline int prefill_passes()
+{
+    static const int n = [] { const char* e = getenv("SKS_PREFILL_PB"); return (e && atoi(e) > 0) ? atoi(e) : SKS_PREFILL_PASSES; }();
+    return n > 32 ? 32 : n;
+}
+inline bool prefill_possible(int P, int W, int H, unsigned flags)
+{
+    return P >= 1 && P <= 64 && P <= SKS_SMALL_P && !(flags & (SKS_FORCE_BINNED | SKS_NO_NT_STORES | SKS_DEBUG_SYNC | (1u << 20))) &&
+           (W % 4 == 0 || (W % 4 == 2 && H % 2 == 0));
+}
+bool prefill_cut(PreFill& f, float* color, float* invdepth, int V, int C, int W, int H, int zid0, int nz, long long per_unit, long long max_units)
+{
+    const int gy = (H + TILE - 1) / TILE;
+    const bool lines = color && invdepth && (((uintptr_t)color | (uintptr_t)invdepth) & 127u) == 0;
+    const int lead = (lines && (long long)H * W % 32 == 0 && TILE * W % 32 == 0) ? 0 : 31;
+    const int passes = (TILE * W + lead + 1023) / 1024;
+    const int pb = prefill_passes();
+    const int fsplit = (passes + pb - 1) / pb;
+    const long long rows = (long long)fsplit * gy, nfill = rows * nz;
+    if (zid0 < 0 || nz < 1 || zid0 + nz > (C + 1) * V || nfill * rows >= (1ll << 32) || (nfill + per_unit - 1) / per_unit > max_units) return false;
+    f = PreFill{ color, invdepth, C, W, H, gy, zid0, (unsigned)nfill, fsplit, pb, 0, ((1u << 20) + (unsigned)C) / (unsigned)(C + 1),
+                 rows > 1 ? magic32((unsigned)rows) : 0u, fsplit > 1 ? magic32((unsigned)fsplit) : 0u };
+    return true;
+}
+
 template <int CG>
 void launch_bwd_small(const BwdArgs& a, const ViewTan& vt, const ViewOff& vo, int V, int gy, bool dfeat, hipStream_t st,
-                      const ProfScope& prof)
+                      const ProfScope& prof, const PreFill* pf = nullptr)
 {
     (void)gy;
     if (a.P <= 64 && !(a.flags & (1u << 20))) {
         dim3 grid(a.P, V, bwd_wave_groups(V, a.P, a.flags));
+        if (pf) {
+            PreFill f = *pf;
+            f.zs = (int)grid.z;
+            grid.z += (unsigned)((f.nfill + (unsigned)(a.P * V) - 1) / (unsigned)(a.P * V));
+            if (dfeat) SKS_LAUNCH(prof, (k_render_bwd_wave<CG, true, false, false, false, PreFill>), grid, dim3(256), 0, st, a, vt, vo, f);
+            else SKS_LAUNCH(prof, (k_render_bwd_wave<CG, false, false, false, false, PreFill>), grid, dim3(256), 0, st, a, vt, vo, f);
+            return;
+        }
         if (dfeat) SKS_LAUNCH(prof, (k_render_bwd_wave<CG, true, false>), grid, dim3(256), 0, st, a, vt, vo);
         else SKS_LAUNCH(prof, (k_render_bwd_wave<CG, false, false>), grid, dim3(256), 0, st, a, vt, vo);
         return;
@@ -290,10 +331,11 @@
                  const float* opacities, const float* scales, const float* rotations, const float* cov3D_precomp,
                  float scale_modifier, unsigned flags, float* out_color, float* out_invdepth, int* radii, void* geom,
                  void* binning, size_t bin_capacity, int* num_rendered_dev, float* final_T, uint32_t* n_contrib,
-                 void* stream, const FwdHook* hook)
+                 void* stream, const FwdHook* hook, int prefilled = 0)
 {
     if (int rc = check_common(V, P, C, W, H)) return rc;
     hipStream_t st = (hipStream_t)stream;
+    if (prefilled < 0 || prefilled > (C + 1) * V) return fail(-1, "prefilled_planes=%d out of range [0,%d]", prefilled, (C + 1) * V);
     if (!out_color || !out_invdepth) return fail(-2, "out_color / out_invdepth must be provided");
     if (((uintptr_t)out_color | (uintptr_t)out_invdepth) & 15u)
         return fail(-2, "out_color / out_invdepth must be 16-byte aligned (the planes are written with 16-byte stores)");
@@ -328,19 +370,26 @@
                (W >= 2 && W < 16384) ? (unsigned)(((1ull << 32) + (unsigned)W - 1) / (unsigned)W) : 0u };
     const int cg = pick_cg(C);
     const int planes = (C + 1) * V;
+    int pre = 0;
+    if (prefilled > 0 && small && !hook && !final_T && !n_contrib && !(flags & SKS_DEBUG_SYNC) &&
+        !(prof_next_forward_sampled() && !prof_has_parked(st)))
+        pre = prefilled;
+    const int zp = planes - pre;
     int early = 0;
-    if (small && !hook && g.cover && !final_T && !n_contrib && !(flags & (SKS_DEBUG_SYNC | SKS_NO_EARLY_FILL)))
+    if (small && !hook && g.cover && !final_T && !n_contrib && !(flags & (SKS_DEBUG_SYNC | SKS_NO_EARLY_FILL))) {
         early = early_fill_planes(flags, planes, HW * 4);
+        if (early > zp) early = zp;
+    }
     int efs = 0, epb = 0;
-    if (early > 0 && early_fill_cut(a, V, gy, gplanes, planes - early, efs, epb)) {
-        ProfScope prof(0, st, true);
-        launch_geom_fill(a, V, gy, gplanes, planes - early, efs, epb, vt, viewmatrix, projmatrix, means3D, opacities, scales, rotations,
+    if (early > 0 && early_fill_cut(a, V, gy, gplanes, zp - early, zp, efs, epb)) {
+        ProfScope prof(0, st, true, pre > 0);
+        launch_geom_fill(a, V, gy, gplanes, zp - early, zp, efs, epb, vt, viewmatrix, projmatrix, means3D, opacities, scales, rotations,
                          cov3D_precomp, scale_modifier, radii, st, prof);
         switch (cg) {
-            case 4: launch_fwd_small<4>(a, V, gy, planes - early, st, prof); break;
-            case 16: launch_fwd_small<16>(a, V, gy, planes - early, st, prof); break;
-            case 20: launch_fwd_small<20>(a, V, gy, planes - early, st, prof); break;
-            default: launch_fwd_small<32>(a, V, gy, planes - early, st, prof); break;
+            case 4: launch_fwd_small<4>(a, V, gy, zp - early, st, prof); break;
+            case 16: launch_fwd_small<16>(a, V, gy, zp - early, st, prof); break;
+            case 20: launch_fwd_small<20>(a, V, gy, zp - early, st, prof); break;
+            default: launch_fwd_small<32>(a, V, gy, zp - early, st, prof); break;
         }
         HIP_TRY(hipGetLastError());
         return 0;
@@ -362,12 +411,12 @@
 
     if (small) {
         {
-            ProfScope prof(0, st, true);
+            ProfScope prof(0, st, true, pre > 0);
             switch (cg) {
-                case 4: launch_fwd_small<4>(a, V, gy, planes, st, prof); break;
-                case 16: launch_fwd_small<16>(a, V, gy, planes, st, prof); break;
-                case 20: launch_fwd_small<20>(a, V, gy, planes, st, prof); break;
-                default: launch_fwd_small<32>(a, V, gy, planes, st, prof); break;
+                case 4: launch_fwd_small<4>(a, V, gy, zp, st, prof); break;
+                case 16: launch_fwd_small<16>(a, V, gy, zp, st, prof); break;
+                case 20: launch_fwd_small<20>(a, V, gy, zp, st, prof); break;
+                default: launch_fwd_small<32>(a, V, gy, zp, st, prof); break;
             }
         }
         STAGE_CHECK("render(small)");
@@ -447,7 +496,7 @@
                   const void* binning, size_t bin_capacity, const float* dL_dout_color, const float* dL_dout_invdepth,
                   void* accum, float* dL_dmeans3D, float* dL_dmeans2D, float* dL_dopacity, float* dL_dscales,
                   float* dL_drotations, float* dL_dcov3D, float* dL_dfeatures, float* dL_dmeans3D_mean, void* stream,
-                  unsigned phases, int group)
+                  unsigned phases, int group, const PrefillReq* pre = nullptr)
 {
     if (int rc = check_common(V, P, C, W, H)) return rc;
     if (P == 0) return 0;
@@ -468,13 +517,32 @@
     int vg = V, ng = 1;
     if (!small) bin_groups(flags, V, vg, ng);
     if (group >= ng) return fail(-1, "view group %d of %d", group, ng);
+    const bool geom_all = dL_dmeans3D_mean && V * P <= 256 && small;
+    PreFill pfw{}, pfg{};
+    bool have_pfw = false, have_pfg = false;
+    if (pre && pre->planes_wave + pre->planes_geom > 0) {
+        const int planes = (C + 1) * V, n = pre->planes_wave + pre->planes_geom;
+        const int n_geom = geom_all ? pre->planes_geom : 0, nw = n - n_geom;
+        if (nw > 0) {
+            if (!prefill_cut(pfw, pre->color, pre->invdepth, V, C, W, H, planes - n, nw, (long long)P * V, 65535 - BWD_SPLITS))
+                return fail(-1, "sks_backward_prefill: %d planes of %dx%d do not fit the compositing backward's launch", nw, W, H);
+            have_pfw = true;
+        }
+        if (n_geom > 0) {
+            if (!prefill_cut(pfg, pre->color, pre->invdepth, V, C, W, H, planes - n_geom, n_geom, 1, (1ll << 31) - 2))
+                return fail(-1, "sks_backward_prefill: %d planes of %dx%d do not fit the geometry backward's launch", n_geom, W, H);
+            have_pfg = true;
+        }
+        if (prof_next_forward_sampled()) prof_park_begin(st);
+    }
     if ((phases & BWD_RENDER) && small) {
         ProfScope prof(1, st, true);
+        const PreFill* pf = have_pfw ? &pfw : nullptr;
         switch (cg) {
-            case 4: launch_bwd_small<4>(a, vt, vo, V, gy, dfeat, st, prof); break;
-            case 16: launch_bwd_small<16>(a, vt, vo, V, gy, dfeat, st, prof); break;
-            case 20: launch_bwd_small<20>(a, vt, vo, V, gy, dfeat, st, prof); break;
-            default: launch_bwd_small<32>(a, vt, vo, V, gy, dfeat, st, prof); break;
+            case 4: launch_bwd_small<4>(a, vt, vo, V, gy, dfeat, st, prof, pf); break;
+            case 16: launch_bwd_small<16>(a, vt, vo, V, gy, dfeat, st, prof, pf); break;
+            case 20: launch_bwd_small<20>(a, vt, vo, V, gy, dfeat, st, prof, pf); break;
+            default: launch_bwd_small<32>(a, vt, vo, V, gy, dfeat, st, prof, pf); break;
         }
         STAGE_CHECK("render-backward(small)");
     } else if (phases & BWD_RENDER) {
@@ -507,8 +575,9 @@
         ga.cap = bin_capacity;
         ga.bin_hdr = b.hdr;
     }
-    if (dL_dmeans3D_mean && V * P <= 256 && small) {
-        hipLaunchKernelGGL(k_geom_bwd_all, dim3(1), dim3(256), 0, st, ga, vt, V, dL_dmeans3D_mean);
+    if (geom_all) {
+        if (have_pfg) hipLaunchKernelGGL((k_geom_bwd_all<PreFill>), dim3(1u + pfg.nfill), dim3(256), 0, st, ga, vt, V, dL_dmeans3D_mean, pfg);
+        else hipLaunchKernelGGL((k_geom_bwd_all<>), dim3(1), dim3(256), 0, st, ga, vt, V, dL_dmeans3D_mean);
     } else {
         if (small) hipLaunchKernelGGL(k_geom_bwd, dim3((P + 255) / 256, V), dim3(256), 0, st, ga, vt);
         else {
@@ -519,6 +588,7 @@
         if (dL_dmeans3D_mean && (small || group < 0 || group == ng - 1))
             hipLaunchKernelGGL(k_mean_views, dim3((3 * P + 255) / 256), dim3(256), 0, st, V, P, dL_dmeans3D, dL_dmeans3D_mean);
     }
+    if (have_pfw || have_pfg) prof_park_end(st);
     STAGE_CHECK("geometry-backward");
     return 0;
 }
@@ -539,6 +609,74 @@
                          cov3D_precomp, scale_modifier, flags, radii, geom, binning, bin_capacity, dL_dout_color, dL_dout_invdepth, accum,
                          dL_dmeans3D, dL_dmeans2D, dL_dopacity, dL_dscales, dL_drotations, dL_dcov3D, dL_dfeatures, dL_dmeans3D_mean,
                          stream, BWD_RENDER | BWD_GEOM, -1);
+}
+
+int sks_forward_prefilled(int V, int P, int C, int W, int H, const float* viewmatrix, const float* projmatrix,
+                          const float* tanfovx, const float* tanfovy, const float* means3D, const float* features,
+                          const float* opacities, const float* scales, const float* rotations, const float* cov3D_precomp,
+                          float scale_modifier, unsigned flags, float* out_color, float* out_invdepth, int* radii, void* geom,
+                          void* binning, size_t bin_capacity, int* num_rendered_dev, float* final_T, uint32_t* n_contrib,
+                          int prefilled_planes, void* stream)
+{
+    return forward_impl(V, P, C, W, H, viewmatrix, projmatrix, tanfovx, tanfovy, means3D, features, opacities, scales, rotations,
+                        cov3D_precomp, scale_modifier, flags, out_color, out_invdepth, radii, geom, binning, bin_capacity,
+                        num_rendered_dev, final_T, n_contrib, stream, nullptr, prefilled_planes);
+}
+
+int sks_backward_prefill(int V, int P, int C, int W, int H, const float* viewmatrix, const float* projmatrix,
+                         const float* tanfovx, const float* tanfovy, const float* bg, const float* means3D,
+                         const float* features, const float* opacities, const float* scales, const float* rotations,
+                         const float* cov3D_precomp, float scale_modifier, unsigned flags, const int* radii, const void* geom,
+                         const void* binning, size_t bin_capacity, const float* dL_dout_color, const float* dL_dout_invdepth,
+                         void* accum, float* dL_dmeans3D, float* dL_dmeans2D, float* dL_dopacity, float* dL_dscales,
+                         float* dL_drotations, float* dL_dcov3D, float* dL_dfeatures, float* dL_dmeans3D_mean,
+                         float* next_color, float* next_invdepth, int planes_wave, int planes_geom, void* stream)
+{
+    if (int rc = check_common(V, P, C, W, H)) return rc;
+    if (planes_wave < 0 || planes_geom < 0 || (long long)planes_wave + planes_geom > (long long)(C + 1) * V)
+        return fail(-1, "sks_backward_prefill: planes_wave=%d planes_geom=%d out of range (the call has %d planes)", planes_wave, planes_geom, (C + 1) * V);
+    const PrefillReq req{ next_color, next_invdepth, planes_wave, planes_geom };
+    if (planes_wave + planes_geom > 0) {
+        if (!prefill_possible(P, W, H, flags & ~SKS_NO_NT_STORES))
+            return fail(-1, "sks_backward_prefill: no prefill for this call (wave-resident small path with 16-byte non-temporal stores only: "
+                            "1 <= P <= 64, W %% 4 == 0 or W %% 4 == 2 with an even H, no SKS_NO_NT_STORES / SKS_DEBUG_SYNC / SKS_FORCE_BINNED)");
+        if (!next_color || !next_invdepth) return fail(-2, "sks_backward_prefill: next_color / next_invdepth must be provided");
+        if (((uintptr_t)next_color | (uintptr_t)next_invdepth) & 15u) return fail(-2, "next_color / next_invdepth must be 16-byte aligned");
+    }
+    return backward_impl(V, P, C, W, H, viewmatrix, projmatrix, tanfovx, tanfovy, bg, means3D, features, opacities, scales, rotations,
+                         cov3D_precomp, scale_modifier, flags, radii, geom, binning, bin_capacity, dL_dout_color, dL_dout_invdepth, accum,
+                         dL_dmeans3D, dL_dmeans2D, dL_dopacity, dL_dscales, dL_drotations, dL_dcov3D, dL_dfeatures, dL_dmeans3D_mean,
+                         stream, BWD_RENDER | BWD_GEOM, -1, planes_wave + planes_geom > 0 ? &req : nullptr);
+}
+
+#ifndef SKS_PREFILL_WAVE_BYTES
+#define SKS_PREFILL_WAVE_BYTES 56000000u
+#endif
+#ifndef SKS_PREFILL_GEOM_BYTES
+#define SKS_PREFILL_GEOM_BYTES 28000000u
+#endif
+int sks_prefill_planes(int V, int P, int C, int W, int H, unsigned flags, int* planes_wave, int* planes_geom)
+{
+    if (int rc = check_common(V, P, C, W, H)) return rc;
+    if (!planes_wave || !planes_geom) return fail(-2, "sks_prefill_planes: planes_wave / planes_geom must be provided");
+    *planes_wave = *planes_geom = 0;
+    if (!prefill_possible(P, W, H, flags) || !cover_enabled(P, W, H)) return 0;
+    const int planes = (C + 1) * V;
+    const size_t plane_bytes = (size_t)H * W * 4;
+    const int early = (flags & SKS_NO_EARLY_FILL) ? 0 : early_fill_planes(flags, planes, plane_bytes);
+    int room = planes / 2 - early;
+    if (room <= 0) return 0;
+    if (W % 4 != 0 || C > 20 || V * P < 51 || V * P > 85 || bwd_wave_groups(V, P, flags) != 16) return 0;
+    long long nw = ((long long)SKS_PREFILL_WAVE_BYTES + plane_bytes / 2) / plane_bytes;
+    long long ng = ((long long)SKS_PREFILL_GEOM_BYTES + plane_bytes / 2) / plane_bytes;
+    if (nw > room) nw = room;
+    if (ng > room - nw) ng = room - nw;
+    PreFill f;
+    if (nw > 0 && !prefill_cut(f, nullptr, nullptr, V, C, W, H, planes - (int)(nw + ng), (int)nw, (long long)P * V, 65535 - BWD_SPLITS)) nw = 0;
+    if (ng > 0 && !prefill_cut(f, nullptr, nullptr, V, C, W, H, planes - (int)ng, (int)ng, 1, (1ll << 31) - 2)) ng = 0;
+    *planes_wave = (int)nw;
+    *planes_geom = (int)ng;
+    return 0;
 }
 
 int sks_forward_backward(int V, int P, int C, int W, int H, const float* viewmatrix, const float* projmatrix,
@@ -901,6 +1039,7 @@
     tl_prof->skip = (on >> 16) & 3;
     tl_prof->recorded = (on >> 18) & 1;
     tl_prof->seen[0] = tl_prof->seen[1] = 0;
+    tl_prof->parked = false;
     return 0;
 }
 
@@ -918,9 +1057,8 @@
     ProfKind& p = tl_prof->kind[kind];
     double tot = 0;
     for (int i = 0; i < p.n; i++) {
-        HIP_TRY(hipEventSynchronize(p.e[i]));
         float ms = 0;
-        HIP_TRY(hipEventElapsedTime(&ms, p.b[i], p.e[i]));
+        HIP_TRY(prof_elapsed(p, i, &ms));
         tot += ms;
     }
     *total_ms = tot;
@@ -937,8 +1075,7 @@
     static thread_local float t[PROF_MAX];
     double tot = 0;
     for (int i = 0; i < p.n; i++) {
-        HIP_TRY(hipEventSynchronize(p.e[i]));
-        HIP_TRY(hipEventElapsedTime(&t[i], p.b[i], p.e[i]));
+        HIP_TRY(prof_elapsed(p, i, &t[i]));
         tot += t[i];
     }
     const int n = p.n;
diff --git a/skelsplat_amd/rasterizer.py b/skelsplat_amd/rasterizer.py
--- a/skelsplat_amd/rasterizer.py
+++ b/skelsplat_amd/rasterizer.py
@@ -39,11 +39,16 @@
 
 class Workspace:
 
-    def __init__(self):
+    def __init__(self, prefill=None):
         self._t = {}
         self._plans = {}
         self._aux = {}
         self._pending_join = None
+        if prefill is not None and prefill != 0:
+            prefill = (int(prefill[0]), int(prefill[1]))
+        self._prefill = prefill
+        self._pf = None
+        self._pf_off = prefill == 0
 
     def aux_stream(self, dev_index):
         st = self._aux.get(dev_index)
@@ -86,6 +91,22 @@
         return t
 
 
+class _Prefill:
+    __slots__ = ("shape", "sets", "results", "cur", "note", "fargs", "bplan", "bargs", "rule")
+
+    def __init__(self, shape, color, invdepth, radii, st, args):
+        self.shape = shape
+        self.sets = [(color, invdepth), None]
+        self.results = [(color, invdepth, radii, st), None]
+        self.cur, self.note = 0, None
+        self.fargs = list(args[:-1]) + [0, None]
+        self.bplan = self.bargs = None
+        self.rule = {}
+
+
+_PREFILL_MAX_SET_BYTES = 1 << 30
+
+
 def _sig(t):
     if t is None or t.numel() == 0:
         return None
@@ -101,6 +122,7 @@
 _F_V, _F_FLAGS, _F_COLOR, _F_INVDEPTH, _F_RADII, _F_GEOM, _F_NUM_RENDERED = (
     _lib.FWD[n] for n in ("V", "flags", "out_color", "out_invdepth", "radii", "geom", "num_rendered_dev"))
 _B_RADII, _B_GEOM, _B_DL_COLOR, _B_DL_INVDEPTH = (_lib.BWD[n] for n in ("radii", "geom", "dL_dout_color", "dL_dout_invdepth"))
+_B_DFEAT = _lib.BWD["dL_dfeatures"]
 _GRAD_SLOTS = tuple((k, _lib.BWD[n]) for k, n in (
     ("means3D", "dL_dmeans3D"), ("means2D", "dL_dmeans2D"), ("opacities", "dL_dopacity"), ("scales", "dL_dscales"),
     ("rotations", "dL_drotations"), ("cov3D", "dL_dcov3D"), ("features", "dL_dfeatures")))
@@ -148,6 +170,14 @@
     if key is not None and workspace is not None:
         plan = workspace._plans.get("fwd")
         if plan is not None and plan.key == key:
+            pf = workspace._pf
+            if pf is not None:
+                rc = _forward_two_sets(lib, workspace, pf, plan)
+                if rc != 0:
+                    del workspace._plans["fwd"]
+                    workspace._pf = None
+                _lib.check(rc, "sks_forward")
+                return pf.results[pf.cur]
             ticket = _replay_ticket(workspace, plan)
             rc = _replay(lib.sks_forward, plan.args, plan.dev_index)
             if rc != 0:
@@ -156,6 +186,8 @@
             if ticket is None or (_arena.finish(ticket) or 0) <= ticket.cap:
                 return plan.result
             del workspace._plans["fwd"]
+    if workspace is not None and workspace._pf is not None:
+        workspace._pf.note = None
     if views.mixed:
         raise RuntimeError("the dense forward writes one (V,C,H,W) tensor: all views of the batch must share the image size")
     if means3D is None or means3D.dim() != 2 or means3D.shape[1] != 3:
@@ -228,7 +260,69 @@
         keep = (means3D, feat2, opacities, scales, rotations, cov3D_precomp)
         arena = (ticket.key, cap, True if check_capacity is True else "lazy") if binned and check_capacity else None
         workspace._plans["fwd"] = _FwdRecord(key, (views, keep), args, dev.index, (color, invdepth, radii, st), arena)
+        workspace._pf = None
+        if not binned and P and not workspace._pf_off and _lib.HAS_PREFILL and 4 * (C + 1) * V * H * W <= _PREFILL_MAX_SET_BYTES:
+            workspace._pf = _Prefill((V, P, C, W, H), color, invdepth, radii, st, args)
+    else:
+        workspace._pf_off = True
     return color, invdepth, radii, st
+
+
+def _forward_two_sets(lib, workspace, pf, plan):
+    note, pf.note = pf.note, None
+    args = plan.args
+    if note is not None:
+        if workspace._pf_off or torch.cuda.is_current_stream_capturing():
+            workspace._pf_off = True
+        elif note[1] == torch._C._cuda_getCurrentRawStream(plan.dev_index):
+            other = 1 - pf.cur
+            color, invdepth = pf.sets[other]
+            fargs = pf.fargs
+            fargs[_F_FLAGS], fargs[_F_COLOR], fargs[_F_INVDEPTH], fargs[-2] = args[_F_FLAGS], color.data_ptr(), invdepth.data_ptr(), note[0]
+            rc = _replay(lib.sks_forward_prefilled, fargs, plan.dev_index)
+            if rc == 0:
+                pf.cur = other
+                args[_F_COLOR], args[_F_INVDEPTH] = fargs[_F_COLOR], fargs[_F_INVDEPTH]
+            return rc
+    elif not workspace._pf_off and torch.cuda.is_current_stream_capturing():
+        workspace._pf_off = True
+    return _replay(lib.sks_forward, args, plan.dev_index)
+
+
+def _backward_prefill(lib, workspace, plan):
+    pf = workspace._pf
+    if pf is None or workspace._pf_off or plan.key[0] != id(pf.results[0][3]):
+        return None
+    if torch.cuda.is_current_stream_capturing():
+        workspace._pf_off, pf.note = True, None
+        return None
+    fplan = workspace._plans.get("fwd")
+    if fplan is None:
+        return None
+    fflags = fplan.args[_F_FLAGS]
+    n = pf.rule.get(fflags)
+    if n is None:
+        V, P, C, W, H = pf.shape
+        n = pf.rule[fflags] = _lib.prefill_planes(V, P, C, W, H, fflags) if workspace._prefill is None else workspace._prefill
+    if workspace._prefill is None and plan.args[_B_DFEAT] is not None:
+        return None
+    if n[0] + n[1] == 0:
+        return None
+    if pf.sets[1] is None:
+        color, invdepth, radii, st = pf.results[0]
+        c2 = workspace.get(("fwd", "color2"), color.shape, color.dtype, color.device)
+        i2 = workspace.get(("fwd", "invdepth2"), invdepth.shape, invdepth.dtype, invdepth.device)
+        pf.sets[1], pf.results[1] = (c2, i2), (c2, i2, radii, st)
+    if pf.bplan is not plan:
+        pf.bplan, pf.bargs = plan, list(plan.args[:-1]) + [None, None, 0, 0, None]
+    color, invdepth = pf.sets[1 - pf.cur]
+    bargs = pf.bargs
+    bargs[-5], bargs[-4], bargs[-3], bargs[-2] = color.data_ptr(), invdepth.data_ptr(), n[0], n[1]
+    pf.note = None
+    rc = _replay(lib.sks_backward_prefill, bargs, plan.dev_index)
+    if rc == 0:
+        pf.note = (n[0] + n[1], bargs[-1])
+    return rc
 
 
 def _replay_ticket(workspace, plan):
@@ -351,7 +445,9 @@
                        want_dfeatures, tune_flags, want_mean, out_means3D, torch._C._cuda_getCurrentRawStream(st.geom.device.index))
         plan = workspace._plans.get("bwd")
         if plan is not None and plan.key == key:
-            rc = _replay(lib.sks_backward, plan.args, plan.dev_index)
+            rc = _backward_prefill(lib, workspace, plan)
+            if rc is None:
+                rc = _replay(lib.sks_backward, plan.args, plan.dev_index)
             if rc != 0:
                 reset_scratch()
                 del workspace._plans["bwd"]
@@ -436,7 +532,8 @@
                 if not join and not overlap:
                     aux.wait_stream(torch.cuda.current_stream(dev_index))
                 if ticket is None or (_arena.finish(ticket) or 0) <= ticket.cap:
-                    return fplan.result + (bplan.result,)
+                    pf = workspace._pf
+                    return (fplan.result if pf is None else pf.results[pf.cur]) + (bplan.result,)
                 del workspace._plans["fwd"]
                 workspace.settle()
     out = forward_views(views, means3D, features, opacities, scales, rotations, cov3D_precomp, scale_modifier, antialiasing, clamp01,
```

Result: faster. 70000, median of 6 (+10.7%).
